# kbastani/pinot

Hardware: AMD Instinct MI355X
Metric: rows/sec scanned+aggregated (node) & % HBM peak, AdAnalytics GROUP BY query (higher is better)
Workload: dtype int64; 1 GPU; adanalytics; segments_per_gpu=1000, rows_per_gpu=1000000000, global_rows=1000000000, parallelism=dp1, groups=8, queries_in_flight=3, combine=local

## Files before the change

### include/pinotgpu.h

```cpp
#ifndef PINOTGPU_H
#define PINOTGPU_H

#include <stddef.h>
#include <stdint.h>

#ifdef __cplusplus
extern "C" {
#endif

#define PGPU_ABI_VERSION 3

#define PGPU_OK 0
#define PGPU_ERR_INVALID_ARGUMENT (-1)
#define PGPU_ERR_BAD_QUERY (-2)
#define PGPU_ERR_UNSUPPORTED (-3)
#define PGPU_ERR_DEVICE (-4)
#define PGPU_ERR_OUT_OF_MEMORY (-5)
#define PGPU_ERR_NOT_FOUND (-6)
#define PGPU_ERR_TIMEOUT (-7)
#define PGPU_ERR_CANCELLED (-8)

enum pgpu_data_type { PGPU_INT = 0, PGPU_LONG = 1, PGPU_FLOAT = 2, PGPU_DOUBLE = 3, PGPU_STRING = 4 };

enum pgpu_fwd_format { PGPU_FWD_FIXED_BIT = 0, PGPU_FWD_SORTED_PAIRS = 1, PGPU_FWD_RAW_FIXED = 2 };
// ... 78 lines not shown
  int32_t num_values;
  int32_t lower_inclusive;
  const char* const* values;
  int32_t upper_inclusive;
  int32_t reserved;
} pgpu_predicate;

enum pgpu_filter_opcode { PGPU_OP_PRED = 0, PGPU_OP_AND = 1, PGPU_OP_OR = 2, PGPU_OP_NOT = 3 };
typedef struct {
  int32_t op;
  int32_t arg;
} pgpu_filter_op;

enum pgpu_agg_fn { PGPU_AGG_COUNT = 0, PGPU_AGG_SUM = 1, PGPU_AGG_MIN = 2, PGPU_AGG_MAX = 3, PGPU_AGG_AVG = 4,
                   PGPU_AGG_DISTINCTCOUNT = 5, PGPU_AGG_PERCENTILE = 6 };
#define PGPU_AGG_PERCENTILE_MAX_E4 1000000
#define PGPU_AGG_PERCENTILE_OF(p_e4) ((int32_t)(PGPU_AGG_PERCENTILE | ((int32_t)(p_e4) << 8)))
#define PGPU_AGG_FN(fn) ((int32_t)((fn) & 0xFF))
#define PGPU_AGG_PERCENTILE_E4(fn) ((int32_t)(((uint32_t)(fn)) >> 8))
typedef struct {
  int32_t fn;
  int32_t column;
} pgpu_agg;

enum pgpu_expr_opcode { PGPU_EXPR_COLUMN = 0, PGPU_EXPR_LITERAL = 1, PGPU_EXPR_ADD = 2, PGPU_EXPR_SUB = 3,
                        PGPU_EXPR_MULT = 4, PGPU_EXPR_DIV = 5,
                        PGPU_EXPR_EQ = 6, PGPU_EXPR_NE = 7, PGPU_EXPR_GT = 8, PGPU_EXPR_GE = 9, PGPU_EXPR_LT = 10,
                        PGPU_EXPR_LE = 11, PGPU_EXPR_AND = 12, PGPU_EXPR_OR = 13, PGPU_EXPR_SELECT = 14,
                        PGPU_EXPR_ABS = 16, PGPU_EXPR_CEIL = 17, PGPU_EXPR_FLOOR = 18, PGPU_EXPR_SQRT = 19,
                        PGPU_EXPR_MOD = 20, PGPU_EXPR_LDIV = 21 };
#define PGPU_EXPR_MAX_OPS 16
#define PGPU_EXPR_MAX_DEPTH 4
#define PGPU_EXPR_MAX_COLUMNS 4
#define PGPU_EXPR_MAX_PER_TABLE 256
typedef struct {
  int32_t op;
  int32_t column;
  double literal;
} pgpu_expr_op;
int pgpu_table_add_expression(pgpu_table table, const pgpu_expr_op* ops, int32_t n, const char* name, int32_t* column);
int pgpu_table_expression(pgpu_table table, int32_t column, pgpu_expr_op* ops, int32_t cap, int32_t* n, char* name,
                          int32_t name_cap);

#define PGPU_GROUP_EXPR_COLUMN_BASE (1 << 20)
#define PGPU_GROUP_EXPR_MAX_PER_TABLE 64
#define PGPU_GROUP_EXPR_MAX_PRODUCT (1 << 22)
int pgpu_table_add_group_expression(pgpu_table table, const pgpu_expr_op* ops, int32_t n, const char* name,
                                    int32_t result_type , int32_t* column);

typedef struct {
  int32_t num_predicates;
  int32_t num_filter_ops;
  const pgpu_predicate* predicates;
  const pgpu_filter_op* filter;
  int32_t num_group_by;
  int32_t num_aggs;
  const int32_t* group_by;
  const pgpu_agg* aggs;
  int32_t num_groups_limit;
  int32_t options;
  int64_t end_time_ms;
} pgpu_query;

#define PGPU_OPT_NO_STAR_TREE 1
#define PGPU_OPT_SQL_GROUP_BY 2
#define PGPU_OPT_NO_PLAN_CACHE 4
#define PGPU_OPT_TIMING 8
#define PGPU_OPT_EXACT_FP_SUM 16

typedef struct pgpu_plan_s* pgpu_plan;
typedef struct pgpu_result_s* pgpu_result;

int pgpu_plan_create(pgpu_table table, const int64_t* segment_handles, int32_t num_segments, const pgpu_query* q,
                     pgpu_plan* out);
int pgpu_plan_destroy(pgpu_plan plan);

enum pgpu_slot_kind { PGPU_SLOT_COUNT = 0, PGPU_SLOT_SUM_I64 = 1, PGPU_SLOT_SUM_F64 = 2, PGPU_SLOT_MIN_KEY = 3,
                      PGPU_SLOT_MAX_KEY = 4 };
int pgpu_plan_layout(pgpu_plan plan, int32_t* num_slots, int64_t* num_keys, int32_t* slot_kinds );

int pgpu_plan_cancel(pgpu_plan plan);

int pgpu_plan_leaf_kinds(pgpu_plan plan, int64_t* counts);

int pgpu_plan_regexp_stats(pgpu_plan plan, int64_t* out4);
int pgpu_regex_check(const char* pattern, int32_t* states, int32_t* classes, int64_t* table_bytes);
int pgpu_regex_match_host(const char* pattern, const void* value, int64_t len, int32_t* matched);
int pgpu_table_regexp_dict_ids(pgpu_table table, int32_t column, const char* pattern, uint64_t* bitmap, int64_t words);

enum pgpu_group_path { PGPU_PATH_LDS = 0, PGPU_PATH_GLOBAL = 1, PGPU_PATH_HASH = 2, PGPU_PATH_PARTITIONED = 3,
                       PGPU_PATH_HASH_PARTITIONED = 4 };
int pgpu_plan_group_path(pgpu_plan plan, int32_t* path);

int pgpu_plan_execute(pgpu_plan plan, void* stream, void* d_table);

int pgpu_plan_finalize(pgpu_plan plan, void* stream, const void* d_table, pgpu_result* out);

int pgpu_plan_finalize_range(pgpu_plan plan, void* stream, const void* d_table_shard, int64_t key_begin,
                             int64_t key_count, pgpu_result* out);

int pgpu_plan_exchange_counts(pgpu_plan plan, void* stream, int32_t nparts, int64_t* counts);
int pgpu_plan_exchange_export(pgpu_plan plan, void* stream, int32_t nparts, const int32_t* kinds, void* d_out,
                              int64_t cap);
int pgpu_plan_exchange_merge(pgpu_plan plan, void* stream, const int32_t* kinds, const void* d_records, int64_t n);

typedef struct pgpu_comm_s* pgpu_comm;
#define PGPU_COMM_RCCL 0
#define PGPU_COMM_HOST 1
#define PGPU_COMM_ID_BYTES 128
int pgpu_comm_unique_id(int32_t kind, void* id );
int pgpu_comm_create(int32_t kind, const void* id, int32_t nranks, int32_t rank, int32_t device, pgpu_comm* out);
int pgpu_comm_destroy(pgpu_comm comm);
int pgpu_comm_rank(pgpu_comm comm, int32_t* rank, int32_t* nranks);
int pgpu_comm_allgather(pgpu_comm comm, const void* send, int64_t bytes, void* recv);
int pgpu_comm_set_timeout(pgpu_comm comm, int64_t timeout_ms);
int pgpu_comm_abort(pgpu_comm comm);
int pgpu_comm_status(pgpu_comm comm, int32_t* aborted);
int pgpu_comm_recreate(pgpu_comm comm, const void* id);

#define PGPU_COMBINE_LOCAL 0
#define PGPU_COMBINE_ALL_REDUCE 1
#define PGPU_COMBINE_REDUCE_SCATTER 2
#define PGPU_COMBINE_HASH 3
#define PGPU_COMBINE_ROWS 4
int pgpu_plan_combine_mode(pgpu_plan plan, pgpu_comm comm, int64_t shard_bytes, int32_t* mode, int32_t* kinds);
int pgpu_plan_combine(pgpu_plan plan, pgpu_comm comm, void* stream, void* d_table, int32_t mode, const int32_t* kinds,
                      void* d_shard, int64_t* key_begin, int64_t* key_count);
int pgpu_result_combine_rows(pgpu_result r, pgpu_comm comm, pgpu_result* out);

int pgpu_execute_groupby(pgpu_table table, const int64_t* segment_handles, int32_t num_segments, const pgpu_query* q,
                         void* stream, pgpu_result* out);

int pgpu_plan_create_execute(pgpu_table table, const int64_t* segment_handles, int32_t num_segments,
                             const pgpu_query* q, void* stream, void* d_table, pgpu_plan* out);

int pgpu_plan_timing(pgpu_plan plan, double* out4);

int pgpu_plan_fp_sum_format(pgpu_plan plan, int agg, int32_t out[4]);

typedef struct {
  int32_t is_sum;
  int32_t any, finite;
  int32_t E, L;
  int32_t reserved;
  int64_t docs;
  double  int_sum_bound;
} pgpu_fp_sum_range;
int pgpu_query_fp_sum_ranges(pgpu_table table, const int64_t* segment_handles, int32_t num_segments,
                             const pgpu_query* q, pgpu_fp_sum_range* out);
int pgpu_fp_sum_ranges_merge(const pgpu_fp_sum_range* all, int32_t nranks, int32_t num_aggs, pgpu_fp_sum_range* out);
int pgpu_comm_agree_fp_sum_ranges(pgpu_comm comm, pgpu_fp_sum_range* ranges, int32_t num_aggs);
int pgpu_plan_create_agreed(pgpu_table table, const int64_t* segment_handles, int32_t num_segments,
                            const pgpu_query* q, const pgpu_fp_sum_range* agreed, pgpu_plan* out);

int pgpu_plan_star_work(pgpu_plan plan, int64_t* out3);
int pgpu_plan_scan_geometry(pgpu_plan plan, int64_t* out16);
int pgpu_plan_star_metric_bytes(pgpu_plan plan, int64_t* bytes);

int pgpu_plan_scanned_segments(pgpu_plan plan, uint8_t* out);

enum pgpu_leaf_type { PGPU_LEAF_EMPTY = 0, PGPU_LEAF_MATCH_ALL = 1, PGPU_LEAF_SCAN = 2, PGPU_LEAF_SORTED = 3,
                      PGPU_LEAF_BITMAP = 4, PGPU_LEAF_RANGE_INDEX = 5, PGPU_LEAF_EXPRESSION = 6 };
int pgpu_filter_entries_scanned(const pgpu_filter_op* filter, int32_t num_filter_ops, const int32_t* leaf_types,
                                const uint32_t* const* leaf_masks, int32_t num_leaves, int32_t num_docs,
                                int64_t* out);

// ... 118 lines not shown
```

### pinot_amd/_lib.py

```python
import ctypes
import os

from .build import LIB_PATH

c_int = ctypes.c_int
c_i32 = ctypes.c_int32
c_i64 = ctypes.c_int64
c_u8p = ctypes.POINTER(ctypes.c_uint8)
c_i32p = ctypes.POINTER(ctypes.c_int32)
c_i64p = ctypes.POINTER(ctypes.c_int64)
c_u64p = ctypes.POINTER(ctypes.c_uint64)
c_f64p = ctypes.POINTER(ctypes.c_double)
c_voidp = ctypes.c_void_p
c_char_pp = ctypes.POINTER(ctypes.c_char_p)

PGPU_OK = 0
PGPU_ERR_INVALID_ARGUMENT = -1
PGPU_ERR_BAD_QUERY = -2
PGPU_ERR_UNSUPPORTED = -3
PGPU_ERR_DEVICE = -4
PGPU_ERR_OUT_OF_MEMORY = -5
PGPU_ERR_NOT_FOUND = -6
PGPU_ERR_TIMEOUT = -7
PGPU_ERR_CANCELLED = -8
# ... 114 lines not shown
    def as_tuple(self):
        return (self.is_sum, self.any, self.finite, self.E, self.L, self.docs, self.int_sum_bound)

    @classmethod
    def from_tuple(cls, t):
        return cls(int(t[0]), int(t[1]), int(t[2]), int(t[3]), int(t[4]), 0, int(t[5]), float(t[6]))


def fp_sum_range_array(ranges):
    items = [r if isinstance(r, FpSumRangeC) else FpSumRangeC.from_tuple(r) for r in ranges]
    arr = (FpSumRangeC * max(len(items), 1))()
    for i, r in enumerate(items):
        arr[i] = r
    return arr


def merge_fp_sum_ranges(per_rank):
    nranks, na = len(per_rank), len(per_rank[0])
    if any(len(r) != na for r in per_rank):
        raise ValueError("ranks report different numbers of aggregations")
    flat = fp_sum_range_array([x for r in per_rank for x in r])
    out = (FpSumRangeC * max(na, 1))()
    check(load().pgpu_fp_sum_ranges_merge(flat, nranks, na, out))
    return [FpSumRangeC.from_tuple(out[a].as_tuple()) for a in range(na)]


class PinotGpuError(RuntimeError):
    def __init__(self, code, message):
        super().__init__("pgpu error %d: %s" % (code, message))
        self.code = code
        self.message = message


class BadQueryRequestException(PinotGpuError):
    """PGPU_ERR_BAD_QUERY: mirrors org.apache.pinot.spi.exception.BadQueryRequestException."""


class UnsupportedQueryError(PinotGpuError):
    """PGPU_ERR_UNSUPPORTED: the query shape is outside the GPU path."""


class QueryCancelledError(PinotGpuError):
    """PGPU_ERR_CANCELLED: pgpu_plan_cancel abandoned the query (BaseOperator's EarlyTerminationException after the
    combine cancels its futures, BaseOperator.java:37-39 / BaseCombineOperator.java:124-130)."""


class QueryTimeoutError(PinotGpuError):
    """PGPU_ERR_TIMEOUT: the query's end time passed (the combine's TimeoutException; Pinot reports
    QueryException.EXECUTION_TIMEOUT_ERROR_CODE 250 for aggregation-only and QUERY_EXECUTION_ERROR_CODE 200 for
    group-by, BaseCombineOperator.java:193-203 / GroupByCombineOperator.java:193-203)."""


_PROTOS = {
    "pgpu_abi_version": (c_int, []),
    "pgpu_init": (c_int, [c_int]),
    "pgpu_shutdown": (c_int, []),
    "pgpu_last_error": (c_int, [ctypes.c_char_p, ctypes.c_size_t]),
    "pgpu_device_count": (c_int, [ctypes.POINTER(c_int)]),
    "pgpu_table_create": (c_int, [c_int, c_int, c_char_pp, c_i32p, ctypes.POINTER(c_voidp)]),
    "pgpu_config_default": (c_int, [ctypes.POINTER(ConfigC)]),
    "pgpu_table_set_config": (c_int, [c_voidp, ctypes.POINTER(ConfigC)]),
    "pgpu_table_get_config": (c_int, [c_voidp, ctypes.POINTER(ConfigC)]),
    "pgpu_table_destroy": (c_int, [c_voidp]),
    "pgpu_table_add_expression": (c_int, [c_voidp, ctypes.POINTER(ExprOpC), c_i32, ctypes.c_char_p, c_i32p]),
    "pgpu_table_add_group_expression": (c_int, [c_voidp, ctypes.POINTER(ExprOpC), c_i32, ctypes.c_char_p, c_i32, c_i32p]),
    "pgpu_table_expression": (c_int, [c_voidp, c_i32, ctypes.POINTER(ExprOpC), c_i32, c_i32p, ctypes.c_char_p, c_i32]),
    "pgpu_pin_segment": (c_int, [c_voidp, ctypes.POINTER(SegmentDesc), c_i64p]),
    "pgpu_unpin_segment": (c_int, [c_voidp, c_i64]),
    "pgpu_table_num_segments": (c_int, [c_voidp, c_i32p]),
    "pgpu_table_device_bytes": (c_i64, [c_voidp]),
    "pgpu_table_add_dictionary_values": (c_int, [c_voidp, c_int, c_i64, c_i64p, c_f64p, c_u8p, c_i64p]),
    "pgpu_table_dictionary_size": (c_int, [c_voidp, c_int, c_i64p]),
    "pgpu_table_dictionary_i64": (c_int, [c_voidp, c_int, c_i64p]),
    "pgpu_table_dictionary_f64": (c_int, [c_voidp, c_int, c_f64p]),
    "pgpu_table_dictionary_str": (c_int, [c_voidp, c_int, c_u8p, c_i64, c_i64p]),
    "pgpu_read_dict_ids": (c_int, [c_voidp, c_i64, c_int, c_i32p, c_i32, c_i32p]),
    "pgpu_unpack_fixed_bit_device": (c_int, [c_voidp, c_i64, c_i32, c_i64, c_i64, c_voidp, c_voidp]),
    "pgpu_plan_create": (c_int, [c_voidp, c_i64p, c_i32, ctypes.POINTER(QueryC), ctypes.POINTER(c_voidp)]),
    "pgpu_plan_destroy": (c_int, [c_voidp]),
    "pgpu_plan_create_execute": (c_int, [c_voidp, c_i64p, c_i32, ctypes.POINTER(QueryC), c_voidp, c_voidp,
                                         ctypes.POINTER(c_voidp)]),
    "pgpu_plan_layout": (c_int, [c_voidp, c_i32p, c_i64p, c_i32p]),
    "pgpu_plan_leaf_kinds": (c_int, [c_voidp, c_i64p]),
    "pgpu_plan_group_path": (c_int, [c_voidp, c_i32p]),
    "pgpu_plan_regexp_stats": (c_int, [c_voidp, c_i64p]),
    "pgpu_regex_check": (c_int, [ctypes.c_char_p, c_i32p, c_i32p, c_i64p]),
    "pgpu_regex_match_host": (c_int, [ctypes.c_char_p, ctypes.c_char_p, c_i64, c_i32p]),
    "pgpu_table_regexp_dict_ids": (c_int, [c_voidp, c_i32, ctypes.c_char_p, c_u64p, c_i64]),
    "pgpu_plan_cancel": (c_int, [c_voidp]),
    "pgpu_plan_execute": (c_int, [c_voidp, c_voidp, c_voidp]),
    "pgpu_plan_finalize": (c_int, [c_voidp, c_voidp, c_voidp, ctypes.POINTER(c_voidp)]),
    "pgpu_plan_finalize_range": (c_int, [c_voidp, c_voidp, c_voidp, c_i64, c_i64, ctypes.POINTER(c_voidp)]),
    "pgpu_plan_exchange_counts": (c_int, [c_voidp, c_voidp, c_i32, c_i64p]),
    "pgpu_plan_exchange_export": (c_int, [c_voidp, c_voidp, c_i32, c_i32p, c_voidp, c_i64]),
    "pgpu_plan_exchange_merge": (c_int, [c_voidp, c_voidp, c_i32p, c_voidp, c_i64]),
    "pgpu_execute_groupby": (c_int, [c_voidp, c_i64p, c_i32, ctypes.POINTER(QueryC), c_voidp,
                                     ctypes.POINTER(c_voidp)]),
    "pgpu_plan_timing": (c_int, [c_voidp, c_f64p]),
    "pgpu_plan_fp_sum_format": (c_int, [c_voidp, c_int, c_i32p]),
    "pgpu_query_fp_sum_ranges": (c_int, [c_voidp, c_i64p, c_i32, ctypes.POINTER(QueryC), ctypes.POINTER(FpSumRangeC)]),
    "pgpu_fp_sum_ranges_merge": (c_int, [ctypes.POINTER(FpSumRangeC), c_i32, c_i32, ctypes.POINTER(FpSumRangeC)]),
    "pgpu_comm_agree_fp_sum_ranges": (c_int, [c_voidp, ctypes.POINTER(FpSumRangeC), c_i32]),
    "pgpu_plan_create_agreed": (c_int, [c_voidp, c_i64p, c_i32, ctypes.POINTER(QueryC), ctypes.POINTER(FpSumRangeC),
                                        ctypes.POINTER(c_voidp)]),
    "pgpu_plan_star_work": (c_int, [c_voidp, c_i64p]),
    "pgpu_plan_scan_geometry": (c_int, [c_voidp, c_i64p]),
    "pgpu_plan_star_metric_bytes": (c_int, [c_voidp, c_i64p]),
    "pgpu_plan_scanned_segments": (c_int, [c_voidp, c_u8p]),
    "pgpu_attach_startree": (c_int, [c_voidp, c_i64, ctypes.POINTER(StarTreeDescC)]),
    "pgpu_attach_inverted_index": (c_int, [c_voidp, c_i64, c_i32, c_voidp, c_i64]),
    "pgpu_inverted_index_check": (c_int, [c_voidp, c_i64, c_i32, c_i32, c_voidp]),
    "pgpu_build_inverted_index": (c_int, [c_voidp, c_i64, c_i32, c_i32, c_i32, c_voidp, c_i64, c_i64p]),
    "pgpu_raw_forward_index_values": (c_int, [c_voidp, c_i64, c_i32, c_i32, c_i64p, c_f64p]),
    "pgpu_startree_build": (c_int, [ctypes.POINTER(SegmentDesc), c_i32p, c_i32p, c_i32, c_i32p, c_i32,
                                    ctypes.POINTER(AggC), c_i32, c_i32, ctypes.POINTER(c_voidp)]),
    "pgpu_startree_load": (c_int, [c_voidp, c_i64, ctypes.c_char_p, c_i64, c_i32, c_i32, c_i32, c_char_pp, c_i32p,
                                   ctypes.POINTER(c_voidp)]),
    "pgpu_startree_get_desc": (c_int, [c_voidp, ctypes.POINTER(StarTreeDescC)]),
    "pgpu_startree_num_raw_records": (c_int, [c_voidp, c_i32p]),
    "pgpu_startree_destroy": (c_int, [c_voidp]),
    "pgpu_result_num_groups": (c_int, [c_voidp, c_i64p]),
    "pgpu_result_key_dictionary": (c_int, [c_voidp, c_int, c_u64p, c_i64p]),
    "pgpu_result_key_dictionary_i64": (c_int, [c_voidp, c_int, c_i64p]),
    "pgpu_result_key_dictionary_f64": (c_int, [c_voidp, c_int, c_f64p]),
    "pgpu_result_key_dictionary_str": (c_int, [c_voidp, c_int, c_u8p, c_i64, c_i64p]),
    "pgpu_result_group_ids": (c_int, [c_voidp, c_i32p]),
    "pgpu_result_group_ids_column": (c_int, [c_voidp, c_int, c_i32p]),
    "pgpu_result_group_ids_view": (c_int, [c_voidp, c_int, ctypes.POINTER(c_voidp)]),
    "pgpu_result_words_view": (c_int, [c_voidp, c_int, ctypes.POINTER(c_voidp), c_i32p]),
    "pgpu_result_values": (c_int, [c_voidp, c_int, c_f64p]),
    "pgpu_result_avg_counts": (c_int, [c_voidp, c_int, c_i64p]),
    "pgpu_result_values_i64": (c_int, [c_voidp, c_int, c_i64p]),
    "pgpu_result_stats": (c_int, [c_voidp, c_i64p]),
    "pgpu_result_groups_limit_reached": (c_int, [c_voidp, ctypes.POINTER(ctypes.c_int32)]),
    "pgpu_result_slot_kinds": (c_int, [c_voidp, c_i32p, c_i32p]),
    "pgpu_result_exchange_rows": (c_int, [c_voidp, c_i32, c_i32p, c_i64p, c_i64p]),
    "pgpu_result_merge_rows": (c_int, [c_voidp, c_i64p, c_i64, c_i32p, ctypes.POINTER(c_voidp)]),
    "pgpu_result_destroy": (c_int, [c_voidp]),
    "pgpu_comm_unique_id": (c_int, [c_i32, c_voidp]),
    "pgpu_comm_create": (c_int, [c_i32, c_voidp, c_i32, c_i32, c_i32, ctypes.POINTER(c_voidp)]),
    "pgpu_comm_destroy": (c_int, [c_voidp]),
    "pgpu_comm_rank": (c_int, [c_voidp, c_i32p, c_i32p]),
    "pgpu_comm_allgather": (c_int, [c_voidp, c_voidp, c_i64, c_voidp]),
    "pgpu_comm_set_timeout": (c_int, [c_voidp, c_i64]),
    "pgpu_comm_abort": (c_int, [c_voidp]),
    "pgpu_comm_status": (c_int, [c_voidp, c_i32p]),
    "pgpu_attach_range_index": (c_int, [c_voidp, c_i64, c_i32, c_voidp, c_i64]),
    "pgpu_range_index_check": (c_int, [c_voidp, c_i64, c_i32, c_i32, c_i32p, c_i32p, c_i64p]),
    "pgpu_range_index_partial_entries": (c_int, [c_voidp, c_i64, c_i32, c_i32, c_i32, c_i32, c_i64p]),
    "pgpu_comm_recreate": (c_int, [c_voidp, c_voidp]),
    "pgpu_plan_combine_mode": (c_int, [c_voidp, c_voidp, c_i64, c_i32p, c_i32p]),
    "pgpu_plan_combine": (c_int, [c_voidp, c_voidp, c_voidp, c_voidp, c_i32, c_i32p, c_voidp, c_i64p, c_i64p]),
    "pgpu_result_combine_rows": (c_int, [c_voidp, c_voidp, ctypes.POINTER(c_voidp)]),
    "pgpu_free_result": (c_int, [c_voidp]),
    "pgpu_filter_bitmap": (c_int, [c_voidp, c_i64, ctypes.POINTER(QueryC), c_u64p]),
    "pgpu_result_trim_sql": (c_int, [c_voidp, ctypes.POINTER(SqlTrimC), ctypes.POINTER(c_voidp)]),
    "pgpu_result_trim_pql": (c_int, [c_voidp, c_i32, c_i32, c_i64p, c_i64, c_i64p]),
    "pgpu_result_datatable": (c_int, [c_voidp, c_voidp, c_voidp, c_i64, c_i64p]),
    "pgpu_broker_reduce_sql": (c_int, [ctypes.POINTER(c_voidp), c_i64p, c_i32, ctypes.POINTER(SqlTrimC), c_voidp,
                                       c_i64, c_i64p]),
    "pgpu_filter_entries_scanned": (c_int, [ctypes.POINTER(FilterOpC), c_i32, c_i32p, ctypes.POINTER(c_voidp), c_i32,
                                            c_i32, c_i64p]),
    "pgpu_generate_segment": (c_int, [c_voidp, ctypes.POINTER(GenColumnC), c_i32, c_i64, c_i32, c_i64p]),
    "pgpu_segment_column_info": (c_int, [c_voidp, c_i64, c_int, c_i32p, c_i32p, c_i64p, c_i64p]),
    "pgpu_segment_column_bytes": (c_int, [c_voidp, c_i64, c_int, c_u8p, c_u8p]),
}
# ... 79 lines not shown
```

### pinot_amd/build.py

```python
import hashlib
import os
import shutil
import subprocess

HERE = os.path.dirname(os.path.abspath(__file__))
ROOT = os.path.dirname(HERE)
CSRC = os.path.join(HERE, "csrc")
LIB_PATH = os.path.join(HERE, "libpinotgpu.so")
RUNTIME = ["rt_core", "rt_dict", "rt_plan", "rt_plan_create", "rt_exec", "rt_finalize", "rt_groups", "rt_regex",
           "abi_table", "abi_plan", "abi_combine", "abi_result"]
SOURCES = [("kernels.hip", [], "kernels")] + [(n + ".cpp", [], n) for n in RUNTIME] + [("startree.cpp", [], "startree"),
           ("filter_stats.cpp", [], "filter_stats"), ("range_index.cpp", [], "range_index"), ("comm.cpp", [], "comm"), ("server_response.cpp", [], "server_response"),
           ("k_partition.hip", [], "k_partition"), ("k_partition_fx.hip", [], "k_partition_fx"),
           ("k_hashfinal.hip", [], "k_hashfinal"), ("k_derive.hip", [], "k_derive"),
           ("regex_dfa.cpp", [], "regex_dfa"), ("k_regex.hip", [], "k_regex")] + \
    [("k_%s.hip" % k, ["-DPGPU_FAMILY=%d" % f, "-DPGPU_MODE=%d" % m], "k_%s%s_%d" % (k, ("", "_fx", "_dc", "_hist", "_expr")[f], m))
     for k, f, modes in (("direct", 0, 3), ("startree", 0, 3), ("direct", 1, 3), ("startree", 1, 3), ("direct", 2, 2),
                         ("direct", 3, 2), ("direct", 4, 3))
     for m in range(modes)]
HEADERS = ["internal.h", "device.h", "scan_direct.h", "host_common.h", "startree_kernels.h",
           "partition.h", "filter_stats.h", "host_result.h", "comm.h", "range_index.h", "rt.h",
           "rt_decls.h", "tile_split.h", "fx_sum.h", "key_range.h", "expr_eval.h", "expr_leaf.h", "expr_docs.h", "derive.h", "group_expr.h", "regex_dfa.h", "scan_direct_body.inc", "part_aggregate_body.inc",
           "part_hash_aggregate_body.inc"]
ARCH = os.environ.get("PGPU_OFFLOAD_ARCH", "gfx950")


def _hipcc():
    for cand in (os.environ.get("HIPCC"), "/opt/rocm/bin/hipcc", shutil.which("hipcc")):
        if cand and os.path.exists(cand):
            return cand
    raise RuntimeError("hipcc not found (ROCm is required to build libpinotgpu.so)")


def _inputs():
    files = [os.path.join(CSRC, s[0]) for s in SOURCES] + [os.path.join(CSRC, h) for h in HEADERS]
    files.append(os.path.join(ROOT, "include", "pinotgpu.h"))
    return files


def is_stale():
    if not os.path.exists(LIB_PATH):
        return True
    t = os.path.getmtime(LIB_PATH)
    return any(os.path.getmtime(f) > t for f in _inputs())


def build(force=False, verbose=False, defines=(), out=None):
    lib_path = out or LIB_PATH
    if not force and not defines and not out and not is_stale():
        return LIB_PATH
    hipcc = _hipcc()
    flags = ["--offload-arch=" + ARCH, "-O3", "-fPIC", "-std=c++17", "-munsafe-fp-atomics",
             "-Wall", "-Wno-unused-result", "-Wno-unused-value"] + ["-D" + d for d in defines]
    objdir = os.path.join(ROOT, "build", "obj" if not out else "obj_" + os.path.basename(out).replace(".", "_"))
    os.makedirs(objdir, exist_ok=True)
    procs = []
    objs = []
    common = hashlib.sha1()
    for h in HEADERS + ["../../include/pinotgpu.h"]:
        with open(os.path.join(CSRC, h), "rb") as f:
            common.update(f.read())
    for src, extra, name in SOURCES:
        obj = os.path.join(objdir, name + ".o")
        objs.append(obj)
        dbg = ["-g"] if src.endswith(".cpp") else []
        cmd = [hipcc] + flags + dbg + extra + ["-c", os.path.join(CSRC, src), "-o", obj]
        key = common.copy()
        key.update(" ".join(cmd).encode())
        with open(os.path.join(CSRC, src), "rb") as f:
            key.update(f.read())
        key = key.hexdigest()
        if not force and os.path.exists(obj) and os.path.exists(obj + ".key"):
            with open(obj + ".key") as f:
                if f.read() == key:
                    continue
        if verbose:
            print(" ".join(cmd))
        procs.append((src, obj, key, subprocess.Popen(cmd, cwd=ROOT, stdout=subprocess.PIPE, stderr=subprocess.STDOUT,
                                                      text=True)))
    errors = []
    for src, obj, key, pr in procs:
        out, _ = pr.communicate()
        if pr.returncode != 0:
            errors.append("%s:\n%s" % (src, out[-8000:]))
        else:
            with open(obj + ".key", "w") as f:
                f.write(key)
    if errors:
        raise RuntimeError("hipcc failed:\n" + "\n".join(errors))
    cmd = [hipcc, "--offload-arch=" + ARCH, "-shared", "-fPIC", "-o", lib_path + ".tmp"] + objs + ["-ldl"]
    res = subprocess.run(cmd, cwd=ROOT, stdout=subprocess.PIPE, stderr=subprocess.STDOUT, text=True)
    if res.returncode != 0:
        raise RuntimeError("hipcc link failed:\n" + res.stdout[-8000:])
    os.replace(lib_path + ".tmp", lib_path)
    return lib_path


def build_tools():
    hipcc = _hipcc()
    out = os.path.join(ROOT, "tools", "qps_native")
    cmd = [hipcc, "--offload-arch=" + ARCH, "-O2", "-std=c++17", os.path.join(ROOT, "tools", "qps_native.cpp"), "-I" + os.path.join(ROOT, "include"),
           "-L" + HERE, "-lpinotgpu", "-Wl,-rpath,$ORIGIN/../pinot_amd", "-o", out]
    res = subprocess.run(cmd, cwd=ROOT, stdout=subprocess.PIPE, stderr=subprocess.STDOUT, text=True)
    if res.returncode != 0:
        raise RuntimeError("hipcc (tools) failed:\n" + res.stdout[-4000:])
    return out


SAN_FLAGS = ["-Xarch_host", "-fsanitize=address", "-Xarch_host", "-fsanitize=undefined", "-Xarch_host",
             "-fno-sanitize-recover=undefined", "-Xarch_host", "-fno-omit-frame-pointer"]
FUZZ_PATH = os.path.join(ROOT, "build", "host_fuzz")


def build_host_fuzz(force=False):
    src = os.path.join(ROOT, "tools", "host_fuzz.cpp")
    if not force and os.path.exists(FUZZ_PATH) and \
            all(os.path.getmtime(f) <= os.path.getmtime(FUZZ_PATH) for f in _inputs() + [src]):
        return FUZZ_PATH
    hipcc = _hipcc()
    flags = ["--offload-arch=" + ARCH, "-O1", "-g", "-std=c++17", "-fPIC",
             "-I" + os.path.join(ROOT, "include")] + SAN_FLAGS
    objdir = os.path.join(ROOT, "build", "obj_san")
    os.makedirs(objdir, exist_ok=True)
    jobs = [(os.path.join(CSRC, s), extra, os.path.join(objdir, name + ".o")) for s, extra, name in SOURCES]
    jobs.append((src, [], os.path.join(objdir, "host_fuzz_main.o")))
    hdr_t = max(os.path.getmtime(f) for f in _inputs() if not f.endswith((".cpp", ".hip")))
    procs = [(s, subprocess.Popen([hipcc] + flags + extra + ["-c", s, "-o", o], cwd=ROOT, stdout=subprocess.PIPE,
                                  stderr=subprocess.STDOUT, text=True)) for s, extra, o in jobs
             if force or not os.path.exists(o) or os.path.getmtime(o) < max(os.path.getmtime(s), hdr_t)]
    errors = []
    for s, pr in procs:
        out, _ = pr.communicate()
        if pr.returncode != 0:
            errors.append("%s:\n%s" % (s, out[-6000:]))
    if errors:
        raise RuntimeError("hipcc (host sanitizers) failed:\n" + "\n".join(errors))
    cmd = [hipcc, "--offload-arch=" + ARCH, "-fsanitize=address", "-fsanitize=undefined", "-o", FUZZ_PATH + ".tmp"] + \
        [o for _, _, o in jobs] + ["-ldl", "-lpthread"]
    res = subprocess.run(cmd, cwd=ROOT, stdout=subprocess.PIPE, stderr=subprocess.STDOUT, text=True)
    if res.returncode != 0:
        raise RuntimeError("hipcc (host sanitizers) link failed:\n" + res.stdout[-6000:])
    os.replace(FUZZ_PATH + ".tmp", FUZZ_PATH)
    return FUZZ_PATH


def _build_header_check(name, src, hdr, force=False, extra=()):
    out = os.path.join(ROOT, "build", name)
    src = os.path.join(ROOT, "tools", src)
    hdr = os.path.join(CSRC, hdr)
    if not force and os.path.exists(out) and all(os.path.getmtime(f) <= os.path.getmtime(out) for f in (src, hdr)):
        return out
    os.makedirs(os.path.dirname(out), exist_ok=True)
    hipcc = _hipcc()
    obj = out + ".o"
    for cmd in ([hipcc, "--offload-arch=" + ARCH, "-O1", "-g", "-std=c++17", "-I" + CSRC] + SAN_FLAGS +
                list(extra) + ["-c", src, "-o", obj],
                [hipcc, "--offload-arch=" + ARCH, "-fsanitize=address", "-fsanitize=undefined", obj,
                 "-o", out + ".tmp"]):
        res = subprocess.run(cmd, cwd=ROOT, stdout=subprocess.PIPE, stderr=subprocess.STDOUT, text=True)
        if res.returncode != 0:
            raise RuntimeError("hipcc (%s) failed:\n%s" % (name, res.stdout[-6000:]))
    os.replace(out + ".tmp", out)
    return out


SPLIT_CHECK_PATH = os.path.join(ROOT, "build", "tile_split_check")
FX_CHECK_PATH = os.path.join(ROOT, "build", "fx_sum_check")
AGREE_CHECK_PATH = os.path.join(ROOT, "build", "fx_agree_check")


def build_tile_split_check(force=False):
    return _build_header_check("tile_split_check", "tile_split_check.cpp", "tile_split.h", force)


def build_fx_sum_check(force=False):
    return _build_header_check("fx_sum_check", "fx_sum_check.cpp", "fx_sum.h", force)


def build_fx_agree_check(force=False):
    return _build_header_check("fx_agree_check", "fx_agree_check.cpp", "fx_sum.h", force)


def build_key_range_check(force=False):
    return _build_header_check("key_range_check", "key_range_check.cpp", "key_range.h", force)


def build_expr_check(force=False):
    return _build_header_check("expr_check", "expr_check.cpp", "expr_eval.h", force, extra=("-ffp-contract=off",))


def build_case_check(force=False):
    return _build_header_check("case_check", "case_check.cpp", "expr_eval.h", force, extra=("-ffp-contract=off",))


def build_math_check(force=False):
    return _build_header_check("math_check", "math_check.cpp", "expr_eval.h", force, extra=("-ffp-contract=off",))


def build_group_expr_check(force=False):
    return _build_header_check("group_expr_check", "group_expr_check.cpp", "group_expr.h", force,
                               extra=("-ffp-contract=off",))


def build_expr_filter_check(force=False):
    out = os.path.join(ROOT, "build", "expr_filter_check")
    srcs = [os.path.join(ROOT, "tools", "expr_filter_check.cpp"), os.path.join(CSRC, "filter_stats.cpp")]
    deps = srcs + [os.path.join(CSRC, h) for h in ("expr_leaf.h", "expr_eval.h", "internal.h", "filter_stats.h",
                                                    "host_common.h", "tile_split.h")]
    if not force and os.path.exists(out) and all(os.path.getmtime(f) <= os.path.getmtime(out) for f in deps):
        return out
    os.makedirs(os.path.dirname(out), exist_ok=True)
    hipcc = _hipcc()
    objs = [out + "_%d.o" % i for i in range(len(srcs))]
    cmds = [[hipcc, "--offload-arch=" + ARCH, "-O1", "-g", "-std=c++17", "-I" + CSRC, "-I" + os.path.join(ROOT, "include"),
             "-ffp-contract=off"] + SAN_FLAGS + ["-c", s, "-o", o] for s, o in zip(srcs, objs)]
    cmds.append([hipcc, "--offload-arch=" + ARCH, "-fsanitize=address", "-fsanitize=undefined"] + objs + ["-o", out + ".tmp"])
    for cmd in cmds:
        res = subprocess.run(cmd, cwd=ROOT, stdout=subprocess.PIPE, stderr=subprocess.STDOUT, text=True)
        if res.returncode != 0:
            raise RuntimeError("hipcc (expr_filter_check) failed:\n%s" % res.stdout[-6000:])
    os.replace(out + ".tmp", out)
    return out


def build_regex_fuzz(force=False):
    out = os.path.join(ROOT, "build", "regex_fuzz")
    srcs = [os.path.join(ROOT, "tools", "regex_fuzz.cpp"), os.path.join(CSRC, "regex_dfa.cpp")]
    deps = srcs + [os.path.join(CSRC, "regex_dfa.h")]
    if not force and os.path.exists(out) and all(os.path.getmtime(f) <= os.path.getmtime(out) for f in deps):
        return out
    os.makedirs(os.path.dirname(out), exist_ok=True)
    hipcc = _hipcc()
    objs = [out + "_%d.o" % i for i in range(len(srcs))]
    cmds = [[hipcc, "--offload-arch=" + ARCH, "-O1", "-g", "-std=c++17", "-I" + CSRC] + SAN_FLAGS + ["-c", s, "-o", o]
            for s, o in zip(srcs, objs)]
    cmds.append([hipcc, "--offload-arch=" + ARCH, "-fsanitize=address", "-fsanitize=undefined"] + objs + ["-o", out + ".tmp"])
    for cmd in cmds:
        res = subprocess.run(cmd, cwd=ROOT, stdout=subprocess.PIPE, stderr=subprocess.STDOUT, text=True)
        if res.returncode != 0:
            raise RuntimeError("hipcc (regex_fuzz) failed:\n%s" % res.stdout[-6000:])
    os.replace(out + ".tmp", out)
    return out


if __name__ == "__main__":
    print(build(force=True, verbose=True))
```

### pinot_amd/csrc/abi_result.cpp

```cpp
#include "rt_decls.h"

extern "C" {

int pgpu_execute_groupby(pgpu_table t, const int64_t* handles, int32_t nsegs, const pgpu_query* q, void* stream,
                         pgpu_result* out) try {
  PGPU_ABI_GUARD;
  pgpu_plan P = nullptr;
  TRY(pgpu_plan_create_execute(t, handles, nsegs, q, stream, nullptr, &P));
  int rc = pgpu_plan_finalize(P, stream, nullptr, out);
  std::string keep = g_err;
  pgpu_plan_destroy(P);
  g_err = keep;
  return rc;
} PGPU_ABI_CATCH

int pgpu_plan_scanned_segments(pgpu_plan P, uint8_t* out) try {
  PGPU_ABI_GUARD;
  if (!P || !out) return fail(PGPU_ERR_INVALID_ARGUMENT, "null argument");
  if (!P->seg_scanned.empty()) memcpy(out, P->seg_scanned.data(), P->seg_scanned.size());
  return 0;
} PGPU_ABI_CATCH

int pgpu_plan_star_work(pgpu_plan P, int64_t* out3) try {
  PGPU_ABI_GUARD;
// ... 308 lines not shown
      std::vector<double> sorted = vals;
      std::sort(sorted.begin(), sorted.end(), dbl_less);
      sorted.erase(std::unique(sorted.begin(), sorted.end(),
                               [](double a, double b) { return !dbl_less(a, b) && !dbl_less(b, a); }),
                   sorted.end());
      D.code_to_pos.resize(g0.n);
      for (int i = 0; i < g0.n; ++i)
        D.code_to_pos[i] = (int32_t)(std::lower_bound(sorted.begin(), sorted.end(), vals[i], dbl_less) - sorted.begin());
      D.pos_f64 = sorted;
      D.npos = (int64_t)sorted.size();
    } else {
      return fail(PGPU_ERR_INVALID_ARGUMENT, "column %d: bad generator kind", c);
    }
  }
  GenScratch& G = t->gen;
  std::vector<std::vector<int32_t>> pos_to_id(ncols);
  TRY(G.pos.ensure((size_t)std::max(num_docs, 1) * 4 * ncols));
  for (int c = 0; c < ncols; ++c) {
    const pgpu_gen_column& g0 = gc[c];
    Domain& D = dom[c];
    const int64_t pres_words = (D.npos + 31) / 32;
    TRY(G.presence.ensure((size_t)pres_words * 4));
    HIP_TRY(hipMemsetAsync(G.presence.p, 0, (size_t)pres_words * 4, st));
    if (!D.code_to_pos.empty()) {
      TRY(G.code_to_pos.ensure(D.code_to_pos.size() * 4));
      HIP_TRY(hipMemcpyAsync(G.code_to_pos.p, D.code_to_pos.data(), D.code_to_pos.size() * 4, hipMemcpyHostToDevice, st));
    }
    if (g0.kind == PGPU_GEN_ZIPF) {
      TRY(G.cdf.ensure((size_t)g0.n * 8));
      HIP_TRY(hipMemcpyAsync(G.cdf.p, g0.cdf, (size_t)g0.n * 8, hipMemcpyHostToDevice, st));
    }
    const uint64_t seed = (uint64_t)(0x5EED0000u + (uint32_t)g0.column_index) << 32;
    const int32_t ncodes = g0.kind == PGPU_GEN_UNIFORM ? 0 : g0.n;
    if (launch_gen_positions(g0.kind, seed, g0.lo, g0.hi - g0.lo, G.cdf.as<double>(), G.code_to_pos.as<int32_t>(),
                             ncodes, row0, num_docs, G.pos.as<int32_t>() + (size_t)c * std::max(num_docs, 1),
                             G.presence.as<uint32_t>(), st))
      return fail(PGPU_ERR_DEVICE, "gen positions launch failed");
    std::vector<uint32_t> pres(pres_words);
    HIP_TRY(hipMemcpyAsync(pres.data(), G.presence.p, (size_t)pres_words * 4, hipMemcpyDeviceToHost, st));
    HIP_TRY(hipStreamSynchronize(st));
    Column& col = seg->cols[c];
    col.dict.type = t->types[c];
    std::vector<int32_t>& p2i = pos_to_id[c];
    p2i.assign(std::max<int64_t>(D.npos, 1), 0);
    int32_t card = 0;
    for (int64_t p = 0; p < D.npos; ++p)
      if ((pres[p >> 5] >> (p & 31)) & 1u) {
        p2i[p] = card++;
        if (g0.kind == PGPU_GEN_UNIFORM) col.dict.iv.push_back(g0.lo + p);
        else if (g0.kind == PGPU_GEN_ZIPF) col.dict.iv.push_back(D.pos_i64[p]);
        else col.dict.dv.push_back(D.pos_f64[p]);
      }
    col.card = card;
    col.bits = num_bits_per_value(card - 1);
    const int type = t->types[c];
    col.entry_width = (type == PGPU_INT || type == PGPU_FLOAT) ? 4 : 8;
    col.raw_dict.assign((size_t)card * col.entry_width, 0);
    for (int32_t i = 0; i < card; ++i) {
      uint8_t* o = col.raw_dict.data() + (size_t)i * col.entry_width;
      if (type == PGPU_INT) wr_be32(o, (uint32_t)(int32_t)col.dict.iv[i]);
      else if (type == PGPU_LONG) wr_be64(o, (uint64_t)col.dict.iv[i]);
      else if (type == PGPU_FLOAT) { float f = (float)col.dict.dv[i]; uint32_t u; memcpy(&u, &f, 4); wr_be32(o, u); }
      else { uint64_t u; memcpy(&u, &col.dict.dv[i], 8); wr_be64(o, u); }
    }
    col.fwd_bytes = ((int64_t)num_docs * col.bits + 7) / 8;
    col.fwd_words = padded_fwd_words(num_docs, col.bits);
    total_words += (col.fwd_words + 63) & ~int64_t(63);
  }
  HIP_TRY(hipMalloc(&seg->d_block, (size_t)std::max<int64_t>(total_words, 64) * 4));
  t->device_bytes += std::max<int64_t>(total_words, 64) * 4;
  HIP_TRY(hipMemsetAsync(seg->d_block, 0, (size_t)std::max<int64_t>(total_words, 64) * 4, st));
  int64_t off = 0;
  for (int c = 0; c < ncols; ++c) {
    Column& col = seg->cols[c];
    col.d_fwd = reinterpret_cast<uint32_t*>(seg->d_block) + off;
    off += (col.fwd_words + 63) & ~int64_t(63);
    TRY(G.pos_to_id.ensure(pos_to_id[c].size() * 4));
    HIP_TRY(hipMemcpyAsync(G.pos_to_id.p, pos_to_id[c].data(), pos_to_id[c].size() * 4, hipMemcpyHostToDevice, st));
    if (launch_gen_pack(G.pos.as<int32_t>() + (size_t)c * std::max(num_docs, 1), G.pos_to_id.as<int32_t>(), num_docs,
                        col.bits, col.d_fwd, st))
      return fail(PGPU_ERR_DEVICE, "gen pack launch failed");
    HIP_TRY(hipStreamSynchronize(st));
  }
  std::lock_guard<std::mutex> lk(t->mu);
  *handle = register_segment(t, std::move(seg));
  return 0;
} PGPU_ABI_CATCH

int pgpu_segment_column_info(pgpu_table t, int64_t h, int col, int32_t* card, int32_t* bits, int64_t* dict_len,
                             int64_t* fwd_len) try {
  PGPU_ABI_GUARD;
  if (!t) return fail(PGPU_ERR_INVALID_ARGUMENT, "null table");
  DeviceGuard g(t->device);
  std::lock_guard<std::mutex> lk(t->mu);
  auto it = t->segments.find(h);
  if (it == t->segments.end()) return fail(PGPU_ERR_NOT_FOUND, "unknown segment handle");
  const Column* cp = nullptr;
  TRY(segment_column(t, *it->second, col, &cp));
  const Column& c = *cp;
  if (card) *card = c.card;
  if (bits) *bits = c.bits;
  if (dict_len) *dict_len = (int64_t)c.raw_dict.size();
  if (fwd_len) *fwd_len = c.fwd_bytes;
  return 0;
} PGPU_ABI_CATCH

int pgpu_segment_column_bytes(pgpu_table t, int64_t h, int col, uint8_t* dict_out, uint8_t* fwd_out) try {
  PGPU_ABI_GUARD;
  if (!t) return fail(PGPU_ERR_INVALID_ARGUMENT, "null table");
  DeviceGuard g(t->device);
  std::shared_ptr<Segment> s;
  const Column* cp = nullptr;
  {
    std::lock_guard<std::mutex> lk(t->mu);
    auto it = t->segments.find(h);
    if (it == t->segments.end()) return fail(PGPU_ERR_NOT_FOUND, "unknown segment handle");
    s = it->second;
    TRY(segment_column(t, *s, col, &cp));
  }
  const Column& c = *cp;
  if (dict_out && !c.raw_dict.empty()) memcpy(dict_out, c.raw_dict.data(), c.raw_dict.size());
  if (fwd_out && c.fwd_bytes > 0) {
    HIP_TRY(hipMemcpyAsync(fwd_out, c.d_fwd, (size_t)c.fwd_bytes, hipMemcpyDeviceToHost, t->stream));
    HIP_TRY(hipStreamSynchronize(t->stream));
  }
  return 0;
} PGPU_ABI_CATCH

}
```

### pinot_amd/csrc/abi_table.cpp

```cpp
#include "rt_decls.h"

extern "C" {

int pgpu_abi_version(void) { return PGPU_ABI_VERSION; }

namespace {
std::mutex g_init_mu;
int g_init_devices = 0;
}

int pgpu_init(int n_gpus) try {
  PGPU_ABI_GUARD;
  install_crash_trace();
  int count = 0;
  HIP_TRY(hipGetDeviceCount(&count));
  if (n_gpus > count) return fail(PGPU_ERR_INVALID_ARGUMENT, "%d devices requested, %d visible", n_gpus, count);
  const int n = n_gpus > 0 ? n_gpus : count;
  std::lock_guard<std::mutex> g(g_init_mu);
  int prev = 0;
  HIP_TRY(hipGetDevice(&prev));
  for (int d = g_init_devices; d < n; ++d) {
    HIP_TRY(hipSetDevice(d));
    HIP_TRY(hipFree(nullptr));
  }
// ... 305 lines not shown
                    (long long)cb.fwd_len, (long long)need);
      col.fwd_bytes = need;
    } else if (cb.fwd_format == PGPU_FWD_SORTED_PAIRS) {
      if (cb.fwd_len < (int64_t)cb.cardinality * 8) return fail(PGPU_ERR_INVALID_ARGUMENT, "column %d: sorted index too small", c);
      col.bits = num_bits_per_value(cb.cardinality - 1);
      col.fwd_bytes = ((int64_t)d->num_docs * col.bits + 7) / 8;
      std::vector<uint32_t>& w = sorted_expansion[c];
      w.assign(padded_fwd_words(d->num_docs, col.bits), 0u);
      col.sorted = true;
      col.sorted_start.assign((size_t)cb.cardinality + 1, d->num_docs);
      int32_t prev_end = -1;
      for (int32_t id = 0; id < cb.cardinality; ++id) {
        const int32_t s = (int32_t)rd_be32(cb.fwd + (int64_t)id * 8), e = (int32_t)rd_be32(cb.fwd + (int64_t)id * 8 + 4);
        if (s < 0 || e >= d->num_docs || (e < s && e != s - 1)) return fail(PGPU_ERR_INVALID_ARGUMENT, "bad sorted pair");
        if (s != prev_end + 1) return fail(PGPU_ERR_INVALID_ARGUMENT, "sorted pairs are not contiguous");
        prev_end = e;
        col.sorted_start[id] = s;
        for (int32_t doc = s; doc <= e; ++doc) {
          const uint64_t bit = (uint64_t)doc * col.bits;
          for (int b = 0; b < col.bits; ++b)
            if ((id >> (col.bits - 1 - b)) & 1) {
              const uint64_t pos = bit + b;
              w[pos >> 5] |= 1u << (31 - (pos & 31));
            }
        }
      }
      if (d->num_docs > 0 && prev_end != d->num_docs - 1)
        return fail(PGPU_ERR_INVALID_ARGUMENT, "sorted pairs do not cover every doc");
      for (auto& x : w) x = __builtin_bswap32(x);
    } else if (cb.fwd_format == PGPU_FWD_RAW_FIXED) {
      TRY(parse_raw_column(t->types[c], cb, d->num_docs, c, &col, &raw_values[c]));
      any_raw = true;
      continue;
    } else {
      return fail(PGPU_ERR_INVALID_ARGUMENT, "column %d: bad forward-index format", c);
    }
    col.fwd_words = padded_fwd_words(d->num_docs, col.bits);
    total_words += (col.fwd_words + 63) & ~int64_t(63);
  }
  HIP_TRY(hipMalloc(&seg->d_block, (size_t)std::max<int64_t>(total_words, 64) * 4));
  t->device_bytes += std::max<int64_t>(total_words, 64) * 4;
  int64_t off = 0;
  for (int c = 0; c < d->num_columns; ++c) {
    Column& col = seg->cols[c];
    if (col.raw) {
      const size_t n = (size_t)raw_padded_docs(d->num_docs);
      raw_values[c].key.resize(n, 0);
      raw_values[c].val.resize(n, 0.0);
      HIP_TRY(hipMalloc(&col.d_key, n * 8));
      HIP_TRY(hipMalloc(&col.d_val, n * 8));
      t->device_bytes += 16 * (int64_t)n;
      HIP_TRY(hipMemcpyAsync(col.d_key, raw_values[c].key.data(), n * 8, hipMemcpyHostToDevice, t->stream));
      HIP_TRY(hipMemcpyAsync(col.d_val, raw_values[c].val.data(), n * 8, hipMemcpyHostToDevice, t->stream));
      continue;
    }
    col.d_fwd = reinterpret_cast<uint32_t*>(seg->d_block) + off;
    const pgpu_column_buffers& cb = d->columns[c];
    HIP_TRY(hipMemsetAsync(col.d_fwd, 0, (size_t)col.fwd_words * 4, t->stream));
    if (cb.fwd_format == PGPU_FWD_SORTED_PAIRS) {
      HIP_TRY(hipMemcpyAsync(col.d_fwd, sorted_expansion[c].data(), (size_t)col.fwd_words * 4, hipMemcpyHostToDevice,
                             t->stream));
    } else if (col.fwd_bytes > 0) {
      HIP_TRY(hipMemcpyAsync(col.d_fwd, cb.fwd, (size_t)col.fwd_bytes, hipMemcpyHostToDevice, t->stream));
    }
    off += (col.fwd_words + 63) & ~int64_t(63);
  }
  std::vector<int> check;
  for (int c = 0; c < d->num_columns; ++c) {
    const Column& col = seg->cols[c];
    if (!col.raw && !col.sorted && d->num_docs > 0 && (int64_t)col.card < (INT64_C(1) << col.bits)) check.push_back(c);
  }
  DevBuf dmax;
  struct Release { DevBuf& b; ~Release() { b.release(); } } release_dmax{dmax};
  std::vector<uint32_t> hmax(check.size(), 0);
  if (!check.empty()) {
    TRY(dmax.ensure(check.size() * 4));
    HIP_TRY(hipMemsetAsync(dmax.p, 0, check.size() * 4, t->stream));
    for (size_t i = 0; i < check.size(); ++i)
      if (launch_fwd_max(seg->cols[check[i]].d_fwd, d->num_docs, seg->cols[check[i]].bits,
                         dmax.as<unsigned int>() + i, t->stream))
        return fail(PGPU_ERR_DEVICE, "forward-index check launch failed: %s", hipGetErrorString(hipGetLastError()));
    HIP_TRY(hipMemcpyAsync(hmax.data(), dmax.p, check.size() * 4, hipMemcpyDeviceToHost, t->stream));
  }
  HIP_TRY(hipStreamSynchronize(t->stream));
  for (size_t i = 0; i < check.size(); ++i)
    if ((int64_t)hmax[i] >= seg->cols[check[i]].card) {
      account_unpin(t, seg.get());
      return fail(PGPU_ERR_INVALID_ARGUMENT, "column %d: forward index holds dictId %u, cardinality is %d", check[i],
                  hmax[i], seg->cols[check[i]].card);
    }
  std::lock_guard<std::mutex> lk(t->mu);
  if (any_raw) TRY(ensure_docid(t, d->num_docs, t->stream));
  *handle = register_segment(t, std::move(seg));
  return 0;
} PGPU_ABI_CATCH

int pgpu_unpin_segment(pgpu_table t, int64_t h) try {
  PGPU_ABI_GUARD;
  if (t) t->version++;
  if (!t) return fail(PGPU_ERR_INVALID_ARGUMENT, "null table");
  DeviceGuard g(t->device);
  std::shared_ptr<Segment> seg;
  {
    std::lock_guard<std::mutex> lk(t->mu);
    auto it = t->segments.find(h);
    if (it == t->segments.end()) return fail(PGPU_ERR_NOT_FOUND, "unknown segment handle %lld", (long long)h);
    seg = std::move(it->second);
    account_unpin(t, seg.get());
    t->by_handle[h].reset();
    t->segments.erase(it);
  }
  plan_cache_clear(t);
  hipStreamSynchronize(t->stream);
  return 0;
} PGPU_ABI_CATCH

namespace {
bool parse_roaring(const uint8_t* b, int64_t n, int32_t num_docs, std::vector<uint32_t>& words,
                   std::vector<InvIndex::Cont>& conts, int64_t* docs) {
  auto u16 = [&](int64_t o) { return (uint32_t)b[o] | ((uint32_t)b[o + 1] << 8); };
  auto u32 = [&](int64_t o) { return u16(o) | (u16(o + 2) << 16); };
  if (n < 4) return false;
  const uint32_t cookie = u32(0);
  int64_t pos, size;
  const uint8_t* runbits = nullptr;
  bool offsets;
  if ((cookie & 0xFFFF) == 12347) {
    size = (cookie >> 16) + 1;
    runbits = b + 4;
    pos = 4 + (size + 7) / 8;
    offsets = size >= 4;
  } else if (cookie == 12346) {
    if (n < 8) return false;
    size = u32(4);
    pos = 8;
    offsets = true;
  } else {
    return false;
  }
  if (size < 0 || size > 65536 || pos + size * 4 > n) return false;
  const int64_t desc = pos;
  pos += size * 4 + (offsets ? size * 4 : 0);
  *docs = 0;
  int32_t prev_key = -1;
  std::vector<uint32_t> vals;
  for (int64_t i = 0; i < size; ++i) {
    const int32_t key = (int32_t)u16(desc + 4 * i);
    const int32_t card = (int32_t)u16(desc + 4 * i + 2) + 1;
    if (key <= prev_key || ((int64_t)key << 16) >= num_docs) return false;
    prev_key = key;
    const bool run = runbits && ((runbits[i >> 3] >> (i & 7)) & 1);
    vals.clear();
    std::vector<uint32_t> bm;
    if (run) {
      if (pos + 2 > n) return false;
      const int64_t nruns = u16(pos);
      pos += 2;
      if (pos + nruns * 4 > n) return false;
      for (int64_t r = 0; r < nruns; ++r) {
        const uint32_t start = u16(pos + 4 * r), len = u16(pos + 4 * r + 2);
        if (start + len > 65535) return false;
        if ((int64_t)vals.size() + len + 1 > card) return false;
        for (uint32_t v = start; v <= start + len; ++v) vals.push_back(v);
      }
      pos += nruns * 4;
    } else if (card <= 4096) {
      if (pos + (int64_t)card * 2 > n) return false;
      for (int32_t k = 0; k < card; ++k) vals.push_back(u16(pos + 2 * k));
      pos += (int64_t)card * 2;
    } else {
      if (pos + 8192 > n) return false;
      bm.resize(kContainerWords);
      for (int w = 0; w < kContainerWords; ++w) bm[w] = u32(pos + 4 * w);
// ... 230 lines not shown
```

### pinot_amd/csrc/device.h

```cpp
#pragma once
#include <hip/hip_runtime.h>

#include <utility>

#include "fx_sum.h"
#include "internal.h"

namespace pgpu {

#define PGPU_HIP_OK(x) ((x) == hipSuccess ? 0 : -1)

template <typename T>
using gmem = const __attribute__((address_space(1))) T;
template <typename T>
__device__ __forceinline__ gmem<T>* gp(const T* p) { return (gmem<T>*)p; }
template <typename T>
using cmem = const __attribute__((address_space(4))) T;
using KColC = cmem<KCol>;
using KLeafC = cmem<KLeaf>;
template <typename T>
__device__ __forceinline__ cmem<T>* cp(const T* p) { return (cmem<T>*)p; }

__device__ __forceinline__ uint32_t bswap32(uint32_t x) { return __builtin_bswap32(x); }

// ... 170 lines not shown
}

__device__ __forceinline__ uint32_t bitdir_mask(uint64_t e, int negate, int64_t group) {
  const uint32_t m = (e & 1ull) ? array_group_mask(e, group) : e ? gp(reinterpret_cast<const uint32_t*>(e))[group & 2047] : 0u;
  return negate ? ~m : m;
}

template <int B>
__device__ __forceinline__ void bitdir_range_b(const uint32_t* __restrict__ words, uint32_t lo, uint32_t span,
                                               uint64_t e, int neg0, int64_t group, uint32_t& m0, uint32_t& m1) {
  uint32_t w[B + 1];
  load_group<B, true>(words, w);
  m0 = bitdir_mask(e, neg0, group);
  m1 = span == 1 ? eq_all<B>(w, lo, std::make_integer_sequence<int, 32>{})
                 : range_all<B>(w, lo, lo + span, std::make_integer_sequence<int, 32>{});
}
__device__ __forceinline__ void bitdir_range(const uint32_t* fwd, int bits, uint32_t lo, uint32_t span, int neg1,
                                             uint64_t e, int neg0, int64_t group, uint32_t& m0, uint32_t& m1) {
  const uint32_t* words = fwd + group * (int64_t)bits;
  m0 = 0;
  m1 = 0;
  switch (bits) {
#define PGPU_CASE(B)                                                 \
  case B:                                                            \
    bitdir_range_b<B>(words, lo, span, e, neg0, group, m0, m1); \
    break;
    PGPU_CASE(1) PGPU_CASE(2) PGPU_CASE(3) PGPU_CASE(4) PGPU_CASE(5) PGPU_CASE(6) PGPU_CASE(7) PGPU_CASE(8)
    PGPU_CASE(9) PGPU_CASE(10) PGPU_CASE(11) PGPU_CASE(12) PGPU_CASE(13) PGPU_CASE(14) PGPU_CASE(15)
    PGPU_CASE(16) PGPU_CASE(17) PGPU_CASE(18) PGPU_CASE(19) PGPU_CASE(20) PGPU_CASE(21) PGPU_CASE(22)
    PGPU_CASE(23) PGPU_CASE(24) PGPU_CASE(25) PGPU_CASE(26) PGPU_CASE(27) PGPU_CASE(28) PGPU_CASE(29)
    PGPU_CASE(30) PGPU_CASE(31)
#undef PGPU_CASE
    default: break;
  }
  if (neg1) m1 = ~m1;
}

__device__ __forceinline__ uint32_t leaf_eval(int kind, int negate, uint32_t lo, uint32_t span, const uint32_t* set,
                                              const uint32_t* fwd, int bits, int64_t group) {
  if (kind == LEAF_DOCRANGE) {
    const uint32_t m = docrange_mask(group, lo, span);
    return negate ? ~m : m;
  }
  if (kind == LEAF_BITMAP) {
    const uint32_t m = gp(set)[group];
    return negate ? ~m : m;
  }
  if (kind == LEAF_BITDIR) {
    const uint64_t e = gp(reinterpret_cast<const uint64_t*>(set))[group >> 11];
    const uint32_t m = (e & 1ull) ? array_group_mask(e, group) : e ? gp(reinterpret_cast<const uint32_t*>(e))[group & 2047] : 0u;
    return negate ? ~m : m;
  }
  return leaf_eval_words(kind, negate, lo, span, set, fwd + group * (int64_t)bits, bits);
}

__device__ __forceinline__ uint32_t raw_group_mask(int kind, int64_t lo, int64_t hi, const int64_t* set_keys,
                                                   const int64_t* keys, int64_t group) {
  gmem<int64_t>* __restrict__ s = gp(set_keys);
  gmem<int64_t>* __restrict__ v = gp(keys) + group * 32;
  uint32_t m = 0;
  if (kind == LEAF_RAW_RANGE) {
#pragma unroll
    for (int i = 0; i < 32; ++i) {
      const int64_t x = v[i];
      m |= (uint32_t)(lo <= x && x <= hi) << i;
    }
  } else {
    const int n = (int)hi;
    for (int i = 0; i < 32; ++i) {
      const int64_t key = v[i];
      int a = 0, b = n;
      while (a < b) {
        const int mid = (a + b) >> 1;
        if (s[mid] < key) a = mid + 1;
        else b = mid;
      }
      m |= (uint32_t)(a < n && s[a] == key) << i;
    }
  }
  return m;
}

__device__ __forceinline__ uint32_t leaf_mask(KLeafC& L, KColC& C, int64_t group) {
  return leaf_eval(L.kind, L.negate, L.lo, L.span, L.set, C.fwd, C.bits, group);
}

struct SegView {
  cmem<KSegHdr>* hdr;
  KColC* cols;
  KLeafC* leaves;
};

__device__ __forceinline__ uint32_t vidx(KColC& c, uint32_t id) {
  for (int k = 0; k < c.ngaps; ++k) id += id >= c.gaps[k] ? 1u : 0u;
  return id;
}
template <int N>
__device__ __forceinline__ void vidx_n(KColC& c, uint32_t (&ids)[N]) {
  const int ng = c.ngaps;
  for (int k = 0; k < ng; ++k) {
    const uint32_t g = c.gaps[k];
#pragma unroll
    for (int i = 0; i < N; ++i) ids[i] += ids[i] >= g ? 1u : 0u;
  }
}

__device__ __forceinline__ SegView seg_view(const KParams& p, int seg) {
  const uint8_t* base = p.segs + (int64_t)seg * p.seg_stride;
  SegView v;
  v.hdr = cp(reinterpret_cast<const KSegHdr*>(base));
  v.cols = cp(reinterpret_cast<const KCol*>(base + sizeof(KSegHdr)));
  v.leaves = cp(reinterpret_cast<const KLeaf*>(base + sizeof(KSegHdr) + sizeof(KCol) * p.num_cols));
  return v;
}

__device__ __forceinline__ void put_compact(uint8_t* o, int64_t j, int width, uint64_t v) {
  switch (width) {
    case 1: o[j] = (uint8_t)v; break;
    case 2: reinterpret_cast<uint16_t*>(o)[j] = (uint16_t)v; break;
    case 3:
      o[3 * j] = (uint8_t)v;
      o[3 * j + 1] = (uint8_t)(v >> 8);
      o[3 * j + 2] = (uint8_t)(v >> 16);
      break;
    case 4: reinterpret_cast<uint32_t*>(o)[j] = (uint32_t)v; break;
    default: reinterpret_cast<uint64_t*>(o)[j] = v; break;
  }
}

__device__ __forceinline__ uint64_t slot_init(int kind) {
  if (kind == SLOT_MIN_KEY) return (uint64_t)INT64_MAX;
  if (kind == SLOT_MAX_KEY) return (uint64_t)INT64_MIN;
  return 0ull;
}
__device__ __forceinline__ uint64_t slot_init_lds(int kind, bool narrow) {
  if (narrow) return kind == SLOT_MIN_KEY ? 0xFFFFFFFFull : 0ull;
  return slot_init(kind);
}

struct LeafReg {
  const uint32_t* fwd;
  const uint32_t* set;
  int32_t bits, kind, negate;
  uint32_t lo, span;
};

__device__ __forceinline__ uint32_t leaf_mask_reg(const LeafReg& R, int64_t group) {
  return leaf_eval(R.kind, R.negate, R.lo, R.span, R.set, R.fwd, R.bits, group);
}

__device__ __forceinline__ LeafReg load_leaf_reg(const KParams& p, const SegView& S, int l) {
  LeafReg r;
  KLeafC& L = S.leaves[l];
  KColC& C = S.cols[p.leaf_col[l]];
  r.fwd = C.fwd;
  r.bits = C.bits;
  r.kind = L.kind;
  r.negate = L.negate;
  r.lo = L.lo;
  r.span = L.span;
  r.set = L.set;
  return r;
}

__device__ __forceinline__ uint32_t eval_filter(const KParams& p, const SegView& S, int64_t group, uint32_t mask,
                                                uint32_t* __restrict__ stack) {
  if (p.num_ops == 0) return mask;
  if (p.pure_and) {
    for (int l = 0; l < p.num_leaves; ++l) {
      if (!__any(mask != 0u)) break;
      mask &= leaf_mask(S.leaves[l], S.cols[p.leaf_col[l]], group);
    }
    return mask;
  }
  const int tid = threadIdx.x;
  int sp = 0;
  for (int k = 0; k < p.num_ops; ++k) {
    const int op = p.ops[k] >> 16, arg = p.ops[k] & 0xFFFF;
    if (op == OP_LEAF) {
      stack[sp * kBlock + tid] = leaf_mask(S.leaves[arg], S.cols[p.leaf_col[arg]], group);
      ++sp;
    } else if (op == OP_NOT) {
      stack[(sp - 1) * kBlock + tid] = ~stack[(sp - 1) * kBlock + tid];
    } else {
      uint32_t acc = stack[(sp - arg) * kBlock + tid];
      for (int j = sp - arg + 1; j < sp; ++j) {
        const uint32_t x = stack[j * kBlock + tid];
        acc = (op == OP_AND) ? (acc & x) : (acc | x);
      }
      sp -= arg;
      stack[sp * kBlock + tid] = acc;
      ++sp;
    }
  }
  return mask & stack[tid];
}

__device__ __forceinline__ int64_t hash_slot(unsigned long long* __restrict__ keys, int64_t cap, uint64_t key,
                                             unsigned long long* full) {
  uint64_t h = key * 0x9E3779B97F4A7C15ull;
  h ^= h >> 29;
  int64_t s = (int64_t)(h & (uint64_t)(cap - 1));
  for (int64_t probes = 0; probes < cap; ++probes) {
    unsigned long long k = keys[s];
    if (k == key) return s;
    if (k == ~0ull) {
      const unsigned long long prev = atomicCAS(&keys[s], ~0ull, (unsigned long long)key);
      if (prev == ~0ull || prev == key) return s;
    }
    s = (s + 1) & (cap - 1);
  }
  if (full) atomicOr(full, 1ull);
  return -1;
}

__device__ __forceinline__ const KFxSplit& fx_split(const KParams& p) { return static_cast<const KParamsFx&>(p).fx; }

__device__ __forceinline__ const KDistinct& dc_bitmaps(const KParams& p) { return static_cast<const KParamsDc&>(p).dc; }

__device__ __forceinline__ void distinct_mark(unsigned long long* __restrict__ row, uint32_t gid) {
  unsigned long long* w = row + (gid >> 6);
  const unsigned long long m = 1ull << (gid & 63u);
  if (!(*gp(w) & m)) atomicOr(w, m);
}

__device__ __forceinline__ const KHist& side_hists(const KParams& p) { return static_cast<const KParamsHist&>(p).hs; }

__device__ __forceinline__ void hist_add(uint32_t* __restrict__ row, uint32_t gid) { atomicAdd(row + gid, 1u); }

constexpr int kSideNone = 0, kSideBitmap = 1, kSideHist = 2;
constexpr int kSideExpr = 3;
template <int DC>
__device__ __forceinline__ constexpr int side_slot_kind() { return DC == kSideHist ? SLOT_PERCENTILE : SLOT_DISTINCT; }

__device__ __forceinline__ const KExpr& expr_programs(const KParams& p) { return static_cast<const KParamsExpr&>(p).ex; }

template <int NB>
__device__ __forceinline__ void expr_batch(const ExprProg& P, const SegView (&S)[NB], const int64_t (&doc)[NB],
                                           const bool (&ok)[NB], double (&out)[NB]) {
// ... 802 lines not shown
```

### pinot_amd/csrc/internal.h

```cpp
#pragma once
#include <stdint.h>

#include "expr_eval.h"
#include "tile_split.h"

namespace pgpu {

constexpr int kDocsPerLane = 32;
constexpr int kTileDocs = kBlock * kDocsPerLane;
constexpr int kLdsPackShift = 40;
constexpr int kMaxQueryCols = 16;
constexpr int kMaxLeaves = 16;
constexpr int kMaxOps = 48;
constexpr int kMaxKeys = 16;
constexpr int kMaxSlots = 24;
constexpr int kFwdPadWords = 4;
constexpr int kFlushAt = 128;
constexpr int kDenseGroupMin = 256;
constexpr int kFastLeaves = 4;

enum LeafKind : int32_t { LEAF_NONE = 0, LEAF_ALL = 1, LEAF_RANGE = 2, LEAF_SET = 3, LEAF_DOCRANGE = 4, LEAF_BITMAP = 5,
                          LEAF_RAW_RANGE = 6, LEAF_RAW_IN = 7, LEAF_BITDIR = 8, LEAF_EXPR_RANGE = 9, LEAF_EXPR_IN = 10 };
constexpr int kLeafKinds = 9;
enum OpCode : int32_t { OP_LEAF = 0, OP_AND = 1, OP_OR = 2, OP_NOT = 3 };
enum SlotKind : int32_t { SLOT_COUNT = 0, SLOT_SUM_I64 = 1, SLOT_SUM_F64 = 2, SLOT_MIN_KEY = 3, SLOT_MAX_KEY = 4,
                          SLOT_SUM_FX = 5, SLOT_DISTINCT = 6, SLOT_PERCENTILE = 7 };
enum Mode : int32_t { MODE_LDS = 0, MODE_GLOBAL = 1, MODE_HASH = 2 };

enum StatsWord : int {
  STAT_MATCHED = 0,
  STAT_STAR_ENTRIES = 1,
  STAT_SCAN_ENTRIES = 2,
  STAT_STAR_DOCS_READ = 3,
  STAT_HASH_FULL = 4,
  STAT_TIMED_OUT = 5,
  STAT_TILE_CLAIMS = 6,
  STAT_STAR_SECTORS = 7,
};
constexpr int kStatsWords = 8;
constexpr int kStatsBytes = kStatsWords * 8;
constexpr int kStatsReadWords = STAT_TIMED_OUT + 1;
constexpr int kStatsReadBytes = kStatsReadWords * 8;

struct KLeaf {
  int32_t kind;
  int32_t negate;
  uint32_t lo;
  uint32_t span;
  const uint32_t* set;
};

constexpr int kMaxValueGaps = 16;

struct KCol {
  const uint32_t* fwd;
  const int32_t* lut;
  const int64_t* dkey;
  const double* dval;
  int64_t key_base;
  int32_t bits;
  int32_t lut_off;
  int32_t ngaps;
  uint32_t gaps[kMaxValueGaps];
};

struct KSegHdr {
  int32_t num_docs;
  int32_t tile_base;
  int32_t num_tiles;
  int32_t stats;
};
enum KStats : int32_t { KSTATS_NONE = 0, KSTATS_CHAIN = 1, KSTATS_LEAP2 = 2 };

struct KParams {
  const uint8_t* segs;
  const int32_t* tile_seg;
  int32_t seg_stride;
  int32_t num_cols;
  int32_t num_segs;
  int32_t num_tiles;
  int32_t tile_shift;
  int32_t tile_chunks;
  int32_t slot_n;
  uint16_t slot_w[4];
  int32_t pair_leaves;
  int32_t num_ops;
  int32_t pure_and;
  int32_t ops[kMaxOps];
  int32_t num_leaves;
  int32_t leaf_col[kMaxLeaves];
  int32_t num_keys;
  int32_t key_col[kMaxKeys];
  int64_t key_stride[kMaxKeys];
  int64_t num_keys_total;
  int64_t key_bias;
  int32_t num_slots;
  int32_t slot_kind[kMaxSlots];
  int32_t slot_col[kMaxSlots];
  int32_t pack_slot;
  int32_t pack_shift;
  uint32_t narrow;
  uint64_t* table;
  uint64_t* slab;
  unsigned long long* hash_keys;
  int32_t num_stages;
  int32_t stage_end[kMaxKeys];
  int64_t stage_cap[kMaxKeys];
  int64_t stage_off[kMaxKeys];
  int64_t stage_mult[kMaxKeys];
  unsigned long long* stage_keys;
  unsigned long long* stats;
  uint8_t* leap_maps;
  uint64_t deadline;
  unsigned long long* diag_times;
  unsigned int* claim;
  int32_t claim_base;
  int32_t claim_tiles;
};

struct KFxSplit {
  int16_t sh[kMaxSlots];
  int8_t k[kMaxSlots];
  int8_t j[kMaxSlots];
};
struct KParamsFx : KParams {
  KFxSplit fx;
};

constexpr int kMaxDistinct = 8;
constexpr int64_t kDistinctMaxBytes = int64_t(1) << 30;
struct KDistinct {
  unsigned long long* bits[kMaxDistinct];
// ... 154 lines not shown
  uint64_t* mid_val;
  int32_t val32;
  int32_t pack_bits;
  int64_t pack_min;
  int32_t fine_pack;
  int32_t cs_pack;
  int64_t pack_range;
  int32_t hashed;
  int32_t pbits;
  int32_t sbits;
  uint32_t* rec_key32;
  int32_t mid_pair;
  int32_t staged;
  int32_t stage_off;
  uint64_t* out_rec;
  unsigned long long* out_count;
  int64_t out_cap;
  unsigned long long* out_mm;
  uint32_t* chunk_cnt;
  long long* chunk_mm;
};
struct KPartParamsFx : KPartParams {
  KFxSplit fx;
};
constexpr int kHashPartStreams = 4;
constexpr int kHashPartProbes = 128;

constexpr int kSplitBatch = 2048;
constexpr size_t part_split_lds(int cshift, int streams, int batch, int key_bytes = 2) {
  return (size_t)3 * ((size_t)1 << cshift) * 4 + 8 + (size_t)streams * batch * 8 + (size_t)batch * (4 + key_bytes) + 16;
}
constexpr size_t part_hash_lds(int sbits, int num_slots) {
  return ((size_t)1 << sbits) * ((size_t)num_slots * 8 + 4);
}

enum ContainerType : int32_t { CONT_ARRAY = 0, CONT_BITMAP = 1 };
constexpr int kContainerWords = 2048;
struct KBitTask {
  const uint32_t* payload;
  int32_t type;
  int32_t n;
  int64_t dst;
};
struct KBitBlock {
  int64_t dst;
  int32_t task_begin;
  int32_t num_tasks;
};

struct KRawTask {
  const int64_t* keys;
  int64_t dst;
  int64_t lo, hi;
  int32_t num_docs;
  int32_t kind;
  int32_t negate;
  int32_t pad;
};
struct KRawJob {
  int32_t task;
  int32_t group0;
};

struct KExprLeafTask {
  ExprOperands ops;
  ExprProg prog;
  int64_t dst;
  int64_t lo, hi;
  int32_t num_docs;
  int32_t kind;
  int32_t negate;
  int32_t pad;
};
static_assert(__builtin_offsetof(KExprLeafTask, prog) == 80 && sizeof(KExprLeafTask) == 336, "the layout the kernel was built for");
constexpr int kExprLeafJobDocs = 8192;
struct KExprLeafJob {
  int32_t task;
  int32_t doc0;
};

int launch_unpack(const uint32_t* fwd, int32_t bits, int64_t start, int64_t n, int32_t* out, void* stream);
int launch_gather_ids(const uint32_t* fwd, int32_t bits, const int32_t* docs, int32_t n, int32_t* out, void* stream);
int launch_fwd_max(const void* d_fwd, int64_t n, int32_t bits, unsigned int* d_out, void* stream);
int launch_hash_unpack(uint64_t* table, const unsigned long long* hash_keys, int64_t cap, int32_t pack_slot,
                       int32_t shift, void* stream);
int launch_table_init(uint64_t* table, const int32_t* slot_kind, int32_t num_slots, int64_t num_keys,
                      unsigned long long* hash_keys, void* stream);
int launch_expand_tiles(const uint8_t* segs, int32_t seg_stride, int32_t num_segs, int32_t* tile_seg,
                        uint64_t deadline, unsigned long long* stats, void* stream);
KernelEntry scan_entry(int mode, int variant);
int launch_scan(const KParams& p, const KFxSplit& fx, const KDistinct& dc, const KHist& hs, const KExpr& ex, int mode,
                int variant, int grid, size_t lds_bytes, void* stream);
int launch_percentile_select(const KHist& hs, const KPctSelect& sel, uint64_t* table, int64_t num_keys, void* stream);
int launch_distinct_popcount(const KDistinct& dc, uint64_t* table, int64_t num_keys, void* stream);
int launch_distinct_merge_popcount(const KDistinct& dc, const KDistinctRecv& rv, uint64_t* table, int64_t num_keys,
                                   int64_t begin, int64_t count, int nranks, void* stream);
int occupancy_scan(int mode, int variant, size_t lds_bytes);
int launch_reduce_slabs(const uint64_t* slab, const int32_t* slot_kind_dev, int32_t num_slots, int64_t num_keys,
                        int32_t num_blocks, uint64_t* out, void* stream);
int launch_compact(const uint64_t* table, const unsigned long long* hash_keys, int32_t num_slots, int64_t num_keys,
                   unsigned long long* counter, uint64_t* out, int64_t out_cap, void* stream);
int64_t compact_ordered_chunks(int64_t num_keys);
int launch_compact_ordered(const uint64_t* table, int32_t num_slots, int64_t num_keys, int64_t key_base,
                           const int64_t* key_stride, const int64_t* key_card, const int64_t* key_off,
                           int32_t num_key_cols,
                           uint32_t* chunk_scratch,
                           unsigned long long* total, void* out, int64_t cap, void* stream);
int launch_exchange_count(const uint64_t* table, const unsigned long long* hash_keys, int64_t num_keys, int32_t nparts,
                          unsigned long long* counts, void* stream);
int launch_exchange_scatter(const uint64_t* table, const unsigned long long* hash_keys, int64_t num_keys,
                            int32_t num_slots, int32_t nparts, uint32_t conv, unsigned long long* cursor, uint64_t* out,
                            void* stream);
int launch_i64_to_f64(uint64_t* p, int64_t n, void* stream);
int launch_hash_minmax(const uint64_t* rec, const unsigned long long* count, int64_t cap, int32_t num_slots,
                       unsigned long long* mm, void* stream);
int launch_hash_minmax_parts(const unsigned long long* part_mm, int32_t num_parts, int32_t num_slots,
                             unsigned long long* mm, void* stream);
int launch_hash_compact(const uint64_t* rec, int64_t n, int32_t num_slots, int32_t key_width, const int32_t* width,
                        const int64_t* slot_off, uint8_t* out, void* stream);
int launch_hash_decode(const uint64_t* rec, int64_t n, int32_t num_slots, int32_t num_keys, const int64_t* stride,
                       const int64_t* card, const int64_t* off, uint8_t* out, size_t slot_off, void* stream);
int launch_merge_records(const uint64_t* rec, int64_t n, int32_t num_slots, const int32_t* slot_kind, uint64_t* table,
                         unsigned long long* hash_keys, int64_t num_keys, void* stream);
size_t compact_scratch_bytes(int64_t num_keys, int32_t num_slots);
int launch_compact_dense_count(const uint64_t* table, int32_t num_slots, int64_t num_keys, uint32_t* chunk_scratch,
                               unsigned long long* total, long long* minmax, void* stream, bool counted = false);
constexpr int kCompactChunkKeys = 4096;
int launch_compact_dense_scatter(const uint64_t* table, int32_t num_slots, int64_t num_keys, const int32_t* slot_kind,
                                 const uint32_t* chunk_scratch, const long long* minmax, uint64_t* bitmap,
                                 void* out_slots, int64_t cap, void* stream);
int compact_slot_width(long long lo, long long hi, int kind);
int launch_compact_ordered_scatter(const uint64_t* table, int32_t num_slots, int64_t num_keys, int64_t key_base,
                                   const int64_t* key_stride, const int64_t* key_card, const int64_t* key_off,
                                   int32_t num_key_cols, const uint32_t* chunk_scratch, void* out, int64_t cap,
                                   void* stream);
int occupancy_part_pass(size_t pass_lds, int num_parts, int num_coarse, int staged);
int launch_partitioned(const KPartParams& pp, int grid, size_t pass_lds, void* stream, const KFxSplit* fx = nullptr);
int launch_part_aggregate_fx(const KPartParamsFx& pp, size_t lds_bytes, void* stream);
int launch_part_hash_aggregate_fx(const KPartParamsFx& pp, size_t lds_bytes, void* stream);
int launch_exclusive_scan_u32(uint32_t* data, int32_t n, void* stream);
int launch_filter_bitmap(const KParams& p, uint32_t* out_words, void* stream);
int launch_epilogue(const uint64_t* slab, const int32_t* slot_kind, int32_t num_slots, int64_t num_keys,
                    int32_t num_blocks, uint64_t* out, const uint8_t* segs, int32_t seg_stride, int32_t num_segs,
                    const uint8_t* maps, unsigned long long* stats, void* stream);
int launch_leap2_compose(const uint8_t* segs, int32_t seg_stride, int32_t num_segs, const uint8_t* maps,
                         unsigned long long* stats, void* stream);
int launch_leaf_masks(const KParams& p, const KMaskJob* jobs, int32_t num_jobs, uint32_t* out, void* stream);
int launch_inv_materialize(const KBitBlock* blocks, int64_t num_blocks, const KBitTask* tasks, uint32_t* docbits,
                           void* stream);
int launch_raw_leaf_bitmaps(const KRawJob* jobs, int64_t num_jobs, const KRawTask* tasks, const int64_t* raw_vals,
                            uint32_t* docbits, void* stream);
int launch_expr_leaf_bitmaps(const KExprLeafJob* jobs, int64_t num_jobs, const KExprLeafTask* tasks,
                             const int64_t* expr_vals, uint32_t* docbits, void* stream);
constexpr int kStarMaxSegs = 4096;
int launch_deadline_gate(uint64_t deadline, unsigned long long* stats, void* stream);
int launch_startree_traverse(const KStarSeg* segs, int32_t num_segs, int64_t* seg_total, uint64_t deadline,
                             unsigned long long* stats, void* stream);
int launch_startree_scan(const KStarParams& p, int mode, bool fx, size_t lds_bytes, void* stream);
int launch_gen_positions(int32_t kind, uint64_t seed, int64_t lo, int64_t span, const double* cdf,
                         const int32_t* code_to_pos, int32_t n_codes, int64_t row0, int32_t num_docs,
                         int32_t* pos_out, uint32_t* presence, void* stream);
int launch_read_clock(uint64_t* out, void* stream);
int launch_gen_pack(const int32_t* pos, const int32_t* pos_to_id, int32_t num_docs, int32_t bits, uint32_t* fwd_out,
                    void* stream);

int launch_regex_match_dict(const uint8_t* cls, const uint16_t* table, int32_t table_entries, int32_t num_classes,
// ... 14 lines not shown
```

### pinot_amd/csrc/rt.h

```cpp
#pragma once
#include <hip/hip_runtime.h>
#include <dlfcn.h>
#include <execinfo.h>
#include <pthread.h>
#include <signal.h>
#include <unistd.h>

#include <algorithm>
#include <array>
#include <atomic>
#include <chrono>
#include <condition_variable>
#include <functional>
#include <thread>
#include <cerrno>
#include <cmath>
#include <cstdarg>
#include <cstdio>
#include <cstdlib>
#include <cstring>
#include <limits>
#include <list>
#include <map>
#include <unordered_map>
#include <memory>
#include <mutex>
#include <numeric>
#include <string>
#include <tuple>
#include <vector>

#include "../../include/pinotgpu.h"
#include "comm.h"
#include "filter_stats.h"
#include "host_common.h"
#include "host_result.h"
#include "internal.h"
#include "range_index.h"



namespace pgpu {

bool diag(const char* word);
void install_crash_trace();
extern thread_local std::string g_err;
bool trace_on();
double now_us();
int fail(int code, const char* fmt, ...) __attribute__((format(printf, 2, 3)));


#define HIP_TRY(expr)                                                                               \
  do {                                                                                              \
    hipError_t _e = (expr);                                                                         \
    if (_e != hipSuccess)                                                                           \
      return fail(_e == hipErrorOutOfMemory ? PGPU_ERR_OUT_OF_MEMORY : PGPU_ERR_DEVICE, "%s: %s (%s:%d)", \
                  #expr, hipGetErrorString(_e), __FILE__, __LINE__);                                \
  } while (0)

#define TRY(expr)          \
  do {                     \
    int _rc = (expr);      \
    if (_rc) return _rc;   \
  } while (0)

#define PGPU_TIMING_RECORD(P, ev, stream)                   \
  do {                                                      \
    if ((P)->timed) HIP_TRY(hipEventRecord(ev, stream));    \
  } while (0)

struct DeviceGuard {
  int prev = -1;
  explicit DeviceGuard(int dev) {
    hipGetDevice(&prev);
    if (prev != dev) hipSetDevice(dev);
  }
  ~DeviceGuard() {
    int cur = -1;
    hipGetDevice(&cur);
    if (prev >= 0 && cur != prev) hipSetDevice(prev);
  }
};

struct DevBuf {
  void* p = nullptr;
  size_t cap = 0;
  int ensure(size_t n) {
    if (n <= cap) return 0;
    if (p && trace_on()) fprintf(stderr, "[pgpu] device buffer grows %zu -> %zu bytes\n", cap, n + n / 4);
    if (p) HIP_TRY(hipFree(p));
    p = nullptr;
    size_t c = std::max<size_t>(n + n / 4, 4096);
    HIP_TRY(hipMalloc(&p, c));
    cap = c;
    return 0;
  }
  void release() {
    if (p) hipFree(p);
    p = nullptr;
    cap = 0;
  }
  template <class T>
  T* as() const { return reinterpret_cast<T*>(p); }
};

struct DevMem {
  void* p = nullptr;
  DevMem() = default;
  DevMem(const DevMem&) = delete;
  DevMem& operator=(const DevMem&) = delete;
  ~DevMem() { if (p) hipFree(p); }
};

class HostPool {
 public:
// ... 129 lines not shown
  while (max_value) { n++; max_value >>= 1; }
  return n;
}

inline bool parse_long(const char* s, int64_t lo, int64_t hi, int64_t* out) {
  const char* p = s;
  bool neg = false;
  if (*p == '+' || *p == '-') { neg = *p == '-'; ++p; }
  if (!*p) return false;
  unsigned __int128 v = 0;
  for (; *p; ++p) {
    if (*p < '0' || *p > '9') return false;
    v = v * 10 + (unsigned)(*p - '0');
    if (v > ((unsigned __int128)1 << 64)) return false;
  }
  __int128 sv = neg ? -(__int128)v : (__int128)v;
  if (sv < lo || sv > hi) return false;
  *out = (int64_t)sv;
  return true;
}
inline bool parse_double(const char* s, double* out) {
  char* end = nullptr;
  errno = 0;
  double d = strtod(s, &end);
  if (end == s) return false;
  while (*end == 'd' || *end == 'D' || *end == 'f' || *end == 'F' || *end == ' ') ++end;
  if (*end) return false;
  *out = d;
  return true;
}

inline int cmp_bytes(const uint8_t* a, size_t na, const uint8_t* b, size_t nb) {
  int c = memcmp(a, b, std::min(na, nb));
  if (c) return c;
  return na < nb ? -1 : (na > nb ? 1 : 0);
}

inline std::atomic<uint64_t> g_dict_ids{1};
struct Dict {
  int type = PGPU_INT;
  uint64_t id = 0;
  uint64_t digest = 0;
  std::vector<int64_t> iv;
  std::vector<double> dv;
  std::vector<std::string> sv;
  size_t size() const { return is_int_type(type) ? iv.size() : is_fp_type(type) ? dv.size() : sv.size(); }
};

struct InvIndex {
  struct Cont { int64_t word; int32_t type, n, key; };
  ~InvIndex() { if (d_block) hipFree(d_block); }
  void* d_block = nullptr;
  int64_t bytes = 0;
  struct Entry { int32_t begin, count; int64_t docs; };
  std::vector<Entry> ids;
  std::vector<Cont> conts;
};

struct Column {
  int32_t card = 0, bits = 0, entry_width = 0, padding = 0;
  int64_t fwd_bytes = 0;
  uint32_t* d_fwd = nullptr;
  int64_t fwd_words = 0;
  Dict dict;
  bool sorted = false;
  std::vector<int32_t> sorted_start;
  std::vector<uint8_t> raw_dict;
  std::shared_ptr<DevMem> lut;
  uint64_t lut_version = ~0ull;
  int32_t lut_off = -1;
  uint64_t vmap_version = ~0ull;
  int32_t vgap_first = -1;
  std::vector<uint32_t> vgaps;
  int64_t* d_key = nullptr;
  double* d_val = nullptr;
  bool key_affine = false;
  int64_t key_base = 0;
  std::shared_ptr<InvIndex> inv;
  std::shared_ptr<const RangeIdx> rng;
  bool raw = false;
  int64_t raw_min = 0, raw_max = 0;
  pgpu::FxRange fx;
  bool fx_known = false;
};

struct StarTreeDev {
  int32_t num_dims = 0, num_nodes = 0, num_docs = 0;
  std::vector<int32_t> dim_cols, dim_bits;
  std::vector<pgpu_agg> metrics;
  void* d_block = nullptr;
  int64_t bytes = 0;
  const int32_t* d_nodes = nullptr;
  std::vector<const uint32_t*> d_dim_fwd;
  std::vector<const double*> d_mf;
  std::vector<const int64_t*> d_mc;
  std::vector<uint8_t> mf_narrow, mc_narrow;
  std::vector<pgpu::FxRange> mf_fx;
  int dim_of(int col) const {
    for (int d = 0; d < num_dims; ++d) if (dim_cols[d] == col) return d;
    return -1;
  }
  int pair(int fn, int col) const {
    for (size_t m = 0; m < metrics.size(); ++m)
      if (metrics[m].fn == fn && (fn == PGPU_AGG_COUNT || metrics[m].column == col)) return (int)m;
    return -1;
  }
};

struct Segment {
  int64_t handle = 0;
  int32_t num_docs = 0;
  void* d_block = nullptr;
  std::vector<Column> cols;
  std::array<std::unique_ptr<Column>, PGPU_GROUP_EXPR_MAX_PER_TABLE> derived;
  Column& col(int c) { return is_group_expr_col(c) ? *derived[c - kGroupExprBase] : cols[c]; }
  const Column& col(int c) const { return is_group_expr_col(c) ? *derived[c - kGroupExprBase] : cols[c]; }
  std::unique_ptr<StarTreeDev> star;
  Segment() = default;
  Segment(const Segment&) = delete;
  Segment& operator=(const Segment&) = delete;
  ~Segment() {
    for (auto& c : cols) {
      if (c.d_key) hipFree(c.d_key);
      if (c.d_val) hipFree(c.d_val);
    }
    for (auto& d : derived) {
      if (!d) continue;
      if (d->d_fwd) hipFree(d->d_fwd);
      if (d->d_key) hipFree(d->d_key);
      if (d->d_val) hipFree(d->d_val);
    }
    if (d_block) hipFree(d_block);
    if (star && star->d_block) hipFree(star->d_block);
  }
};

struct PlanRefs {
  std::vector<std::shared_ptr<Segment>> segs;
  std::vector<std::shared_ptr<DevMem>> luts;
};
struct ValMap {
  const int64_t* keys = nullptr;
  const double* vals = nullptr;
  int32_t ngaps = 0;
  std::array<uint32_t, kMaxValueGaps> gaps{};
};
struct KeyLut {
  const int32_t* lut = nullptr;
  int32_t off = 0;
};

struct DeviceImage {
  std::mutex mu;
  std::atomic<bool> uploaded{false};
  bool ready = false;
  hipEvent_t built = nullptr;
  DevBuf segrec, sets, tile_seg;
  ~DeviceImage() {
    if (built) hipEventDestroy(built);
    segrec.release();
    sets.release();
    tile_seg.release();
  }
};

struct Scratch {
  DevBuf docbits, bittasks, bitblocks;
  DevBuf rawtasks;
  HostPinned rawstage;
  DevBuf exprtasks;
  HostPinned exprstage;
  DevBuf segrec, sets, slab, table, hash_keys, stats, ckeys, cslots, counter, bitmap, tile_seg, starrec, starwork;
  DevBuf part_start, block_off, rec_key, rec_val;
  DevBuf rec_key32;
  DevBuf stage_keys;
  DevBuf coarse_fill, fine_fill, mid_key, mid_val;
  DevBuf leap_maps, mask_jobs, leaf_masks;
  DevBuf xcursor;
  DevBuf xsend, xrecv, xshard;
  DevBuf hsort;
  DevBuf part_mm;
  DevBuf dc_bits;
  DevBuf dc_recv;
  HostPinned xstage;
  HostPinned stage, readback, starstage, bitstage, maskstage;
  std::vector<uint8_t> starrec_sent;
  hipEvent_t ev[4] = {nullptr, nullptr, nullptr, nullptr};
  std::vector<hipEvent_t> cev;
  hipEvent_t busy = nullptr;
  bool abandoned = false;
  std::shared_ptr<DeviceImage> image;
  size_t footprint() const {
    size_t n = 0;
    for (const DevBuf* b : {&docbits, &bittasks, &bitblocks, &rawtasks, &exprtasks, &segrec, &sets, &slab, &table, &hash_keys,
                            &stats, &ckeys, &cslots, &counter, &bitmap, &tile_seg, &starrec, &starwork, &part_start,
                            &block_off, &rec_key, &rec_val, &rec_key32, &stage_keys, &coarse_fill, &fine_fill,
                            &mid_key, &mid_val, &leap_maps, &mask_jobs, &leaf_masks, &hsort, &part_mm, &dc_bits, &dc_recv})
      n += b->cap;
    return n;
  }
  void release() {
    if (busy) { hipEventDestroy(busy); busy = nullptr; }
    abandoned = false;
    for (auto& e : cev) if (e) hipEventDestroy(e);
    cev.clear();
    docbits.release(); bittasks.release(); bitblocks.release(); rawtasks.release(); rawstage.release();
    exprtasks.release(); exprstage.release();
    segrec.release(); tile_seg.release(); sets.release(); slab.release(); table.release(); hash_keys.release(); stats.release();
    ckeys.release(); cslots.release(); counter.release(); bitmap.release(); stage.release(); readback.release();
    starrec.release();
    starrec_sent.clear();
    starstage.release();
    bitstage.release();
    starwork.release();
    part_start.release(); block_off.release(); rec_key.release(); rec_val.release(); stage_keys.release();
    coarse_fill.release(); fine_fill.release(); mid_key.release(); mid_val.release();
    leap_maps.release(); mask_jobs.release(); leaf_masks.release(); maskstage.release();
    xcursor.release(); xstage.release(); xsend.release(); xrecv.release(); xshard.release(); hsort.release(); part_mm.release();
    dc_bits.release();
    dc_recv.release();
    for (auto& e : ev) if (e) { hipEventDestroy(e); e = nullptr; }
  }
};

struct GenScratch {
  DevBuf pos, presence, code_to_pos, cdf, pos_to_id;
};


}

using namespace pgpu;

inline pgpu_config default_config() {
  pgpu_config c;
  memset(&c, 0, sizeof c);
  c.struct_size = (int32_t)sizeof(pgpu_config);
  c.plan_cache = 1;
  c.partitioned_group_by = 1;
  c.hash_partitions = 1;
  c.hash_partition_bits = 14;
  c.hash_partition_lds_kb = 0;
  c.lds_table_kb = 112;
  c.plan_chunk_segments = 4096;
  c.stream_chunks = 1;
  c.compact_results = 1;
  c.star_tree_workgroups = 0;
  c.dense_selectivity = 0.25;
  c.slot_weight_step = 0.11;
  return c;
}

struct pgpu_table_s {
  int device = 0;
  mutable std::mutex cfg_mu;
  pgpu_config cfg = default_config();
  std::vector<std::string> names;
  std::vector<int32_t> types;
  std::mutex mu;
  struct Expr {
    pgpu::ExprProg prog;
    std::vector<pgpu::ExprOpIn> ops;
    std::string name;
    int32_t type = PGPU_DOUBLE;
  };
  std::vector<Expr> exprs;
  using GroupExpr = Expr;
  std::vector<GroupExpr> gexprs;
  int col_slot(int c) const { return is_group_expr_col(c) ? (int)names.size() + (c - kGroupExprBase) : c; }
  bool has_dict_col(int c) const {
    return c >= 0 && (c < (int)names.size() || (is_group_expr_col(c) && c - kGroupExprBase < (int)gexprs.size()));
  }
  int32_t col_type(int c) const { return types[col_slot(c)]; }
  std::shared_ptr<const Dict>& col_global(int c) { return global[col_slot(c)]; }
  uint64_t& col_global_version(int c) { return global_version[col_slot(c)]; }
  const std::string& col_name(int c) const { return is_group_expr_col(c) ? gexprs[c - kGroupExprBase].name : names[c]; }
  std::unordered_map<int64_t, std::shared_ptr<Segment>> segments;
  std::vector<std::shared_ptr<Segment>> by_handle;
  int64_t next_handle = 1;
  std::vector<std::shared_ptr<const Dict>> global;
  std::vector<uint64_t> global_version;
  struct GlobalValues {
    uint64_t version = ~0ull;
    std::shared_ptr<DevMem> keys, vals;
    int64_t n = 0;
  };
  std::vector<GlobalValues> gvalues;
  GlobalValues& col_gvalues(int c) { return gvalues[col_slot(c)]; }
  struct DeviceDict {
    uint64_t version = ~0ull;
    std::shared_ptr<DevMem> blob, offsets;
    int64_t n = 0, bytes = 0, bad_value = -1;
    bool too_large = false;
  };
  std::vector<DeviceDict> ddicts;
  hipStream_t stream = nullptr;
  std::vector<std::unique_ptr<Scratch>> scratch_pool;
  GenScratch gen;
  std::shared_ptr<ResultPool> result_pool = std::make_shared<ResultPool>();
  int64_t device_bytes = 0;
  int num_cus = 256;
  std::atomic<int> scans_inflight{0};
  uint32_t* d_docid_fwd = nullptr;
  int64_t* d_docid_key = nullptr;
  int docid_bits = 0;
  int64_t docid_n = 0;
  std::vector<void*> retired;
  std::atomic<uint64_t> version{1};
  std::mutex cache_mu;
  std::list<std::pair<std::string, std::shared_ptr<pgpu_plan_s>>> plan_cache;
  std::mutex clock_mu;
  hipStream_t clock_stream = nullptr;
  uint64_t* clock_pinned = nullptr;
  double clock_rate_khz = 0;
  double clock_host_us = 0;
  uint64_t clock_ticks = 0;
  double clock_steady_us = -1;
};


namespace pgpu {
struct LeafHost {
  int32_t kind = LEAF_NONE, negate = 0;
  uint32_t lo = 0, span = 0;
  uint32_t dict_lo = 0, dict_span = 0;
  std::vector<uint32_t> set;
  std::vector<int32_t> inv_ids;
  std::vector<int64_t> raw;
  double inv_frac = 0;
};

enum Tri { T_NONE = 0, T_ALL = 1, T_VAR = 2 };

struct LaunchChunk {
  int64_t rec_begin = 0, num_recs = 0, tile_begin = 0, num_tiles = 0;
  int64_t fix_begin = 0, fix_end = 0, set_begin = 0, set_end = 0;
};

struct StreamExec {
// ... 37 lines not shown
  int mode = MODE_LDS;
  std::vector<int32_t> slot_kind, slot_col, slot_tcol;
  bool fx = false, fx_part = false, fx_agreed = false;
  std::vector<int32_t> slot_fx;
  std::vector<pgpu::FxFormat> slot_fmt;
  std::vector<Segment*> fx_scope;
  std::vector<pgpu::FxAgree> fx_ranges;
  struct Distinct {
    int32_t slot = 0, tcol = 0, qcol = 0;
    int64_t card = 0, words = 0;
    std::shared_ptr<const Dict> dict;
  };
  std::vector<Distinct> dc;
  std::vector<int32_t> slot_dc;
  std::vector<KeyLut> dc_lut;
  struct Percentile { int32_t slot = 0, hist = 0, p_e4 = 0; };
  struct Hist {
    int32_t tcol = 0, qcol = 0, dc_slot = -1;
    int64_t card = 0, stride = 0;
    std::shared_ptr<const Dict> dict;
    std::shared_ptr<DevMem> values;
  };
  std::vector<Percentile> pct;
  std::vector<Hist> hist;
  std::vector<int32_t> slot_pct;
  std::vector<KeyLut> hist_lut;
  bool side_slot(size_t s) const { return slot_dc[s] >= 0 || slot_pct[s] >= 0; }
  struct PlanExpr {
    int32_t vcol = 0;
    pgpu::ExprProg prog;
  };
  std::vector<PlanExpr> exprs;
  std::vector<int32_t> slot_expr;
  void slot_value_cols(size_t s, std::vector<int32_t>* out) const {
    out->clear();
    if (slot_expr[s] >= 0) {
      const pgpu::ExprProg& g = exprs[slot_expr[s]].prog;
      out->assign(g.col, g.col + g.ncols);
    } else if (slot_tcol[s] >= 0) {
      out->push_back(slot_tcol[s]);
    }
  }
  std::vector<int32_t> agg_fn, agg_slot, agg_col;
  int num_projected = 0;
  std::vector<uint8_t> segrec;
  int seg_stride = 0;
  std::vector<uint32_t> set_words;
  std::vector<std::pair<int64_t, int64_t>> set_fix;
  bool no_inverted = false;
  int64_t docbit_words = 0;
  std::vector<std::pair<int64_t, int64_t>> bit_fix;
  std::vector<KBitTask> bit_tasks;
  std::vector<KBitBlock> bit_blocks;
  std::vector<KRawTask> raw_tasks;
  std::vector<int64_t> raw_vals;
  std::vector<pgpu::ExprProg> leaf_exprs;
  std::vector<KExprLeafTask> expr_tasks;
  std::vector<int64_t> expr_vals;
  bool expr_leaf(int l) const { return (size_t)l < leaf_exprs.size() && leaf_exprs[l].ncols > 0; }
  std::vector<std::shared_ptr<InvIndex>> inv_refs;
  std::shared_ptr<DeviceImage> image;
  int64_t num_tiles = 0;
  int tile_shift = 0;
  int64_t total_docs = 0;
  int64_t scanned_entries_model = 0;
  bool in_kernel_stats = false;
  bool any_leap2 = false;
  bool leap_reserved = false;
  int64_t leap_tiles = 0;
  struct ScanLaunch {
    int64_t tiles = 0;
    int grid = 0, tile_chunks = 0, slot_n = 0;
    uint16_t slot_w[kMaxCuSlots] = {};
    bool alone = false, declined = false;
  } last_scan;
  struct GenericStat { int64_t rec; int32_t num_docs; StatTree tree; int64_t out_word; };
  std::vector<GenericStat> generic;
  int64_t generic_words = 0;
  std::vector<int> leaf_perm;
  int64_t post_exempt_docs = 0;
  int segments_matched_filter = 0;
  int64_t leaf_kinds[kLeafKinds] = {};
  int64_t regex_stats[4] = {};
  std::vector<uint8_t> seg_scanned;
  int grid = 0;
  size_t lds_bytes = 0;
  ScanVariant variant = kScanSparse;
  bool dense = false;
  bool gathers = false;
  bool fast_wide = false;
  bool partitioned = false;
  std::vector<LaunchChunk> chunks;
  int launches_done = 0;
  int64_t set_words_bound = 0;
  int64_t tile_bound = 0;
  int part_shift = 0, num_parts = 0, part_grid = 0;
  int part_grid_staged[2] = {0, 0};
  size_t part_lds = 0;
  std::vector<int32_t> stream_col, stream_f64, slot_stream;
  bool part_val32 = false;
  bool part_hash = false, part_hash_live = false;
  int part_pbits = 0, part_sbits = 0;
  int64_t part_pack_min = 0, part_pack_range = -1;
  double sel_estimate = 1.0;
  int64_t sel_docs = 0;
  Scratch* scratch = nullptr;
  hipStream_t last_stream = nullptr;
  bool executed = false;
  bool timed = false;
  bool inflight_counted = false;
  bool alone = false;
  bool comm_dense = false;
  bool k8d_counts = false;
  const void* d_table_used = nullptr;
  bool hash = false;
  int64_t num_groups_limit = 0;
  bool limit_sensitive = false;
  int64_t end_time_ms = 0;
  int64_t exec_start_ms = 0;
  int cancel = 0;
  std::vector<int32_t> stage_end;
  std::vector<int64_t> stage_cap, stage_mult, stage_space;
  unsigned long long* d_stats = nullptr;
  std::vector<int64_t> xchg_counts;
  int64_t merged_records = -1;
  int64_t group_bound = 0;
  std::shared_ptr<std::atomic<int64_t>> groups_seen;
  int32_t pack_slot = -1;
  int pack_shift = kLdsPackShift;
  const void* shard = nullptr;
  int64_t shard_begin = 0, shard_count = 0;
  std::vector<int32_t> slot_kind_planned;
  std::shared_ptr<pgpu::Comm> comm_used;
  bool first_doc_slot = false;
  bool composite = false;
  bool pql_cap = false;
  struct Part {
    std::shared_ptr<pgpu_plan_s> plan;
    std::vector<int32_t> seg_index;
    bool first_seen = false;
    bool truncate = false;
  };
  std::vector<Part> parts;
  std::vector<KStarSeg> star;
  std::vector<std::tuple<int, int, int64_t>> star_match_fix;
  std::vector<int64_t> star_work_off;
  int64_t star_work_bytes = 0;
  int star_chunks = 1;
  int star_batches = 0;
  int32_t star_range_cache = 0;
  size_t star_lds_bytes = 0;
  int32_t star_cache_ints = 0;
  int64_t star_segments = 0;
  int64_t star_metric_bytes = -1;
  int64_t star_docs_read = 0;
};

inline bool plan_has_fx(const pgpu_plan_s* P) {
  if (P->fx) return true;
  for (const auto& part : P->parts)
    if (part.plan && part.plan->fx) return true;
  return false;
}
inline bool plan_fx_local(const pgpu_plan_s* P) { return !P->fx_agreed && plan_has_fx(P); }
inline bool result_has_fx(const pgpu_result_s* r) {
  for (const pgpu::FxFormat& f : r->agg_fx)
// ... 192 lines not shown
```

### pinot_amd/csrc/rt_decls.h

```cpp
#pragma once
#include "regex_dfa.h"
#include "rt.h"

namespace pgpu {

void crash_trace_handler(int sig, siginfo_t* si, void* uc);
bool diag(const char* word);
void install_crash_trace();
extern thread_local std::string g_err;
bool trace_on();
double now_us();
int fail(int code, const char* fmt, ...);

int parse_dictionary(int type, const pgpu_column_buffers& cb, Dict* d);
bool dbl_less(double a, double b);
bool merge_dict(std::shared_ptr<const Dict>& g, const Dict& src);
int64_t global_index_of(const Dict& g, const Dict& local, size_t i);
int ensure_lut(pgpu_table_s* t, Segment& s, int col, hipStream_t stream);
int ensure_values(pgpu_table_s* t, Segment& s, int col, hipStream_t stream);
int ensure_global_values(pgpu_table_s* t, int col, hipStream_t stream);
int ensure_value_map(pgpu_table_s* t, Segment& s, int col);
int ensure_docid(pgpu_table_s* t, int64_t n, hipStream_t stream);
int check_expr_segment(const pgpu_table_s* t, const Segment& s, const ExprProg& prog, bool long_result, const char* what);
int ensure_derived(pgpu_table_s* t, Segment& s, int col, hipStream_t stream);
int segment_column(pgpu_table_s* t, Segment& s, int col, const Column** out);
int table_reader_dict(pgpu_table_s* t, int col);
void account_unpin(pgpu_table_s* t, const Segment* s);
int64_t padded_fwd_words(int64_t num_docs, int bits);
int64_t lz4_decode_block(const uint8_t* src, int64_t n, uint8_t* dst, int64_t cap);
int decode_raw_forward_index(int type, const uint8_t* b, int64_t n, int32_t num_docs, int c, RawValues* out);
int parse_raw_column(int type, const pgpu_column_buffers& cb, int32_t num_docs, int c, Column* col, RawValues* out);
int64_t register_segment(pgpu_table_s* t, std::unique_ptr<Segment> seg_in);

int regex_check(const char* pattern, int32_t* states, int32_t* classes, int64_t* table_bytes);
int regex_match_host(const char* pattern, const uint8_t* value, int64_t len, int32_t* matched);
int regex_check_column(const pgpu_table_s* t, const std::vector<Segment*>& segs, int col);
int regex_compile_pattern(const char* pattern, RegexDfa* d);
struct RegexJob {
  RegexDfa dfa;
  int col = -1;
  std::string name;
  std::shared_ptr<DevMem> blob, offsets;
  int64_t n = 0, dict_bytes = 0;
  std::vector<KRegexSetTask> tasks;
  std::vector<std::shared_ptr<DevMem>> luts;
  int64_t out_words = 0;
  int32_t max_card = 0, affine = 0;
  std::vector<std::vector<uint32_t>> sets;
};
int regex_job_snapshot(pgpu_table_s* t, const std::vector<Segment*>& segs, int col, RegexJob* job);
int regex_job_run(pgpu_table_s* t, RegexJob* job, uint64_t* global_out);
int regex_global_ids(pgpu_table_s* t, int col, const char* pattern, uint64_t* bitmap, int64_t words);

int64_t hash_capacity(int64_t groups);
Scratch* acquire_scratch(pgpu_table_s* t);
void release_scratch(pgpu_table_s* t, Scratch* s);
bool parse_literal(int type, const char* lit, bool allow_star, Literal* out);
int insertion_index(const Column& c, const Literal& v);
int parse_predicate(int type, const pgpu_predicate& p, ParsedPred* out);
void to_inverted_leaf(const Column& c, const pgpu_predicate& p, const Segment& s, LeafHost* L);
int translate_predicate(const Column& c, const pgpu_predicate& p, const ParsedPred& pp, LeafHost* L,
                        std::vector<int>& ids);
int translate_predicate_dict(const Column& c, const pgpu_predicate& p, const ParsedPred& pp, LeafHost* L,
                             std::vector<int>& ids);
void translate_raw_predicate(int type, const pgpu_predicate& p, const ParsedPred& pp, LeafHost* L);
double estimate_selectivity(const std::vector<int32_t>& ops, const std::vector<double>& leaf);
Tri fold_program(const std::vector<int32_t>& ops, const std::vector<Tri>& leaf);
bool star_composites(const std::vector<int32_t>& ops, const pgpu_query* q, std::vector<std::vector<int>>* out);
void leaf_bitset(const LeafHost& L, int32_t card, std::vector<uint32_t>& w);
int plan_star_segment(pgpu_plan_s* P, size_t seg_index, Segment* s, const pgpu_query* q,
                      const std::vector<std::vector<int>>& comps, const std::vector<LeafHost>& leaves, bool* used);
SegStats classify_segment_stats(const pgpu_plan_s* P, uint64_t sig);
bool column_int_ends(const Column& c, int64_t* lo, int64_t* hi);
struct IntRange {
  int64_t lo = INT64_MAX, hi = INT64_MIN;
  bool known = true;
};
IntRange int_column_range(const std::vector<Segment*>& segs, int col);
bool int_sum_fits(const std::vector<Segment*>& segs, int col);
long double int_sum_bound(const std::vector<Segment*>& segs, int col);
FxRange fx_operand_range(pgpu_table_s* t, const std::vector<Segment*>& segs, const pgpu_query* q, int tcol, int64_t* docs);
int query_fp_sum_ranges(pgpu_table_s* t, const std::vector<Segment*>& segs, const pgpu_query* q, FxAgree* out);
int32_t pack_slot_for(const pgpu_table_s* t, const pgpu_plan_s* P, const pgpu_query* q, int64_t max_count,
                      int shift);
int32_t lds_pack_slot(const pgpu_table_s* t, const pgpu_plan_s* P, const pgpu_query* q, int64_t G);
int32_t hash_pack_slot(const pgpu_table_s* t, const pgpu_plan_s* P, const pgpu_query* q, int* shift);
bool part_hash_eligible(const pgpu_plan_s* P, int64_t G);
bool dense_part_eligible(const pgpu_plan_s* P, int nslots, int64_t G);
bool part_eligible(const pgpu_plan_s* P, int nslots, int64_t G);
void hash_part_bits(const pgpu_config& cfg, int64_t groups, int nslots, int* pbits, int* sbits);
int part_coarse_shift(int num_parts);
int part_coarse_runs(int num_parts);
bool part_pass_shape(pgpu_plan_s* P, int64_t parts, int64_t tiles);
void hash_part_resize(pgpu_plan_s* P, int64_t groups);
int64_t part_hash_out_cap(const pgpu_plan_s* P);
int part_hash_overflow(const pgpu_plan_s* P, uint64_t groups);

int plan_create_impl(pgpu_table_s* t, const int64_t* handles, int32_t nsegs, const pgpu_query* q, pgpu_plan_s* P,
                     const StreamExec* se = nullptr);

int timeout_fail(const pgpu_plan_s* P);
int abandon_scratch(Scratch* sc, hipStream_t stream);
bool cancelled(const pgpu_plan_s* P);
int wait_plan(pgpu_plan_s* P, hipStream_t stream);
int launch_raw_leaves(const pgpu_plan_s* P, Scratch* sc, hipStream_t stream);
int launch_expr_leaves(const pgpu_plan_s* P, Scratch* sc, hipStream_t stream);
int exec_prologue(pgpu_plan_s* P, hipStream_t stream, void* d_table, int max_chunks, ExecCtx& X);
int exec_upload_chunk(pgpu_plan_s* P, hipStream_t stream, const ExecCtx& X, const LaunchChunk& C);
bool check_launch_on();
bool set_slot_weights(KParams& kp, int grid, int num_cus, double step, int64_t max_run);
void inflight_end(pgpu_plan_s* P);
int exec_launch_chunk(pgpu_plan_s* P, hipStream_t stream, ExecCtx& X, const LaunchChunk& C, int c);
int exec_epilogue(pgpu_plan_s* P, hipStream_t stream, ExecCtx& X);
int plan_execute_impl(pgpu_plan_s* P, hipStream_t stream, void* d_table);

// ... 15 lines not shown
```

### pinot_amd/csrc/rt_dict.cpp

```cpp
#include "derive.h"
#include "group_expr.h"
#include "rt_decls.h"

namespace pgpu {

int parse_dictionary(int type, const pgpu_column_buffers& cb, Dict* d) {
  d->type = type;
  const int64_t card = cb.cardinality;
  if (card < 0) return fail(PGPU_ERR_INVALID_ARGUMENT, "negative cardinality");
  const int w = cb.entry_width;
  if (card > 0 && (!cb.dict || cb.dict_len < card * (int64_t)w))
    return fail(PGPU_ERR_INVALID_ARGUMENT, "dictionary buffer too small (%lld < %lld x %d)", (long long)cb.dict_len,
                (long long)card, w);
  switch (type) {
    case PGPU_INT:
      if (w != 4) return fail(PGPU_ERR_INVALID_ARGUMENT, "INT dictionary entry width %d", w);
      d->iv.resize(card);
      for (int64_t i = 0; i < card; ++i) d->iv[i] = (int32_t)rd_be32(cb.dict + i * 4);
      break;
    case PGPU_LONG:
      if (w != 8) return fail(PGPU_ERR_INVALID_ARGUMENT, "LONG dictionary entry width %d", w);
      d->iv.resize(card);
      for (int64_t i = 0; i < card; ++i) d->iv[i] = (int64_t)rd_be64(cb.dict + i * 8);
      break;
// ... 285 lines not shown
  std::vector<uint32_t> used((size_t)ncand, 0u);
  if (ncand > 0) {
    HIP_TRY(hipMalloc(&d_scratch.p, (size_t)s.num_docs * 4));
    HIP_TRY(hipMalloc(&d_used.p, (size_t)ncand * 4));
    HIP_TRY(hipMemcpyAsync(d_keys.p, cand.data(), (size_t)ncand * 8, hipMemcpyHostToDevice, stream));
    HIP_TRY(hipMemsetAsync(d_used.p, 0, (size_t)ncand * 4, stream));
    ev.mark(2, stream);
    if (launch_derive_ids(T, reinterpret_cast<const int64_t*>(d_keys.p), ncand, reinterpret_cast<uint32_t*>(d_scratch.p),
                          reinterpret_cast<uint32_t*>(d_used.p), stream))
      return fail(PGPU_ERR_DEVICE, "derive ids launch failed: %s", hipGetErrorString(hipGetLastError()));
    ev.mark(3, stream);
    HIP_TRY(hipMemcpyAsync(used.data(), d_used.p, (size_t)ncand * 4, hipMemcpyDeviceToHost, stream));
    HIP_TRY(hipStreamSynchronize(stream));
  }
  GroupExprDict gd = group_expr_compact(cand, used, ge.type);
  auto col_out = std::make_unique<Column>();
  Column& d = *col_out;
  d.card = gd.card;
  d.bits = gd.bits;
  d.entry_width = gd.entry_width;
  d.dict.type = ge.type;
  d.dict.iv = std::move(gd.iv);
  d.dict.dv = std::move(gd.dv);
  d.raw_dict = std::move(gd.bytes);
  d.fwd_bytes = ((int64_t)s.num_docs * d.bits + 7) / 8;
  d.fwd_words = padded_fwd_words(s.num_docs, d.bits);
  void* fwd = nullptr;
  HIP_TRY(hipMalloc(&fwd, (size_t)d.fwd_words * 4));
  d.d_fwd = reinterpret_cast<uint32_t*>(fwd);
  struct FreeFwd {
    Column* c;
    ~FreeFwd() { if (c && c->d_fwd) hipFree(c->d_fwd); }
  } free_fwd{&d};
  if (ncand > 0) {
    HIP_TRY(hipMalloc(&d_remap.p, (size_t)ncand * 4));
    HIP_TRY(hipMemcpyAsync(d_remap.p, gd.remap.data(), (size_t)ncand * 4, hipMemcpyHostToDevice, stream));
    ev.mark(4, stream);
    if (launch_derive_pack(reinterpret_cast<const uint32_t*>(d_scratch.p), reinterpret_cast<const int32_t*>(d_remap.p),
                           s.num_docs, d.bits, d.d_fwd, d.fwd_words, stream))
      return fail(PGPU_ERR_DEVICE, "derive pack launch failed: %s", hipGetErrorString(hipGetLastError()));
    ev.mark(5, stream);
  } else {
    HIP_TRY(hipMemsetAsync(d.d_fwd, 0, (size_t)d.fwd_words * 4, stream));
  }
  HIP_TRY(hipStreamSynchronize(stream));
  free_fwd.c = nullptr;
  if (timed && ncand > 0)
    fprintf(stderr, "[pgpu] derive %s segment %lld docs %d candidates %lld unique %d card %d bits %d fwd_bytes %lld: "
            "candidates_us %.1f ids_us %.1f pack_us %.1f build_us %.1f\n", ge.name.c_str(), (long long)s.handle, s.num_docs,
            (long long)product, ncand, d.card, d.bits, (long long)d.fwd_words * 4, ev.us(0), ev.us(2), ev.us(4),
            now_us() - t_begin);
  t->device_bytes += d.fwd_words * 4;
  if (merge_dict(t->col_global(col), d.dict)) {
    t->col_global_version(col)++;
    t->version++;
    plan_cache_clear(t);
  }
  s.derived[k] = std::move(col_out);
  return 0;
}

int segment_column(pgpu_table_s* t, Segment& s, int col, const Column** out) {
  if (is_group_expr_col(col)) {
    TRY(ensure_derived(t, s, col, t->stream));
    *out = &s.col(col);
    return 0;
  }
  if (col < 0 || col >= (int)s.cols.size()) return fail(PGPU_ERR_INVALID_ARGUMENT, "bad column");
  *out = &s.cols[col];
  return 0;
}

int table_reader_dict(pgpu_table_s* t, int col) {
  if (!t->has_dict_col(col)) return fail(PGPU_ERR_INVALID_ARGUMENT, "bad arguments");
  if (is_group_expr_col(col))
    for (auto& hs : t->segments) TRY(ensure_derived(t, *hs.second, col, t->stream));
  return 0;
}

void account_unpin(pgpu_table_s* t, const Segment* s) {
  int64_t fwd_words = 0;
  for (const auto& c : s->cols) {
    if (c.inv) t->device_bytes -= c.inv->bytes;
    t->device_bytes -= (c.lut ? 4 * std::max(c.card, 1) : 0) +
                       (c.d_key ? 16 * (c.raw ? raw_padded_docs(s->num_docs) : std::max(c.card, 1)) : 0);
    if (!c.raw) fwd_words += (c.fwd_words + 63) & ~int64_t(63);
  }
  for (const auto& d : s->derived)
    if (d)
      t->device_bytes -= d->fwd_words * 4 + (d->lut ? 4 * std::max(d->card, 1) : 0) + (d->d_key ? 16 * std::max(d->card, 1) : 0);
  if (s->d_block) t->device_bytes -= std::max<int64_t>(fwd_words, 64) * 4;
  if (s->star) t->device_bytes -= s->star->bytes;
}

int64_t padded_fwd_words(int64_t num_docs, int bits) {
  return ((num_docs + kTileDocs - 1) / kTileDocs) * (int64_t)kBlock * bits + kFwdPadWords;
}

int64_t lz4_decode_block(const uint8_t* src, int64_t n, uint8_t* dst, int64_t cap) {
  const uint8_t* ip = src;
  const uint8_t* const iend = src + n;
  uint8_t* op = dst;
  uint8_t* const oend = dst + cap;
  auto ext_len = [&](int64_t& len) -> bool {
    uint32_t b;
    do {
      if (ip >= iend) return false;
      b = *ip++;
      len += b;
    } while (b == 255);
    return true;
  };
  while (ip < iend) {
    const uint32_t token = *ip++;
    int64_t lit = token >> 4;
    if (lit == 15 && !ext_len(lit)) return -1;
    if (lit > iend - ip || lit > oend - op) return -1;
    memcpy(op, ip, (size_t)lit);
    ip += lit;
    op += lit;
    if (ip == iend) return op - dst;
    if (iend - ip < 2) return -1;
    const int64_t off = (int64_t)ip[0] | ((int64_t)ip[1] << 8);
    ip += 2;
    int64_t ml = token & 15;
    if (ml == 15 && !ext_len(ml)) return -1;
    ml += 4;
    if (off == 0 || off > op - dst || ml > oend - op) return -1;
    const uint8_t* m = op - off;
    if (off >= ml) {
      memcpy(op, m, (size_t)ml);
      op += ml;
    } else {
      for (int64_t k = 0; k < ml; ++k) op[k] = m[k];
      op += ml;
    }
  }
  return -1;
}

int decode_raw_forward_index(int type, const uint8_t* b, int64_t n, int32_t num_docs, int c, RawValues* out) {
  if (type == PGPU_STRING) return fail(PGPU_ERR_UNSUPPORTED, "column %d: raw STRING columns are not on the GPU path", c);
  if (!b || n < 16) return fail(PGPU_ERR_INVALID_ARGUMENT, "column %d: raw forward index too short", c);
  const int32_t version = (int32_t)rd_be32(b), num_chunks = (int32_t)rd_be32(b + 4);
  const int32_t per_chunk = (int32_t)rd_be32(b + 8), size = (int32_t)rd_be32(b + 12);
  if (version != 2 && version != 3)
    return fail(PGPU_ERR_UNSUPPORTED, "column %d: raw forward index version %d (2 and 3 are read)", c, version);
  if (n < 28) return fail(PGPU_ERR_INVALID_ARGUMENT, "column %d: raw forward index header truncated", c);
  const int32_t total = (int32_t)rd_be32(b + 16), compression = (int32_t)rd_be32(b + 20);
  const int32_t header_start = (int32_t)rd_be32(b + 24);
  if (compression != 0 && compression != 3 && compression != 4)
    return fail(PGPU_ERR_UNSUPPORTED, "column %d: raw chunk compression type %d (PASS_THROUGH, LZ4 and "
                "LZ4_LENGTH_PREFIXED are read)", c, compression);
  const int want = (type == PGPU_INT || type == PGPU_FLOAT) ? 4 : 8;
  if (size != want) return fail(PGPU_ERR_INVALID_ARGUMENT, "column %d: raw entry size %d, type needs %d", c, size, want);
  if (num_chunks < 0 || per_chunk <= 0 || total < num_docs || (int64_t)num_chunks * per_chunk < num_docs)
    return fail(PGPU_ERR_INVALID_ARGUMENT, "column %d: raw forward index covers %d docs, segment has %d", c, total,
                num_docs);
  const int entry = version == 2 ? 4 : 8;
  const int64_t data = (int64_t)header_start + (int64_t)num_chunks * entry;
  if (header_start < 28 || data > n || (compression == 0 && data + (int64_t)num_docs * size > n))
    return fail(PGPU_ERR_INVALID_ARGUMENT, "column %d: raw forward index too short for %d docs", c, num_docs);
  const int64_t chunk_bytes = compression ? std::min<int64_t>(per_chunk, total) * size : 0;
  if (compression && chunk_bytes > (n - data) * 256 + 64)
    return fail(PGPU_ERR_INVALID_ARGUMENT, "column %d: raw chunk of %d docs cannot come from a %lld-byte index", c,
                per_chunk, (long long)n);
// ... 84 lines not shown
```

### pinot_amd/csrc/rt_plan_create.cpp

```cpp
#include "expr_leaf.h"
#include "rt_decls.h"

namespace pgpu {
namespace {

struct PlanCtx {
  pgpu_table_s* t;
  const pgpu_query* q;
  pgpu_plan_s* P;
  const StreamExec* se;
  int64_t G = 1;
  int nslots = 0;
  bool any_raw_leaf = false;
  std::vector<int64_t> gcard;
  std::vector<ParsedPred> parsed;
  std::vector<std::vector<int>> star_comps;
  bool star_allowed = false, exempt_kind = false, minmax_kind = false, any_star = false, any_inv = false;
  std::vector<int> qcol_key;
  std::vector<char> qcol_val;
  std::vector<int> qcol_dc;
  std::vector<int> qcol_hist;
  std::vector<int> perm;
  std::vector<RegexJob> regex;
  double t_start = 0, tr[8] = {0};
  int ntr = 0;
  void mark() { if (trace_on() && ntr < 8) tr[ntr++] = now_us(); }
};

struct Chunk {
  bool gathers = false;
  std::vector<uint8_t> rec;
  std::vector<uint32_t> set_words;
  std::vector<std::pair<int64_t, int64_t>> set_fix;
  std::vector<std::pair<int64_t, int64_t>> bit_fix;
  std::vector<KBitTask> bit_tasks;
  std::vector<KBitBlock> bit_blocks;
  std::vector<KRawTask> raw_tasks;
  std::vector<int64_t> raw_vals;
  std::vector<KExprLeafTask> expr_tasks;
  std::vector<int64_t> expr_vals;
  std::vector<std::shared_ptr<InvIndex>> inv_refs;
  std::vector<pgpu_plan_s::GenericStat> generic;
  bool any_leap2 = false;
  int64_t docbit_words = 0;
  std::vector<uint8_t> scanned;
  int64_t tiles = 0, entries = 0, matched = 0, sel_docs = 0, exempt = 0;
  int64_t leaf_kinds[kLeafKinds] = {};
  double sel = 1.0;
  int rc = 0;
  std::string err;
};

int query_col(pgpu_plan_s* P, int col) {
  for (size_t i = 0; i < P->query_cols.size(); ++i)
    if (P->query_cols[i] == col) return (int)i;
  P->query_cols.push_back(col);
  return (int)P->query_cols.size() - 1;
}

const Column& pred_column(const pgpu_plan_s* P, const Segment* s, const pgpu_query* q, int l) {
  static const Column kNoColumn;
  return P->expr_leaf(l) ? kNoColumn : s->cols[q->predicates[l].column];
}

bool regex_leaf(const pgpu_query* q, int l) { return q->predicates[l].type == PGPU_PRED_REGEXP_LIKE; }

int acquire_segments(PlanCtx& cx, const int64_t* handles, int32_t nsegs) {
  pgpu_table_s* t = cx.t;
  pgpu_plan_s* P = cx.P;
  P->refs = std::make_shared<PlanRefs>();
  std::lock_guard<std::mutex> g(t->mu);
  P->segs.reserve(nsegs);
  P->refs->segs.reserve(nsegs);
  for (int i = 0; i < nsegs; ++i) {
    const int64_t h = handles[i];
    const std::shared_ptr<Segment>* sp = h > 0 && h < (int64_t)t->by_handle.size() ? &t->by_handle[h] : nullptr;
    if (!sp || !*sp) return fail(PGPU_ERR_NOT_FOUND, "unknown segment handle %lld", (long long)h);
    P->segs.push_back(sp->get());
    P->refs->segs.push_back(*sp);
  }
  return 0;
}

int table_expr_prog(pgpu_table_s* t, int vcol, const char* what, ExprProg* out) {
  std::lock_guard<std::mutex> g(t->mu);
  const int e = vcol - (int)t->names.size();
  if (e < 0 || e >= (int)t->exprs.size()) return fail(PGPU_ERR_INVALID_ARGUMENT, "%s: bad column %d", what, vcol);
  *out = t->exprs[e].prog;
  return 0;
}

int bind_expr_leaf(PlanCtx& cx, int i, int vcol) {
  ExprProg& prog = cx.P->leaf_exprs[i];
  const std::string what = "predicate " + std::to_string(i);
  TRY(table_expr_prog(cx.t, vcol, what.c_str(), &prog));
  for (const Segment* s : cx.P->segs) TRY(check_expr_segment(cx.t, *s, prog, false, (what + ": expression").c_str()));
  cx.any_raw_leaf = true;
  return 0;
}

int bind_group_expr(PlanCtx& cx, int i, int gcol) {
  pgpu_table_s* t = cx.t;
  pgpu_plan_s* P = cx.P;
  if (cx.se && cx.se->d_table) return fail(PGPU_ERR_UNSUPPORTED, "a GROUP BY expression with an external table");
  std::lock_guard<std::mutex> g(t->mu);
  if (!t->has_dict_col(gcol)) return fail(PGPU_ERR_INVALID_ARGUMENT, "group-by %d: bad column %d", i, gcol);
  for (Segment* s : P->segs) TRY(ensure_derived(t, *s, gcol, t->stream));
  const ExprProg& prog = t->gexprs[gcol - kGroupExprBase].prog;
  P->group_exprs.push_back({gcol, std::vector<int32_t>(prog.col, prog.col + prog.ncols)});
  return 0;
}

int bind_query_columns(PlanCtx& cx) {
  const pgpu_query* q = cx.q;
  pgpu_plan_s* P = cx.P;
  const int ncols = (int)cx.t->names.size();
  for (int i = 0; i < q->num_predicates; ++i) {
    if (!regex_leaf(q, i)) continue;
    const pgpu_predicate& pr = q->predicates[i];
    if (pr.num_values != 1 || !pr.values || !pr.values[0])
      return fail(PGPU_ERR_INVALID_ARGUMENT, "REGEXP_LIKE predicate %d takes one value, the pattern", i);
    TRY(regex_check_column(cx.t, P->segs, pr.column));
    if (cx.regex.empty()) cx.regex.resize(q->num_predicates);
    TRY(regex_compile_pattern(pr.values[0], &cx.regex[i].dfa));
  }
  for (int i = 0; i < q->num_predicates; ++i)
    if (q->predicates[i].column >= ncols) { P->leaf_exprs.assign(q->num_predicates, ExprProg{}); break; }
  for (int i = 0; i < q->num_predicates; ++i) {
    const int c = q->predicates[i].column;
    if (c >= ncols) {
// ... 835 lines not shown
    const LeafHost& lh = leaves[l];
    C.entries += s->cols[q->predicates[l].column].rng->partial_entries(lh.lo, (int64_t)lh.lo + lh.span - 1);
  }
  if (ss.kind == STATS_GENERIC)
    C.generic.push_back({(int64_t)(C.rec.size() / P->seg_stride), s->num_docs, ss.tree, 0});
  return ss.rec_stats;
}

void estimate_chunk_selectivity(const PlanCtx& cx, const Segment* s, const std::vector<LeafHost>& leaves, Chunk& C) {
  const pgpu_plan_s* P = cx.P;
  std::vector<double> frac(P->num_leaves, 1.0);
  for (int l = 0; l < P->num_leaves; ++l) {
    const LeafHost& lh = leaves[l];
    const double card = std::max(1, pred_column(P, s, cx.q, l).card);
    double f = lh.kind == LEAF_ALL ? 1.0 : lh.kind == LEAF_NONE ? 0.0 : lh.kind == LEAF_RANGE ? lh.span / card : 0.0;
    if (lh.kind == LEAF_DOCRANGE) f = (double)lh.span / std::max(1, s->num_docs);
    if (lh.kind == LEAF_BITMAP) f = lh.inv_frac;
    if (lh.kind == LEAF_RAW_RANGE || lh.kind == LEAF_RAW_IN) f = 0.5;
    if (lh.kind == LEAF_EXPR_RANGE || lh.kind == LEAF_EXPR_IN) f = 0.5;
    if (regex_leaf(cx.q, l)) f = 0.5;
    else if (lh.kind == LEAF_SET) {
      int64_t ones = 0;
      for (uint32_t w : lh.set) ones += __builtin_popcount(w);
      f = ones / card;
    }
    frac[l] = lh.negate ? 1.0 - f : f;
  }
  C.sel = P->num_leaves ? estimate_selectivity(P->ops, frac) : 1.0;
  C.sel_docs = s->num_docs;
}

bool fill_kcols(const PlanCtx& cx, size_t i, KCol* kc) {
  const pgpu_plan_s* P = cx.P;
  const Segment* s = P->segs[i];
  const int nqc = (int)P->query_cols.size();
  bool gathers = false;
  for (int j = 0; j < nqc; ++j) {
    const int tc = P->query_cols[j];
    const Column* c = tc == kDocIdColumn ? nullptr : &s->col(tc);
    if (!c || c->raw) {
      kc[j].fwd = P->docid_fwd;
      kc[j].lut = nullptr;
      kc[j].dkey = c ? c->d_key : P->docid_key;
      kc[j].dval = c ? c->d_val : nullptr;
      kc[j].bits = P->docid_bits;
    } else {
      kc[j].fwd = c->d_fwd;
      kc[j].bits = c->bits;
      if (cx.qcol_key[j] >= 0) {
        const KeyLut& kl = P->key_lut[i * P->key_cols.size() + cx.qcol_key[j]];
        kc[j].lut = kl.lut;
        kc[j].lut_off = kl.off;
      } else if (cx.qcol_dc[j] >= 0) {
        const KeyLut& kl = P->dc_lut[i * P->dc.size() + cx.qcol_dc[j]];
        kc[j].lut = kl.lut;
        kc[j].lut_off = kl.off;
      } else if (cx.qcol_hist[j] >= 0) {
        const KeyLut& kl = P->hist_lut[i * P->hist.size() + cx.qcol_hist[j]];
        kc[j].lut = kl.lut;
        kc[j].lut_off = kl.off;
      }
      if (cx.qcol_val[j]) {
        kc[j].dkey = c->key_affine ? nullptr : c->d_key;
        kc[j].key_base = c->key_base;
        kc[j].dval = c->d_val;
        for (size_t v = 0; v < P->val_cols.size(); ++v) {
          if (P->val_cols[v] != tc) continue;
          const ValMap& vm = P->val_map[i * P->val_cols.size() + v];
          if (vm.keys) {
            kc[j].dkey = vm.keys;
            kc[j].dval = vm.vals;
            kc[j].ngaps = vm.ngaps;
            std::copy(vm.gaps.begin(), vm.gaps.end(), kc[j].gaps);
          }
        }
      }
    }
    gathers |= ((cx.qcol_key[j] >= 0 || cx.qcol_dc[j] >= 0 || cx.qcol_hist[j] >= 0) && kc[j].lut != nullptr) ||
               (cx.qcol_val[j] && kc[j].dkey != nullptr);
  }
  return gathers || !P->exprs.empty();
}

void emit_set_words(Chunk& C, const LeafHost& lh, int64_t field) {
  C.set_fix.emplace_back(field, (int64_t)C.set_words.size());
  C.set_words.insert(C.set_words.end(), lh.set.begin(), lh.set.end());
  if (C.set_words.size() & 1) C.set_words.push_back(0);
}

void emit_raw_task(Chunk& C, const Segment* s, const Column& col, const LeafHost& lh, KLeaf& kl, int64_t field) {
  C.bit_fix.emplace_back(field, C.docbit_words);
  KRawTask rt;
  memset(&rt, 0, sizeof rt);
  rt.keys = col.d_key;
  rt.dst = C.docbit_words;
  rt.num_docs = s->num_docs;
  rt.kind = lh.kind;
  rt.negate = lh.negate;
  if (lh.kind == LEAF_RAW_RANGE) {
    rt.lo = lh.raw[0];
    rt.hi = lh.raw[1];
  } else {
    rt.lo = (int64_t)C.raw_vals.size();
    rt.hi = (int64_t)lh.raw.size();
    C.raw_vals.insert(C.raw_vals.end(), lh.raw.begin(), lh.raw.end());
  }
  C.raw_tasks.push_back(rt);
  C.docbit_words += ((((int64_t)s->num_docs + 31) / 32) + 1) & ~int64_t(1);
  kl.kind = LEAF_BITMAP;
  kl.negate = 0;
}

void emit_expr_task(Chunk& C, const Segment* s, const ExprProg& prog, const LeafHost& lh, KLeaf& kl, int64_t field) {
  C.bit_fix.emplace_back(field, C.docbit_words);
  C.expr_tasks.push_back(make_expr_leaf_task(prog, expr_operands(*s, prog), s->num_docs, lh.kind == LEAF_EXPR_IN, lh.raw,
                                             lh.negate, C.docbit_words, 0, &C.expr_vals));
  C.docbit_words += leaf_region_words(s->num_docs);
  kl.kind = LEAF_BITMAP;
  kl.negate = 0;
}

bool emit_bitdir(Chunk& C, const Segment* s, const Column& col, const LeafHost& lh, KLeaf& kl, int64_t field) {
  const InvIndex& inv = *col.inv;
  const InvIndex::Entry& e = inv.ids[lh.inv_ids[0]];
  auto payload = [&](const InvIndex::Cont& ct) {
    return reinterpret_cast<uint64_t>(reinterpret_cast<const uint32_t*>(inv.d_block) + ct.word);
  };
  for (int32_t ci = e.begin; ci < e.begin + e.count; ++ci) {
    const InvIndex::Cont& ct = inv.conts[ci];
    if (ct.type != CONT_BITMAP && !(ct.type == CONT_ARRAY && ct.n >= 0 && ct.n < 65536 && (payload(ct) >> 47) == 0))
      return false;
  }
  const int64_t nblk = ((int64_t)s->num_docs + 65535) >> 16;
  std::vector<uint64_t> dir((size_t)nblk, 0);
  for (int32_t ci = e.begin; ci < e.begin + e.count; ++ci) {
    const InvIndex::Cont& ct = inv.conts[ci];
    if (ct.key < 0 || ct.key >= nblk) continue;
    const uint64_t a = payload(ct);
    dir[ct.key] = ct.type == CONT_BITMAP ? a : (ct.n > 0 ? (a | 1ull | ((uint64_t)ct.n << 48)) : 0);
  }
  C.inv_refs.push_back(col.inv);
  C.set_fix.emplace_back(field, (int64_t)C.set_words.size());
  for (uint64_t d : dir) {
    C.set_words.push_back((uint32_t)d);
    C.set_words.push_back((uint32_t)(d >> 32));
  }
  kl.kind = LEAF_BITDIR;
  return true;
}

void emit_bitmap_tasks(Chunk& C, const Segment* s, const Column& col, const LeafHost& lh, int64_t field) {
  const InvIndex& inv = *col.inv;
  C.inv_refs.push_back(col.inv);
  C.bit_fix.emplace_back(field, C.docbit_words);
  const int64_t nblk = ((int64_t)s->num_docs + 65535) >> 16;
  const size_t t0 = C.bit_tasks.size();
  for (int32_t id : lh.inv_ids) {
    const InvIndex::Entry& e = inv.ids[id];
    for (int32_t ci = e.begin; ci < e.begin + e.count; ++ci) {
      const InvIndex::Cont& ct = inv.conts[ci];
      KBitTask task;
      task.payload = reinterpret_cast<const uint32_t*>(inv.d_block) + ct.word;
      task.type = ct.type;
      task.n = ct.n;
      task.dst = C.docbit_words + (int64_t)ct.key * kContainerWords;
      C.bit_tasks.push_back(task);
    }
  }
  if (lh.inv_ids.size() > 1)
    std::stable_sort(C.bit_tasks.begin() + t0, C.bit_tasks.end(),
                     [](const KBitTask& x, const KBitTask& y) { return x.dst < y.dst; });
  size_t ti = t0;
  for (int64_t kb = 0; kb < nblk; ++kb) {
    KBitBlock blk;
    blk.dst = C.docbit_words + kb * kContainerWords;
    blk.task_begin = (int32_t)ti;
    while (ti < C.bit_tasks.size() && C.bit_tasks[ti].dst == blk.dst) ++ti;
    blk.num_tasks = (int32_t)(ti - blk.task_begin);
    C.bit_blocks.push_back(blk);
  }
  C.docbit_words += nblk * kContainerWords;
}

void emit_leaves(const PlanCtx& cx, const Segment* s, const std::vector<LeafHost>& leaves, KLeaf* kl, int64_t kl_off,
                 Chunk& C) {
  for (int k = 0; k < cx.P->num_leaves; ++k) {
    const LeafHost& lh = leaves[cx.perm[k]];
    const Column& col = pred_column(cx.P, s, cx.q, cx.perm[k]);
    const int64_t field = kl_off + (int64_t)(k * sizeof(KLeaf) + offsetof(KLeaf, set));
    kl[k].kind = lh.kind;
    kl[k].negate = lh.negate;
    kl[k].lo = lh.lo;
    kl[k].span = lh.span;
    kl[k].set = nullptr;
    if (lh.kind == LEAF_SET) emit_set_words(C, lh, field);
    if (lh.kind == LEAF_RAW_RANGE || lh.kind == LEAF_RAW_IN) emit_raw_task(C, s, col, lh, kl[k], field);
    if (lh.kind == LEAF_EXPR_RANGE || lh.kind == LEAF_EXPR_IN)
      emit_expr_task(C, s, cx.P->leaf_exprs[cx.perm[k]], lh, kl[k], field);
    const bool bitdir = lh.kind == LEAF_BITMAP && lh.inv_ids.size() == 1 && emit_bitdir(C, s, col, lh, kl[k], field);
    if (kl[k].kind >= 0 && kl[k].kind < kLeafKinds) C.leaf_kinds[kl[k].kind]++;
    if (lh.kind == LEAF_BITMAP && !bitdir) emit_bitmap_tasks(C, s, col, lh, field);
  }
}

int plan_range(const PlanCtx& cx, size_t b, size_t e, Chunk& C) {
  const pgpu_plan_s* P = cx.P;
  const int nqc = (int)P->query_cols.size();
  std::vector<LeafHost> leaves(P->num_leaves);
  std::vector<Tri> tri(P->num_leaves);
  std::vector<int> ids_scratch;
  std::vector<uint8_t> rec(P->seg_stride);
  std::unordered_map<uint64_t, SegStats> stat_cache;
  for (size_t i = b; i < e; ++i) {
    Segment* s = P->segs[i];
    Tri whole;
    TRY(translate_leaves(cx, i, leaves, tri, ids_scratch, &whole));
    C.scanned.push_back(0);
    if (whole == T_NONE || s->num_docs == 0) continue;
    C.scanned.back() = 1;
    C.matched++;
    if (cx.exempt_kind && whole == T_ALL && !raw_minmax(cx, s)) C.exempt += s->num_docs;
    if (cx.star_allowed && s->star) {
      bool used = false;
      TRY(plan_star_segment(cx.P, i, s, cx.q, cx.star_comps, leaves, &used));
      if (used) continue;
    }
    const int32_t rec_stats = segment_stats(cx, s, leaves, tri, stat_cache, C);
    if (C.sel_docs == 0) estimate_chunk_selectivity(cx, s, leaves, C);
    std::fill(rec.begin(), rec.end(), 0);
    KSegHdr* h = reinterpret_cast<KSegHdr*>(rec.data());
    h->num_docs = s->num_docs;
    h->tile_base = (int32_t)C.tiles;
    h->num_tiles = (int32_t)((s->num_docs + kTileDocs - 1) / kTileDocs);
    h->stats = rec_stats;
    C.gathers |= fill_kcols(cx, i, reinterpret_cast<KCol*>(rec.data() + sizeof(KSegHdr)));
    const size_t kl_at = sizeof(KSegHdr) + sizeof(KCol) * nqc;
    emit_leaves(cx, s, leaves, reinterpret_cast<KLeaf*>(rec.data() + kl_at), (int64_t)(C.rec.size() + kl_at), C);
    C.rec.insert(C.rec.end(), rec.begin(), rec.end());
    C.tiles += h->num_tiles;
  }
  return 0;
}

void configure_star(PlanCtx& cx) {
  pgpu_plan_s* P = cx.P;
  P->star_segments = (int64_t)P->star.size();
  if (P->star.empty()) return;
  if (P->star_cache_ints < 0) P->star_cache_ints = 0;
  int64_t max_nodes = 0;
  for (const KStarSeg& k : P->star) max_nodes = std::max<int64_t>(max_nodes, k.num_nodes);
  P->star_range_cache = max_nodes * 16 <= 32 * 1024 ? (int32_t)max_nodes : 0;
  const int64_t nseg_launch = std::min<int64_t>((int64_t)P->star.size(), kStarMaxSegs);
  P->star_batches = (int)(((int64_t)P->star.size() + kStarMaxSegs - 1) / kStarMaxSegs);
  const int64_t rc = P->star_range_cache;
  const size_t table_bytes = P->mode == MODE_LDS ? (size_t)((cx.nslots * cx.G + 1) & ~int64_t(1)) * 8 : 0;
  P->star_lds_bytes = table_bytes + (size_t)((nseg_launch + 2) & ~int64_t(1)) * 8 + (size_t)((rc + 2) & ~int64_t(1)) * 8 +
                      (size_t)((2 * rc + 3) & ~int64_t(3)) * 4 + (size_t)P->star_cache_ints * 4;
  const int64_t per_cu = P->mode == MODE_LDS ? std::max<int64_t>(1, std::min<int64_t>(2, (160 * 1024) /
                                                  std::max<size_t>(P->star_lds_bytes, 1))) : 8;
  const int64_t want = P->cfg.star_tree_workgroups;
  P->star_chunks = (int)(want > 0 ? want : (int64_t)cx.t->num_cus * per_cu);
}

void configure_scan_grid(PlanCtx& cx, int64_t tile_base) {
  pgpu_table_s* t = cx.t;
  pgpu_plan_s* P = cx.P;
  P->dense = P->mode != MODE_HASH && P->sel_estimate >= P->cfg.dense_selectivity;
  bool f64 = false;
  for (int k : P->slot_kind) f64 |= k == SLOT_SUM_F64;
  const bool dense_simple = P->dense && !P->gathers && !f64 && !P->fx && P->dc.empty() && P->tile_bound == 0;
  const bool pair = !P->dense && P->pure_and && P->num_leaves == 2 && P->leaf_kinds[LEAF_BITDIR] > 0;
  const bool fast = !P->dense && !pair && P->pure_and && P->num_leaves <= kFastLeaves;
  P->fast_wide = fast && P->sel_estimate >= 1.0 / 16;
  P->variant = !P->exprs.empty() ? (P->dense ? kScanExprDense : kScanExprSparse)
               : !P->pct.empty() ? (P->dense ? kScanHistDense : kScanHistSparse)
               : !P->dc.empty() ? (P->dense ? kScanDcDense : kScanDcSparse)
               : P->fx        ? (P->dense ? kScanFxDense : kScanFxSparse)
               : dense_simple ? kScanDenseSimple
// ... 72 lines not shown
    return;
  const bool hash_part = part_hash_eligible(P, cx.G);
  int shift = 16;
  while (shift > 8 && ((int64_t)nslots << shift) * 8 > kPartLds) --shift;
  int64_t parts = (cx.G + (int64_t(1) << shift) - 1) >> shift;
  int pbits = 0, sbits = 0;
  if (hash_part) {
    hash_part_bits(P->cfg, P->group_bound, nslots, &pbits, &sbits);
    shift = 0;
    parts = int64_t(1) << pbits;
  }
  std::vector<int32_t> scol, sf64, sstream;
  partition_streams(P, &scol, &sf64, &sstream);
  const int64_t rec_bytes = P->total_docs * ((hash_part ? 4 : 2) + 8 * (int64_t)scol.size());
  if (parts > kMaxParts || rec_bytes > kPartMaxRecordBytes || (hash_part && (int)scol.size() > kHashPartStreams) ||
      !part_pass_shape(P, parts, tile_base))
    return;
  P->partitioned = true;
  P->part_hash = hash_part;
  if (hash_part) P->pack_slot = -1;
  P->part_pbits = pbits;
  P->part_sbits = sbits;
  P->part_shift = shift;
  P->num_parts = (int)parts;
  P->stream_col = scol;
  P->stream_f64 = sf64;
  P->slot_stream = sstream;
  partition_value_widths(P);
}

int configure(PlanCtx& cx, int64_t tile_base) {
  cx.P->num_tiles = tile_base;
  if (tile_base > INT32_MAX) return fail(PGPU_ERR_UNSUPPORTED, "too many tiles in one plan");
  configure_star(cx);
  configure_scan_grid(cx, tile_base);
  reserve_leap2(cx, tile_base);
  configure_partitions(cx, tile_base);
  return 0;
}

void merge_chunk(pgpu_plan_s* P, Chunk& C, int64_t tile_shift) {
  if (P->set_words.size() & 1) P->set_words.push_back(0);
  const int64_t rec0 = (int64_t)P->segrec.size(), set0 = (int64_t)P->set_words.size();
  if (tile_shift)
    for (size_t r = 0; r < C.rec.size(); r += P->seg_stride)
      reinterpret_cast<KSegHdr*>(C.rec.data() + r)->tile_base += (int32_t)tile_shift;
  for (auto& f : C.set_fix) P->set_fix.emplace_back(rec0 + f.first, set0 + f.second);
  for (auto& f : C.bit_fix) P->bit_fix.emplace_back(rec0 + f.first, P->docbit_words + f.second);
  for (KBitBlock blk : C.bit_blocks) {
    blk.dst += P->docbit_words;
    blk.task_begin += (int32_t)P->bit_tasks.size();
    P->bit_blocks.push_back(blk);
  }
  P->bit_tasks.insert(P->bit_tasks.end(), C.bit_tasks.begin(), C.bit_tasks.end());
  for (KRawTask rt : C.raw_tasks) {
    rt.dst += P->docbit_words;
    if (rt.kind == LEAF_RAW_IN) rt.lo += (int64_t)P->raw_vals.size();
    P->raw_tasks.push_back(rt);
  }
  P->raw_vals.insert(P->raw_vals.end(), C.raw_vals.begin(), C.raw_vals.end());
  for (KExprLeafTask et : C.expr_tasks) {
    et.dst += P->docbit_words;
    if (et.kind == LEAF_RAW_IN) et.lo += (int64_t)P->expr_vals.size();
    P->expr_tasks.push_back(et);
  }
  P->expr_vals.insert(P->expr_vals.end(), C.expr_vals.begin(), C.expr_vals.end());
  P->inv_refs.insert(P->inv_refs.end(), C.inv_refs.begin(), C.inv_refs.end());
  for (auto& g : C.generic) {
    g.rec += rec0 / std::max(P->seg_stride, 1);
    g.out_word = P->generic_words;
    P->generic_words += (int64_t)P->num_leaves * (((int64_t)g.num_docs + 31) / 32);
    P->generic.push_back(std::move(g));
  }
  P->any_leap2 |= C.any_leap2;
  P->gathers |= C.gathers;
  P->docbit_words += C.docbit_words;
  P->segrec.insert(P->segrec.end(), C.rec.begin(), C.rec.end());
  P->set_words.insert(P->set_words.end(), C.set_words.begin(), C.set_words.end());
  P->seg_scanned.insert(P->seg_scanned.end(), C.scanned.begin(), C.scanned.end());
  P->segments_matched_filter += C.matched;
  P->scanned_entries_model += C.entries;
  P->post_exempt_docs += C.exempt;
  for (int k = 0; k < kLeafKinds; ++k) P->leaf_kinds[k] += C.leaf_kinds[k];
  if (P->sel_docs == 0 && C.sel_docs) { P->sel_estimate = C.sel; P->sel_docs = C.sel_docs; }
}

int run_streamed(PlanCtx& cx, int stream_chunks) {
  const pgpu_query* q = cx.q;
  pgpu_plan_s* P = cx.P;
  const StreamExec* se = cx.se;
  const size_t nseg = P->segs.size();
  for (Segment* s : P->segs) {
    P->tile_bound += (s->num_docs + kTileDocs - 1) / kTileDocs;
    for (int l = 0; l < P->num_leaves; ++l) {
      const int ty = q->predicates[l].type;
      if (ty == PGPU_PRED_IN || ty == PGPU_PRED_NOT_IN || ty == PGPU_PRED_REGEXP_LIKE)
        P->set_words_bound += ((int64_t)pred_column(P, s, q, l).card + 31) / 32;
    }
  }
  if (!P->scratch) return fail(PGPU_ERR_INVALID_ARGUMENT, "streamed plan without scratch");
  ExecCtx X;
  int64_t tile_off = 0;
  cx.mark();
  for (int c = 0; c < stream_chunks; ++c) {
    Chunk C;
    C.rec.reserve((nseg / stream_chunks + 1) * (size_t)P->seg_stride);
    TRY(plan_range(cx, nseg * c / stream_chunks, nseg * (c + 1) / stream_chunks, C));
    LaunchChunk L;
    L.rec_begin = (int64_t)(P->segrec.size() / P->seg_stride);
    L.fix_begin = (int64_t)P->set_fix.size();
    L.set_begin = (int64_t)P->set_words.size();
    L.tile_begin = tile_off;
    merge_chunk(P, C, 0);
    L.num_recs = (int64_t)(P->segrec.size() / P->seg_stride) - L.rec_begin;
    L.fix_end = (int64_t)P->set_fix.size();
    L.set_end = (int64_t)P->set_words.size();
    L.num_tiles = C.tiles;
    tile_off += C.tiles;
    P->chunks.push_back(L);
    if (c == 0) {
      TRY(configure(cx, P->tile_bound));
      TRY(exec_prologue(P, se->stream, se->d_table, stream_chunks, X));
    }
    TRY(exec_upload_chunk(P, se->stream, X, L));
    TRY(exec_launch_chunk(P, se->stream, X, L, c));
  }
  cx.mark();
  P->num_tiles = tile_off;
  TRY(exec_epilogue(P, se->stream, X));
  if (trace_on())
    fprintf(stderr, "[pgpu] plan_create (streamed, %d launches): %.1f us (%zu segments)\n", stream_chunks,
            now_us() - cx.t_start, P->segs.size());
  return 0;
}

int64_t split_small_tiles(PlanCtx& cx, int64_t tile_base) {
  pgpu_plan_s* P = cx.P;
  if (tile_base <= 0 || tile_base >= 2 * (int64_t)cx.t->num_cus || P->any_leap2 || !P->star.empty() ||
      dense_part_eligible(P, cx.nslots, cx.G))
    return tile_base;
  int sh = 1;
  while (sh < 2 && (tile_base << sh) < 2 * (int64_t)cx.t->num_cus) ++sh;
  P->tile_shift = sh;
  for (size_t r = 0; r + sizeof(KSegHdr) <= P->segrec.size(); r += P->seg_stride) {
    KSegHdr* h = reinterpret_cast<KSegHdr*>(P->segrec.data() + r);
    h->tile_base <<= sh;
    h->num_tiles <<= sh;
  }
  return tile_base << sh;
}

int run_pooled(PlanCtx& cx) {
  pgpu_plan_s* P = cx.P;
  const size_t nseg = P->segs.size();
  const int nchunks = cx.any_star ? 1 : (int)std::min<size_t>(host_pool().size() + 1, (nseg + plan_chunk_segs(P->cfg) - 1) / plan_chunk_segs(P->cfg));
  std::vector<Chunk> chunks(std::max(nchunks, 1));
  auto run_chunk = [&](int c) {
    Chunk& C = chunks[c];
    C.rec.reserve((nseg / chunks.size() + 1) * (size_t)P->seg_stride);
    C.rc = plan_range(cx, nseg * c / chunks.size(), nseg * (c + 1) / chunks.size(), C);
    if (C.rc) C.err = g_err;
  };
  cx.mark();
  if (chunks.size() == 1) run_chunk(0);
  else host_pool().run((int)chunks.size(), run_chunk);
  cx.mark();
  int64_t tile_base = 0;
  for (Chunk& C : chunks) {
    if (C.rc) return fail(C.rc, "%s", C.err.c_str());
    merge_chunk(P, C, tile_base);
    tile_base += C.tiles;
  }
  TRY(configure(cx, split_small_tiles(cx, tile_base)));
  P->chunks.assign(1, LaunchChunk{0, (int64_t)(P->segrec.size() / std::max(P->seg_stride, 1)), 0, P->num_tiles, 0,
                                  (int64_t)P->set_fix.size(), 0, (int64_t)P->set_words.size()});
  if (trace_on())
    fprintf(stderr, "[pgpu] plan_create: %.1f us (%zu segments; setup %.1f, ensure %.1f, translate %.1f, rest %.1f)\n",
            now_us() - cx.t_start, P->segs.size(), cx.tr[0] - cx.t_start, cx.tr[1] - cx.tr[0], cx.tr[2] - cx.tr[1],
            now_us() - cx.tr[2]);
  return 0;
}

}

int plan_create_impl(pgpu_table_s* t, const int64_t* handles, int32_t nsegs, const pgpu_query* q, pgpu_plan_s* P,
                     const StreamExec* se) {
  if (!q) return fail(PGPU_ERR_INVALID_ARGUMENT, "null query");
  PlanCtx cx{t, q, P, se};
  cx.t_start = trace_on() ? now_us() : 0;
  P->cfg = table_config(t);
  if (q->num_group_by < 0) return fail(PGPU_ERR_INVALID_ARGUMENT, "negative group-by count");
  if (q->num_group_by > kMaxKeys) return fail(PGPU_ERR_UNSUPPORTED, "more than %d group-by columns", kMaxKeys);
  if (q->num_predicates > kMaxLeaves) return fail(PGPU_ERR_UNSUPPORTED, "more than %d predicates", kMaxLeaves);
  if (q->num_filter_ops > kMaxOps) return fail(PGPU_ERR_UNSUPPORTED, "filter program longer than %d", kMaxOps);
  P->table = t;
  P->end_time_ms = q->end_time_ms;
  TRY(acquire_segments(cx, handles, nsegs));
  TRY(bind_query_columns(cx));
  TRY(compile_filter(q, &P->ops, &P->pure_and, &P->max_depth));
  TRY(assign_slots(cx));
  note_groups_limit(cx);
  TRY(build_device_arrays(cx));
  TRY(run_regex_leaves(cx));
  std::vector<int64_t> kspan;
  TRY(restrict_key_space(cx, &kspan));
  TRY(layout_keys(cx, kspan));
  choose_table_mode(cx);
  TRY(check_distinct_shape(cx));
  TRY(prepare_translation(cx));
  order_leaves(cx);
  const bool partitions = part_eligible(P, cx.nslots, cx.G);
  P->in_kernel_stats = P->pure_and && P->num_leaves <= kFastLeaves && !partitions;
  const int stream_chunks = se ? stream_chunk_count(P->cfg, P->segs.size()) : 1;
  if (se && !cx.any_star && !cx.any_inv && !cx.any_raw_leaf && !partitions && stream_chunks > 1)
    return run_streamed(cx, stream_chunks);
  return run_pooled(cx);
}

}
```

### pinot_amd/executor.py

```python
import ctypes
import time

import numpy as np

from . import _lib as L
from .query import QueryContext


class ExecutionStatistics:

    def __init__(self, stats6):
        (self.num_docs_scanned, self.num_entries_scanned_in_filter, self.num_entries_scanned_post_filter,
         self.num_total_docs, self.num_segments_processed, self.num_segments_matched) = [int(x) for x in stats6]

    def as_tuple(self):
        return (self.num_docs_scanned, self.num_entries_scanned_in_filter, self.num_entries_scanned_post_filter,
                self.num_total_docs)

    def __repr__(self):
        return "ExecutionStatistics(docsScanned=%d, inFilter=%d, postFilter=%d, totalDocs=%d)" % self.as_tuple()


class AvgPair:
    __slots__ = ("sum", "count")
# ... 110 lines not shown
        L.check(lib.pgpu_result_datatable(self._holder.r, self._table.handle, buf, n.value, ctypes.byref(n)))
        return buf.raw[:n.value]


def broker_reduce_sql(datatables, query):
    import json
    lib = L.load()
    keep, spec = query.sql_trim_c()
    bufs = [ctypes.create_string_buffer(bytes(b), max(len(b), 1)) for b in datatables]
    ptrs = (ctypes.c_void_p * max(len(bufs), 1))(*[ctypes.cast(b, ctypes.c_void_p) for b in bufs])
    lens = np.array([len(b) for b in datatables] or [0], dtype=np.int64)
    n = ctypes.c_int64()
    L.check(lib.pgpu_broker_reduce_sql(ptrs, L.ptr(lens, ctypes.c_int64), len(bufs), ctypes.byref(spec), None, 0,
                                       ctypes.byref(n)))
    out = ctypes.create_string_buffer(n.value + 1)
    L.check(lib.pgpu_broker_reduce_sql(ptrs, L.ptr(lens, ctypes.c_int64), len(bufs), ctypes.byref(spec), out,
                                       n.value + 1, ctypes.byref(n)))
    return json.loads(out.value.decode("utf-8"))


def aggregation_defaults(aggregations):
    out = []
    for fn, _ in aggregations:
        if fn.startswith("PERCENTILE"):
            out.append(float("-inf"))
            continue
        out.append({"COUNT": 0, "SUM": 0.0, "MIN": float("inf"), "MAX": float("-inf"), "DISTINCTCOUNT": 0}.get(fn, None)
                   if fn != "AVG" else AvgPair(0.0, 0))
    return out


class AggregationResult:

    def __init__(self, values, stats):
        self.values = values
        self.stats = stats

    def __repr__(self):
        return "AggregationResult(%r, %r)" % (self.values, self.stats)


def _key_str(x):
    if isinstance(x, float):
        return repr(x)
    return str(x)


class GpuTable:
    def __init__(self, schema, device=0, config=None):
        self.lib = L.load()
        self.names = [n for n, _ in schema]
        self.types = [L.TYPE_NAMES[t] if isinstance(t, str) else int(t) for _, t in schema]
        self.index = {n: i for i, n in enumerate(self.names)}
        self.device = device
        names = (ctypes.c_char_p * len(self.names))(*[n.encode() for n in self.names])
        types = (ctypes.c_int32 * len(self.types))(*self.types)
        h = ctypes.c_void_p()
        L.check(self.lib.pgpu_table_create(device, len(self.names), names, types, ctypes.byref(h)))
        self.handle = h
        self._dict_cache = {}
        self._snapshots = {}
        self.group_types = {}
        if config:
            self.set_config(**config)

    def config(self):
        c = L.ConfigC()
        L.check(self.lib.pgpu_table_get_config(self.handle, ctypes.byref(c)))
        return {f: getattr(c, f) for f in L.CONFIG_FIELDS}

    def set_config(self, **fields):
        cur = self.config()
        bad = set(fields) - set(cur)
        if bad:
            raise ValueError("unknown config fields: %s" % sorted(bad))
        cur.update(fields)
        c = L.ConfigC(ctypes.sizeof(L.ConfigC), **cur)
        L.check(self.lib.pgpu_table_set_config(self.handle, ctypes.byref(c)))

    def reset_config(self):
        c = L.ConfigC()
        L.check(self.lib.pgpu_config_default(ctypes.byref(c)))
        L.check(self.lib.pgpu_table_set_config(self.handle, ctypes.byref(c)))

    def close(self):
        if self.handle:
            self.lib.pgpu_table_destroy(self.handle)
            self.handle = None

    def __del__(self):
        try:
            self.close()
        except Exception:
            pass

    def __enter__(self):
        return self

    def __exit__(self, *a):
        self.close()

    def add_expression(self, ops, name=None):
        arr = (L.ExprOpC * max(len(ops), 1))()
        for i, (op, col, lit) in enumerate(ops):
            arr[i].op, arr[i].column, arr[i].literal = int(op), int(col), float(lit)
        out = ctypes.c_int32()
        L.check(self.lib.pgpu_table_add_expression(self.handle, arr, len(ops), name.encode() if name else None,
                                                   ctypes.byref(out)))
        return out.value

    def add_group_expression(self, ops, result_type, name=None):
        arr = (L.ExprOpC * max(len(ops), 1))()
        for i, (op, col, lit) in enumerate(ops):
            arr[i].op, arr[i].column, arr[i].literal = int(op), int(col), float(lit)
        rt = L.TYPE_NAMES[result_type] if isinstance(result_type, str) else int(result_type)
        out = ctypes.c_int32()
        L.check(self.lib.pgpu_table_add_group_expression(self.handle, arr, len(ops), name.encode() if name else None, rt,
                                                         ctypes.byref(out)))
        return out.value

    def _expr_ops(self, tree):
        from .query import expr_columns, expr_program
        types = {n: L.TYPE_NAME_OF[t] for n, t in zip(self.names, self.types)}
        for c in expr_columns(tree):
            if c not in types:
                raise KeyError("unknown column %r" % c)
        return [(op, self.names.index(c) if c is not None else 0, lit) for op, c, lit in expr_program(tree, types)], types

    def _check_long_leaves(self, f, exprs):
        from .query import FilterContext, LONG, expr_type, long_predicate
        if f.type != FilterContext.PREDICATE:
            for k in f.children:
                self._check_long_leaves(k, exprs)
        elif f.predicate.column in exprs:
            types = {n: L.TYPE_NAME_OF[t] for n, t in zip(self.names, self.types)}
            if expr_type(exprs[f.predicate.column], types) == LONG:
                long_predicate(f.predicate)

    def expression(self, column):
        n = ctypes.c_int32()
        arr = (L.ExprOpC * L.EXPR_MAX_OPS)()
        name = ctypes.create_string_buffer(1024)
        L.check(self.lib.pgpu_table_expression(self.handle, column, arr, L.EXPR_MAX_OPS, ctypes.byref(n), name, len(name)))
        return [(arr[i].op, arr[i].column, arr[i].literal) for i in range(n.value)], name.value.decode()

    def query_c(self, query):
        exprs = query.expressions
        used = [(fn, col) for fn, col in query.aggregations]
        if query.filter is not None and exprs:
            preds = []
            query.filter.postfix(preds, [])
            used += [("WHERE", p.column) for p in preds]
        for fn, col in used:
            if col in exprs and col not in self.index and fn != "COUNT":
                ops, _ = self._expr_ops(exprs[col])
                self.index[col] = self.add_expression(ops, col)
        if query.filter is not None and exprs:
            self._check_long_leaves(query.filter, exprs)
        for col in query.group_by:
            if col in exprs and ("group", col) not in self.index:
                from .query import expr_type
                ops, types = self._expr_ops(exprs[col])
                rtype = expr_type(exprs[col], types)
                self.index[("group", col)] = self.add_group_expression(ops, rtype, col)
                self.group_types[col] = L.TYPE_NAMES[rtype]
        return query.to_c(self.index)
# ... 210 lines not shown
        out = (L.FpSumRangeC * max(na, 1))()
        L.check(self.lib.pgpu_query_fp_sum_ranges(self.handle, L.ptr(hs, ctypes.c_int64), len(hs), ctypes.byref(q), out))
        return [L.FpSumRangeC.from_tuple(out[a].as_tuple()) for a in range(na)]

    def plan(self, handles, query, fp_sum_ranges=None):
        return Plan(self, handles, query, fp_sum_ranges=fp_sum_ranges)

    def execute_groupby(self, handles, query, stream=None):
        with Plan(self, handles, query, execute=(stream, None)) as p:
            return p.finalize(stream)

    def plan_execute(self, handles, query, stream=None, d_table=None, fp_sum_ranges=None):
        if fp_sum_ranges is not None:
            p = Plan(self, handles, query, fp_sum_ranges=fp_sum_ranges)
            try:
                p.execute(stream, d_table)
            except Exception:
                p.close()
                raise
            return p
        return Plan(self, handles, query, execute=(stream, d_table))


class Plan:
    def __init__(self, table, handles, query, execute=None, fp_sum_ranges=None):
        if isinstance(query, str):
            from .query import parse_query
            query = parse_query(query, filter_expressions=True, group_by_expressions=True)
        self.table = table
        self.query = query
        self.lib = table.lib
        hs = handles if isinstance(handles, np.ndarray) and handles.dtype == np.int64 else \
            np.ascontiguousarray(list(handles), dtype=np.int64)
        q, keep = table.query_c(query)
        h = ctypes.c_void_p()
        if fp_sum_ranges is not None:
            assert execute is None, "an agreed plan is created, then executed"
            if len(fp_sum_ranges) != len(query.aggregations):
                raise ValueError("one agreed range per aggregation")
            L.check(self.lib.pgpu_plan_create_agreed(table.handle, L.ptr(hs, ctypes.c_int64), len(hs), ctypes.byref(q),
                                                     L.fp_sum_range_array(fp_sum_ranges), ctypes.byref(h)))
        elif execute is None:
            L.check(self.lib.pgpu_plan_create(table.handle, L.ptr(hs, ctypes.c_int64), len(hs), ctypes.byref(q),
                                              ctypes.byref(h)))
        else:
            stream, d_table = execute
            L.check(self.lib.pgpu_plan_create_execute(table.handle, L.ptr(hs, ctypes.c_int64), len(hs),
                                                      ctypes.byref(q), ctypes.c_void_p(stream or 0),
                                                      ctypes.c_void_p(d_table or 0), ctypes.byref(h)))
        self.handle = h
        self.num_segments = len(hs)

    def close(self):
        if self.handle:
            self.lib.pgpu_plan_destroy(self.handle)
            self.handle = None

    def __enter__(self):
        return self

    def __exit__(self, *a):
        self.close()

    def __del__(self):
        try:
            self.close()
        except Exception:
            pass

    def layout(self):
        ns, nk = ctypes.c_int32(), ctypes.c_int64()
        kinds = (ctypes.c_int32 * 32)()
        L.check(self.lib.pgpu_plan_layout(self.handle, ctypes.byref(ns), ctypes.byref(nk), kinds))
        return ns.value, nk.value, [kinds[i] for i in range(ns.value)]

    def cancel(self):
        L.check(self.lib.pgpu_plan_cancel(self.handle))

    def leaf_kinds(self):
        out = np.zeros(len(L.LEAF_KIND_NAMES), dtype=np.int64)
        L.check(self.lib.pgpu_plan_leaf_kinds(self.handle, L.ptr(out, ctypes.c_int64)))
        return {n: int(v) for n, v in zip(L.LEAF_KIND_NAMES, out) if v}

    def regexp_stats(self):
        out = np.zeros(4, dtype=np.int64)
        L.check(self.lib.pgpu_plan_regexp_stats(self.handle, L.ptr(out, ctypes.c_int64)))
        return dict(zip(("sets", "affine", "dict_bytes", "table_bytes"), (int(v) for v in out)))

    def group_path(self):
        out = ctypes.c_int32(-1)
        L.check(self.lib.pgpu_plan_group_path(self.handle, ctypes.byref(out)))
        return L.GROUP_PATH_NAMES[out.value]

    def execute(self, stream=None, d_table=None):
        L.check(self.lib.pgpu_plan_execute(self.handle, ctypes.c_void_p(stream or 0), ctypes.c_void_p(d_table or 0)))

    def scanned_segments(self):
        out = np.zeros(max(self.num_segments, 1), dtype=np.uint8)
        L.check(self.lib.pgpu_plan_scanned_segments(self.handle, L.ptr(out, ctypes.c_uint8)))
        return out[:self.num_segments].astype(bool)

    def timing_us(self):
        out = (ctypes.c_double * 4)()
        L.check(self.lib.pgpu_plan_timing(self.handle, out))
        return out[0], out[1], out[2], out[3]

    def fp_sum_format(self, agg):
        out = (ctypes.c_int32 * 4)()
        L.check(self.lib.pgpu_plan_fp_sum_format(self.handle, int(agg), out))
        return {"mode": L.FP_SUM_MODE_NAMES[out[0]], "E": out[1], "K": out[2], "W": out[3]}

    def star_metric_bytes(self):
        fn = getattr(self.lib, "pgpu_plan_star_metric_bytes", None)
        if fn is None:
            return -1
        out = ctypes.c_int64(0)
        L.check(fn(self.handle, ctypes.byref(out)))
        return out.value

    def star_work(self):
        out = (ctypes.c_int64 * 3)()
        L.check(self.lib.pgpu_plan_star_work(self.handle, out))
        return out[0], out[1], out[2]

    def scan_geometry(self):
        out = (ctypes.c_int64 * 16)()
        L.check(self.lib.pgpu_plan_scan_geometry(self.handle, out))
        return {"grid": out[0], "lds_bytes": out[1], "leap_tiles": out[2], "tiles": out[3],
                "tile_chunks": out[4], "slot_weights": tuple(out[6 + s] for s in range(out[5])),
                "longest_run": out[10], "launch_grid": out[11], "launch_tiles": out[12],
                "alone": bool(out[13]), "weights_declined": bool(out[14]), "variant": out[15]}

    def finalize(self, stream=None, d_table=None):
        r = ctypes.c_void_p()
        t0 = time.perf_counter()
        L.check(self.lib.pgpu_plan_finalize(self.handle, ctypes.c_void_p(stream or 0), ctypes.c_void_p(d_table or 0),
                                            ctypes.byref(r)))
        t1 = time.perf_counter()
        holder = _ResultHolder(self.lib, r)
        res = _decode_result(self.table, self.query, holder)
        self.finalize_us = ((t1 - t0) * 1e6, (time.perf_counter() - t1) * 1e6)
        return res

    def exchange_counts(self, stream, nparts):
        counts = np.zeros(nparts, dtype=np.int64)
        L.check(self.lib.pgpu_plan_exchange_counts(self.handle, ctypes.c_void_p(stream or 0), nparts,
                                                   L.ptr(counts, ctypes.c_int64)))
        return counts

    def exchange_export(self, stream, nparts, kinds, d_out, cap):
        k = np.ascontiguousarray(kinds, dtype=np.int32)
        L.check(self.lib.pgpu_plan_exchange_export(self.handle, ctypes.c_void_p(stream or 0), nparts,
                                                   L.ptr(k, ctypes.c_int32), ctypes.c_void_p(d_out or 0), cap))

    def exchange_merge(self, stream, kinds, d_records, n):
        k = np.ascontiguousarray(kinds, dtype=np.int32)
        L.check(self.lib.pgpu_plan_exchange_merge(self.handle, ctypes.c_void_p(stream or 0), L.ptr(k, ctypes.c_int32),
                                                  ctypes.c_void_p(d_records or 0), n))

    def finalize_range(self, stream, d_shard, key_begin, key_count):
        return _finalize_range(self, stream, d_shard, key_begin, key_count)


GpuPlan = Plan


# ... 76 lines not shown
```

Before: 1571 billion rows/s.

## Add 8-bit filter sketch columns so filter leaves read narrower forward indexes

At segment pin time, builds a per-column histogram on the GPU and picks up to 127 hot dictionary ids as singleton codes, with the gaps between them becoming range codes. It then encodes an 8-bit sketch forward index for wide columns (at least 12 bits). When a range or set predicate maps exactly onto whole codes, the filter leaf reads the narrow sketch instead of the full-width forward index, cutting the bytes filters pull from HBM. The cost is extra device memory, slower segment pinning with extra synchronisation, and per-leaf fwd/bits pointer selection in the kernel.

```diff
diff --git a/include/pinotgpu.h b/include/pinotgpu.h
--- a/include/pinotgpu.h
+++ b/include/pinotgpu.h
@@ -184,6 +184,11 @@
 int pgpu_plan_cancel(pgpu_plan plan);
 
 int pgpu_plan_leaf_kinds(pgpu_plan plan, int64_t* counts);
+
+int pgpu_table_set_filter_sketch(pgpu_table table, int32_t min_bits, double min_cover);
+int pgpu_segment_sketch_info(pgpu_table table, int64_t segment_handle, int32_t column, int32_t* ncodes,
+                             int64_t* singleton_docs, int64_t* bytes, int32_t* first_id_out, int32_t cap);
+int pgpu_plan_sketch_leaves(pgpu_plan plan, int64_t* pairs_using_sketch, int64_t* pairs_declined);
 
 int pgpu_plan_regexp_stats(pgpu_plan plan, int64_t* out4);
 int pgpu_regex_check(const char* pattern, int32_t* states, int32_t* classes, int64_t* table_bytes);
diff --git a/pinot_amd/_lib.py b/pinot_amd/_lib.py
--- a/pinot_amd/_lib.py
+++ b/pinot_amd/_lib.py
@@ -220,6 +220,9 @@
                                          ctypes.POINTER(c_voidp)]),
     "pgpu_plan_layout": (c_int, [c_voidp, c_i32p, c_i64p, c_i32p]),
     "pgpu_plan_leaf_kinds": (c_int, [c_voidp, c_i64p]),
+    "pgpu_table_set_filter_sketch": (c_int, [c_voidp, c_i32, ctypes.c_double]),
+    "pgpu_segment_sketch_info": (c_int, [c_voidp, c_i64, c_i32, c_i32p, c_i64p, c_i64p, c_i32p, c_i32]),
+    "pgpu_plan_sketch_leaves": (c_int, [c_voidp, c_i64p, c_i64p]),
     "pgpu_plan_group_path": (c_int, [c_voidp, c_i32p]),
     "pgpu_plan_regexp_stats": (c_int, [c_voidp, c_i64p]),
     "pgpu_regex_check": (c_int, [ctypes.c_char_p, c_i32p, c_i32p, c_i64p]),
diff --git a/pinot_amd/build.py b/pinot_amd/build.py
--- a/pinot_amd/build.py
+++ b/pinot_amd/build.py
@@ -8,19 +8,19 @@
 CSRC = os.path.join(HERE, "csrc")
 LIB_PATH = os.path.join(HERE, "libpinotgpu.so")
 RUNTIME = ["rt_core", "rt_dict", "rt_plan", "rt_plan_create", "rt_exec", "rt_finalize", "rt_groups", "rt_regex",
-           "abi_table", "abi_plan", "abi_combine", "abi_result"]
+           "rt_sketch", "abi_table", "abi_plan", "abi_combine", "abi_result"]
 SOURCES = [("kernels.hip", [], "kernels")] + [(n + ".cpp", [], n) for n in RUNTIME] + [("startree.cpp", [], "startree"),
            ("filter_stats.cpp", [], "filter_stats"), ("range_index.cpp", [], "range_index"), ("comm.cpp", [], "comm"), ("server_response.cpp", [], "server_response"),
            ("k_partition.hip", [], "k_partition"), ("k_partition_fx.hip", [], "k_partition_fx"),
            ("k_hashfinal.hip", [], "k_hashfinal"), ("k_derive.hip", [], "k_derive"),
-           ("regex_dfa.cpp", [], "regex_dfa"), ("k_regex.hip", [], "k_regex")] + \
+           ("regex_dfa.cpp", [], "regex_dfa"), ("k_regex.hip", [], "k_regex"), ("k_sketch.hip", [], "k_sketch")] + \
     [("k_%s.hip" % k, ["-DPGPU_FAMILY=%d" % f, "-DPGPU_MODE=%d" % m], "k_%s%s_%d" % (k, ("", "_fx", "_dc", "_hist", "_expr")[f], m))
      for k, f, modes in (("direct", 0, 3), ("startree", 0, 3), ("direct", 1, 3), ("startree", 1, 3), ("direct", 2, 2),
                          ("direct", 3, 2), ("direct", 4, 3))
      for m in range(modes)]
 HEADERS = ["internal.h", "device.h", "scan_direct.h", "host_common.h", "startree_kernels.h",
            "partition.h", "filter_stats.h", "host_result.h", "comm.h", "range_index.h", "rt.h",
-           "rt_decls.h", "tile_split.h", "fx_sum.h", "key_range.h", "expr_eval.h", "expr_leaf.h", "expr_docs.h", "derive.h", "group_expr.h", "regex_dfa.h", "scan_direct_body.inc", "part_aggregate_body.inc",
+           "rt_decls.h", "tile_split.h", "fx_sum.h", "key_range.h", "expr_eval.h", "expr_leaf.h", "expr_docs.h", "derive.h", "group_expr.h", "regex_dfa.h", "col_sketch.h", "scan_direct_body.inc", "part_aggregate_body.inc",
            "part_hash_aggregate_body.inc"]
 ARCH = os.environ.get("PGPU_OFFLOAD_ARCH", "gfx950")
 
@@ -173,6 +173,10 @@
     return _build_header_check("tile_split_check", "tile_split_check.cpp", "tile_split.h", force)
 
 
+def build_col_sketch_check(force=False):
+    return _build_header_check("col_sketch_check", "col_sketch_check.cpp", "col_sketch.h", force)
+
+
 def build_fx_sum_check(force=False):
     return _build_header_check("fx_sum_check", "fx_sum_check.cpp", "fx_sum.h", force)
 
diff --git a/pinot_amd/csrc/abi_result.cpp b/pinot_amd/csrc/abi_result.cpp
--- a/pinot_amd/csrc/abi_result.cpp
+++ b/pinot_amd/csrc/abi_result.cpp
@@ -414,6 +414,16 @@
       return fail(PGPU_ERR_DEVICE, "gen pack launch failed");
     HIP_TRY(hipStreamSynchronize(st));
   }
+  {
+    SketchBuild sketches;
+    int rc = sketch_begin(t, seg.get(), st, &sketches);
+    if (!rc && hipStreamSynchronize(st) != hipSuccess) rc = fail(PGPU_ERR_DEVICE, "sketch histogram failed");
+    if (!rc) rc = sketch_finish(t, seg.get(), st, &sketches);
+    if (rc) {
+      account_unpin(t, seg.get());
+      return rc;
+    }
+  }
   std::lock_guard<std::mutex> lk(t->mu);
   *handle = register_segment(t, std::move(seg));
   return 0;
diff --git a/pinot_amd/csrc/abi_table.cpp b/pinot_amd/csrc/abi_table.cpp
--- a/pinot_amd/csrc/abi_table.cpp
+++ b/pinot_amd/csrc/abi_table.cpp
@@ -411,6 +411,11 @@
         return fail(PGPU_ERR_DEVICE, "forward-index check launch failed: %s", hipGetErrorString(hipGetLastError()));
     HIP_TRY(hipMemcpyAsync(hmax.data(), dmax.p, check.size() * 4, hipMemcpyDeviceToHost, t->stream));
   }
+  SketchBuild sketches;
+  if (const int rc = sketch_begin(t, seg.get(), t->stream, &sketches)) {
+    account_unpin(t, seg.get());
+    return rc;
+  }
   HIP_TRY(hipStreamSynchronize(t->stream));
   for (size_t i = 0; i < check.size(); ++i)
     if ((int64_t)hmax[i] >= seg->cols[check[i]].card) {
@@ -418,6 +423,10 @@
       return fail(PGPU_ERR_INVALID_ARGUMENT, "column %d: forward index holds dictId %u, cardinality is %d", check[i],
                   hmax[i], seg->cols[check[i]].card);
     }
+  if (const int rc = sketch_finish(t, seg.get(), t->stream, &sketches)) {
+    account_unpin(t, seg.get());
+    return rc;
+  }
   std::lock_guard<std::mutex> lk(t->mu);
   if (any_raw) TRY(ensure_docid(t, d->num_docs, t->stream));
   *handle = register_segment(t, std::move(seg));
diff --git a/pinot_amd/csrc/col_sketch.h b/pinot_amd/csrc/col_sketch.h
--- /dev/null
+++ b/pinot_amd/csrc/col_sketch.h
@@ -0,0 +1,99 @@
+#pragma once
+#include <stdint.h>
+
+#include <algorithm>
+#include <vector>
+
+namespace pgpu {
+
+constexpr int kSketchHot = 127;
+constexpr int kSketchMaxCodes = 256;
+constexpr int kSketchBits = 8;
+constexpr int kSketchSetWords = kSketchMaxCodes / 32;
+
+struct ColSketch {
+  int32_t card = 0;
+  int32_t ncodes = 0;
+  std::vector<int32_t> first_id;
+  std::vector<uint8_t> singleton;
+  std::vector<uint8_t> lut;
+  int64_t singleton_docs = 0;
+  int64_t total_docs = 0;
+  int code(int64_t id) const { return id >= card ? ncodes : (int)lut[id]; }
+};
+
+template <typename Count>
+inline void sketch_assign(const Count* counts, int32_t card, ColSketch* out) {
+  ColSketch& s = *out;
+  s = ColSketch();
+  if (card <= 0) return;
+  s.card = card;
+  std::vector<int32_t> hot;
+  for (int32_t i = 0; i < card; ++i) {
+    s.total_docs += (int64_t)counts[i];
+    if (counts[i] > 0) hot.push_back(i);
+  }
+  auto hotter = [&](int32_t a, int32_t b) { return counts[a] != counts[b] ? counts[a] > counts[b] : a < b; };
+  if ((int)hot.size() > kSketchHot) {
+    std::nth_element(hot.begin(), hot.begin() + kSketchHot, hot.end(), hotter);
+    hot.resize(kSketchHot);
+  }
+  std::sort(hot.begin(), hot.end());
+  s.lut.assign((size_t)card, 0);
+  int32_t next = 0;
+  auto close_gap = [&](int32_t end) {
+    if (end <= next) return;
+    std::fill(s.lut.begin() + next, s.lut.begin() + end, (uint8_t)s.first_id.size());
+    s.first_id.push_back(next);
+    s.singleton.push_back(0);
+    next = end;
+  };
+  for (int32_t h : hot) {
+    close_gap(h);
+    s.lut[h] = (uint8_t)s.first_id.size();
+    s.first_id.push_back(h);
+    s.singleton.push_back(1);
+    s.singleton_docs += (int64_t)counts[h];
+    next = h + 1;
+  }
+  close_gap(card);
+  s.ncodes = (int32_t)s.first_id.size();
+  s.first_id.push_back(card);
+}
+
+inline bool sketch_range_exact(const ColSketch& s, int64_t lo, int64_t hi, int* clo, int* chi) {
+  if (s.ncodes <= 0 || lo < 0 || lo >= hi || hi > s.card) return false;
+  const int a = s.code(lo), b = s.code(hi);
+  if (s.first_id[a] != lo) return false;
+  if (hi != s.card && s.first_id[b] != hi) return false;
+  *clo = a;
+  *chi = b;
+  return true;
+}
+
+inline int64_t sketch_bits_set(const uint32_t* w, int64_t a, int64_t b) {
+  int64_t n = 0;
+  while (a < b) {
+    const int sh = (int)(a & 31);
+    const int64_t take = std::min<int64_t>(32 - sh, b - a);
+    uint32_t x = w[a >> 5] >> sh;
+    if (take < 32) x &= (1u << take) - 1u;
+    n += __builtin_popcount(x);
+    a += take;
+  }
+  return n;
+}
+
+inline bool sketch_set_exact(const ColSketch& s, const uint32_t* set, uint32_t* codes) {
+  if (s.ncodes <= 0) return false;
+  for (int k = 0; k < kSketchSetWords; ++k) codes[k] = 0;
+  for (int c = 0; c < s.ncodes; ++c) {
+    const int64_t a = s.first_id[c], b = s.first_id[c + 1];
+    const int64_t n = sketch_bits_set(set, a, b);
+    if (n == b - a) codes[c >> 5] |= 1u << (c & 31);
+    else if (n != 0) return false;
+  }
+  return true;
+}
+
+}
diff --git a/pinot_amd/csrc/device.h b/pinot_amd/csrc/device.h
--- a/pinot_amd/csrc/device.h
+++ b/pinot_amd/csrc/device.h
@@ -276,7 +276,8 @@
 }
 
 __device__ __forceinline__ uint32_t leaf_mask(KLeafC& L, KColC& C, int64_t group) {
-  return leaf_eval(L.kind, L.negate, L.lo, L.span, L.set, C.fwd, C.bits, group);
+  const uint32_t* lf = L.fwd;
+  return leaf_eval(L.kind, L.negate, L.lo, L.span, L.set, lf ? lf : C.fwd, lf ? L.bits : C.bits, group);
 }
 
 struct SegView {
@@ -347,8 +348,9 @@
   LeafReg r;
   KLeafC& L = S.leaves[l];
   KColC& C = S.cols[p.leaf_col[l]];
-  r.fwd = C.fwd;
-  r.bits = C.bits;
+  const uint32_t* lf = L.fwd;
+  r.fwd = lf ? lf : C.fwd;
+  r.bits = lf ? L.bits : C.bits;
   r.kind = L.kind;
   r.negate = L.negate;
   r.lo = L.lo;
diff --git a/pinot_amd/csrc/internal.h b/pinot_amd/csrc/internal.h
--- a/pinot_amd/csrc/internal.h
+++ b/pinot_amd/csrc/internal.h
@@ -48,6 +48,9 @@
   uint32_t lo;
   uint32_t span;
   const uint32_t* set;
+  const uint32_t* fwd;
+  int32_t bits;
+  int32_t pad;
 };
 
 constexpr int kMaxValueGaps = 16;
@@ -368,6 +371,10 @@
 int launch_unpack(const uint32_t* fwd, int32_t bits, int64_t start, int64_t n, int32_t* out, void* stream);
 int launch_gather_ids(const uint32_t* fwd, int32_t bits, const int32_t* docs, int32_t n, int32_t* out, void* stream);
 int launch_fwd_max(const void* d_fwd, int64_t n, int32_t bits, unsigned int* d_out, void* stream);
+int launch_sketch_hist(const uint32_t* fwd, int32_t bits, int32_t num_docs, int32_t card, uint32_t* counts,
+                       void* stream);
+int launch_sketch_encode(const uint32_t* fwd, int32_t bits, int32_t num_docs, int32_t card, const uint8_t* lut,
+                         uint32_t* out, void* stream);
 int launch_hash_unpack(uint64_t* table, const unsigned long long* hash_keys, int64_t cap, int32_t pack_slot,
                        int32_t shift, void* stream);
 int launch_table_init(uint64_t* table, const int32_t* slot_kind, int32_t num_slots, int64_t num_keys,
diff --git a/pinot_amd/csrc/k_sketch.hip b/pinot_amd/csrc/k_sketch.hip
--- /dev/null
+++ b/pinot_amd/csrc/k_sketch.hip
@@ -0,0 +1,109 @@
+#include "device.h"
+
+namespace pgpu {
+
+static inline hipStream_t S(void* s) { return reinterpret_cast<hipStream_t>(s); }
+
+constexpr int kSketchHistRange = 16384;
+constexpr int kSketchHistTiles = 8;
+
+__global__ __launch_bounds__(256) void sketch_hist_kernel(const uint32_t* __restrict__ fwd, const int32_t bits,
+                                                          const int32_t num_docs, const int32_t card,
+                                                          uint32_t* __restrict__ counts) {
+  __shared__ uint32_t h[kSketchHistRange];
+  const int tid = threadIdx.x;
+  const int32_t base = (int32_t)blockIdx.y * kSketchHistRange;
+  const uint32_t n = (uint32_t)(card - base < kSketchHistRange ? card - base : kSketchHistRange);
+  for (uint32_t i = tid; i < n; i += 256) h[i] = 0;
+  __syncthreads();
+  const int64_t ngroups = ((int64_t)num_docs + 31) >> 5;
+  for (int k = 0; k < kSketchHistTiles; ++k) {
+    const int64_t group = ((int64_t)blockIdx.x * kSketchHistTiles + k) * 256 + tid;
+    if (group >= ngroups) break;
+    const int64_t doc0 = group << 5;
+    uint32_t ids[16];
+    decode_group<0>(fwd, bits, group, ids);
+#pragma unroll
+    for (int i = 0; i < 16; ++i) {
+      const uint32_t id = ids[i] - (uint32_t)base;
+      if (doc0 + i < num_docs && id < n) atomicAdd(&h[id], 1u);
+    }
+    decode_group<16>(fwd, bits, group, ids);
+#pragma unroll
+    for (int i = 0; i < 16; ++i) {
+      const uint32_t id = ids[i] - (uint32_t)base;
+      if (doc0 + 16 + i < num_docs && id < n) atomicAdd(&h[id], 1u);
+    }
+  }
+  __syncthreads();
+  for (uint32_t i = tid; i < n; i += 256) {
+    const uint32_t v = h[i];
+    if (v) atomicAdd(counts + base + i, v);
+  }
+}
+
+__global__ __launch_bounds__(256) void sketch_encode_kernel(const uint32_t* __restrict__ fwd, const int32_t bits,
+                                                            const int32_t num_docs, const int32_t card,
+                                                            const uint8_t* __restrict__ lut, uint32_t* __restrict__ out) {
+  const int64_t group = (int64_t)blockIdx.x * 256 + threadIdx.x;
+  const int64_t ngroups = ((int64_t)num_docs + 31) >> 5;
+  if (group >= ngroups) return;
+  const int64_t doc0 = group << 5;
+  gmem<uint8_t>* __restrict__ t = gp(lut);
+  uint32_t w[8];
+  uint32_t ids[16];
+  decode_group<0>(fwd, bits, group, ids);
+#pragma unroll
+  for (int q = 0; q < 4; ++q) {
+    uint32_t word = 0;
+#pragma unroll
+    for (int j = 0; j < 4; ++j) {
+      const int i = q * 4 + j;
+      const uint32_t id = ids[i];
+      const uint32_t c = (doc0 + i < num_docs && id < (uint32_t)card) ? (uint32_t)t[id] : 0u;
+      word |= c << (8 * j);
+    }
+    w[q] = word;
+  }
+  decode_group<16>(fwd, bits, group, ids);
+#pragma unroll
+  for (int q = 0; q < 4; ++q) {
+    uint32_t word = 0;
+#pragma unroll
+    for (int j = 0; j < 4; ++j) {
+      const int i = q * 4 + j;
+      const uint32_t id = ids[i];
+      const uint32_t c = (doc0 + 16 + i < num_docs && id < (uint32_t)card) ? (uint32_t)t[id] : 0u;
+      word |= c << (8 * j);
+    }
+    w[4 + q] = word;
+  }
+  uint32_t* o = out + group * 8;
+#pragma unroll
+  for (int q = 0; q < 8; ++q) o[q] = w[q];
+}
+
+int launch_sketch_hist(const uint32_t* fwd, int32_t bits, int32_t num_docs, int32_t card, uint32_t* counts,
+                       void* stream) {
+  if (num_docs <= 0 || card <= 0) return 0;
+  if (bits < 1 || bits > 31) return -1;
+  const int64_t tiles = ((int64_t)num_docs + kTileDocs - 1) / kTileDocs;
+  const int64_t gx = (tiles + kSketchHistTiles - 1) / kSketchHistTiles;
+  const int64_t gy = ((int64_t)card + kSketchHistRange - 1) / kSketchHistRange;
+  if (gx > INT32_MAX || gy > 65535) return -1;
+  hipLaunchKernelGGL(sketch_hist_kernel, dim3((unsigned)gx, (unsigned)gy), dim3(256), 0, S(stream), fwd, bits, num_docs,
+                     card, counts);
+  return PGPU_HIP_OK(hipGetLastError());
+}
+
+int launch_sketch_encode(const uint32_t* fwd, int32_t bits, int32_t num_docs, int32_t card, const uint8_t* lut,
+                         uint32_t* out, void* stream) {
+  if (num_docs <= 0 || card <= 0) return 0;
+  if (bits < 1 || bits > 31) return -1;
+  const int64_t grid = ((((int64_t)num_docs + 31) >> 5) + 255) / 256;
+  hipLaunchKernelGGL(sketch_encode_kernel, dim3((unsigned)grid), dim3(256), 0, S(stream), fwd, bits, num_docs, card, lut,
+                     out);
+  return PGPU_HIP_OK(hipGetLastError());
+}
+
+}
diff --git a/pinot_amd/csrc/rt.h b/pinot_amd/csrc/rt.h
--- a/pinot_amd/csrc/rt.h
+++ b/pinot_amd/csrc/rt.h
@@ -31,6 +31,7 @@
 #include <vector>
 
 #include "../../include/pinotgpu.h"
+#include "col_sketch.h"
 #include "comm.h"
 #include "filter_stats.h"
 #include "host_common.h"
@@ -326,6 +327,9 @@
   int64_t raw_min = 0, raw_max = 0;
   pgpu::FxRange fx;
   bool fx_known = false;
+  uint8_t* d_sketch = nullptr;
+  int64_t sketch_bytes = 0;
+  pgpu::ColSketch sketch;
 };
 
 struct StarTreeDev {
@@ -367,6 +371,7 @@
     for (auto& c : cols) {
       if (c.d_key) hipFree(c.d_key);
       if (c.d_val) hipFree(c.d_val);
+      if (c.d_sketch) hipFree(c.d_sketch);
     }
     for (auto& d : derived) {
       if (!d) continue;
@@ -499,6 +504,8 @@
   int device = 0;
   mutable std::mutex cfg_mu;
   pgpu_config cfg = default_config();
+  int32_t sketch_min_bits = 12;
+  double sketch_min_cover = 0.125;
   std::vector<std::string> names;
   std::vector<int32_t> types;
   std::mutex mu;
@@ -702,6 +709,8 @@
   int segments_matched_filter = 0;
   int64_t leaf_kinds[kLeafKinds] = {};
   int64_t regex_stats[4] = {};
+  bool sketch_on = true;
+  int64_t sketch_leaves[2] = {};
   std::vector<uint8_t> seg_scanned;
   int grid = 0;
   size_t lds_bytes = 0;
diff --git a/pinot_amd/csrc/rt_decls.h b/pinot_amd/csrc/rt_decls.h
--- a/pinot_amd/csrc/rt_decls.h
+++ b/pinot_amd/csrc/rt_decls.h
@@ -31,6 +31,20 @@
 int decode_raw_forward_index(int type, const uint8_t* b, int64_t n, int32_t num_docs, int c, RawValues* out);
 int parse_raw_column(int type, const pgpu_column_buffers& cb, int32_t num_docs, int c, Column* col, RawValues* out);
 int64_t register_segment(pgpu_table_s* t, std::unique_ptr<Segment> seg_in);
+
+struct SketchBuild {
+  std::vector<int> cols;
+  std::vector<int64_t> off;
+  DevBuf d_counts;
+  std::vector<uint32_t> h_counts;
+  double min_cover = 0;
+  SketchBuild() = default;
+  SketchBuild(const SketchBuild&) = delete;
+  SketchBuild& operator=(const SketchBuild&) = delete;
+  ~SketchBuild() { d_counts.release(); }
+};
+int sketch_begin(pgpu_table_s* t, Segment* seg, hipStream_t st, SketchBuild* b);
+int sketch_finish(pgpu_table_s* t, Segment* seg, hipStream_t st, SketchBuild* b);
 
 int regex_check(const char* pattern, int32_t* states, int32_t* classes, int64_t* table_bytes);
 int regex_match_host(const char* pattern, const uint8_t* value, int64_t len, int32_t* matched);
diff --git a/pinot_amd/csrc/rt_dict.cpp b/pinot_amd/csrc/rt_dict.cpp
--- a/pinot_amd/csrc/rt_dict.cpp
+++ b/pinot_amd/csrc/rt_dict.cpp
@@ -391,6 +391,7 @@
   int64_t fwd_words = 0;
   for (const auto& c : s->cols) {
     if (c.inv) t->device_bytes -= c.inv->bytes;
+    t->device_bytes -= c.sketch_bytes;
     t->device_bytes -= (c.lut ? 4 * std::max(c.card, 1) : 0) +
                        (c.d_key ? 16 * (c.raw ? raw_padded_docs(s->num_docs) : std::max(c.card, 1)) : 0);
     if (!c.raw) fwd_words += (c.fwd_words + 63) & ~int64_t(63);
diff --git a/pinot_amd/csrc/rt_plan_create.cpp b/pinot_amd/csrc/rt_plan_create.cpp
--- a/pinot_amd/csrc/rt_plan_create.cpp
+++ b/pinot_amd/csrc/rt_plan_create.cpp
@@ -46,6 +46,7 @@
   std::vector<uint8_t> scanned;
   int64_t tiles = 0, entries = 0, matched = 0, sel_docs = 0, exempt = 0;
   int64_t leaf_kinds[kLeafKinds] = {};
+  int64_t sketch_leaves[2] = {};
   double sel = 1.0;
   int rc = 0;
   std::string err;
@@ -1047,10 +1048,51 @@
   return gathers || !P->exprs.empty();
 }
 
-void emit_set_words(Chunk& C, const LeafHost& lh, int64_t field) {
+void emit_set_words(Chunk& C, const uint32_t* words, size_t n, int64_t field) {
   C.set_fix.emplace_back(field, (int64_t)C.set_words.size());
-  C.set_words.insert(C.set_words.end(), lh.set.begin(), lh.set.end());
+  C.set_words.insert(C.set_words.end(), words, words + n);
   if (C.set_words.size() & 1) C.set_words.push_back(0);
+}
+
+struct SketchLeaf {
+  bool on_sketched = false;
+  bool exact = false;
+  bool use = false;
+  uint32_t lo = 0, span = 0;
+  uint32_t codes[kSketchSetWords] = {};
+};
+
+void choose_sketch_leaves(const PlanCtx& cx, const Segment* s, const std::vector<LeafHost>& leaves,
+                          std::array<SketchLeaf, kMaxLeaves>& sk, Chunk& C) {
+  const pgpu_plan_s* P = cx.P;
+  const int nl = P->num_leaves;
+  for (SketchLeaf& x : sk) x = SketchLeaf();
+  if (!P->sketch_on || nl > kMaxLeaves) return;
+  const Column* lcol[kMaxLeaves] = {};
+  for (int l = 0; l < nl; ++l) {
+    const LeafHost& lh = leaves[l];
+    if ((lh.kind != LEAF_RANGE && lh.kind != LEAF_SET) || P->expr_leaf(l)) continue;
+    const Column& col = pred_column(P, s, cx.q, l);
+    if (!col.d_sketch || col.sketch.ncodes <= 0) continue;
+    lcol[l] = &col;
+    sk[l].on_sketched = true;
+    if (lh.kind == LEAF_RANGE) {
+      int a = 0, b = 0;
+      sk[l].exact = sketch_range_exact(col.sketch, lh.lo, (int64_t)lh.lo + lh.span, &a, &b);
+      sk[l].lo = (uint32_t)a;
+      sk[l].span = (uint32_t)(b - a);
+    } else {
+      sk[l].exact = (int64_t)lh.set.size() * 32 >= col.card && sketch_set_exact(col.sketch, lh.set.data(), sk[l].codes);
+    }
+  }
+  for (int l = 0; l < nl; ++l) {
+    if (!sk[l].on_sketched) continue;
+    bool all = true;
+    for (int m = 0; m < nl; ++m)
+      if (lcol[m] == lcol[l]) all &= sk[m].exact;
+    sk[l].use = all;
+    C.sketch_leaves[all ? 0 : 1]++;
+  }
 }
 
 void emit_raw_task(Chunk& C, const Segment* s, const Column& col, const LeafHost& lh, KLeaf& kl, int64_t field) {
@@ -1149,6 +1191,8 @@
 
 void emit_leaves(const PlanCtx& cx, const Segment* s, const std::vector<LeafHost>& leaves, KLeaf* kl, int64_t kl_off,
                  Chunk& C) {
+  std::array<SketchLeaf, kMaxLeaves> sk;
+  choose_sketch_leaves(cx, s, leaves, sk, C);
   for (int k = 0; k < cx.P->num_leaves; ++k) {
     const LeafHost& lh = leaves[cx.perm[k]];
     const Column& col = pred_column(cx.P, s, cx.q, cx.perm[k]);
@@ -1158,7 +1202,19 @@
     kl[k].lo = lh.lo;
     kl[k].span = lh.span;
     kl[k].set = nullptr;
-    if (lh.kind == LEAF_SET) emit_set_words(C, lh, field);
+    const SketchLeaf* sl = cx.perm[k] < kMaxLeaves && sk[cx.perm[k]].use ? &sk[cx.perm[k]] : nullptr;
+    if (sl) {
+      kl[k].fwd = reinterpret_cast<const uint32_t*>(col.d_sketch);
+      kl[k].bits = kSketchBits;
+      if (lh.kind == LEAF_RANGE) {
+        kl[k].lo = sl->lo;
+        kl[k].span = sl->span;
+      }
+    }
+    if (lh.kind == LEAF_SET) {
+      if (sl) emit_set_words(C, sl->codes, kSketchSetWords, field);
+      else emit_set_words(C, lh.set.data(), lh.set.size(), field);
+    }
     if (lh.kind == LEAF_RAW_RANGE || lh.kind == LEAF_RAW_IN) emit_raw_task(C, s, col, lh, kl[k], field);
     if (lh.kind == LEAF_EXPR_RANGE || lh.kind == LEAF_EXPR_IN)
       emit_expr_task(C, s, cx.P->leaf_exprs[cx.perm[k]], lh, kl[k], field);
@@ -1397,6 +1453,7 @@
   P->scanned_entries_model += C.entries;
   P->post_exempt_docs += C.exempt;
   for (int k = 0; k < kLeafKinds; ++k) P->leaf_kinds[k] += C.leaf_kinds[k];
+  for (int k = 0; k < 2; ++k) P->sketch_leaves[k] += C.sketch_leaves[k];
   if (P->sel_docs == 0 && C.sel_docs) { P->sel_estimate = C.sel; P->sel_docs = C.sel_docs; }
 }
 
@@ -1504,6 +1561,10 @@
   PlanCtx cx{t, q, P, se};
   cx.t_start = trace_on() ? now_us() : 0;
   P->cfg = table_config(t);
+  {
+    std::lock_guard<std::mutex> g(t->cfg_mu);
+    P->sketch_on = t->sketch_min_bits > 0;
+  }
   if (q->num_group_by < 0) return fail(PGPU_ERR_INVALID_ARGUMENT, "negative group-by count");
   if (q->num_group_by > kMaxKeys) return fail(PGPU_ERR_UNSUPPORTED, "more than %d group-by columns", kMaxKeys);
   if (q->num_predicates > kMaxLeaves) return fail(PGPU_ERR_UNSUPPORTED, "more than %d predicates", kMaxLeaves);
diff --git a/pinot_amd/csrc/rt_sketch.cpp b/pinot_amd/csrc/rt_sketch.cpp
--- /dev/null
+++ b/pinot_amd/csrc/rt_sketch.cpp
@@ -0,0 +1,139 @@
+#include "rt_decls.h"
+
+namespace pgpu {
+
+namespace {
+constexpr int32_t kSketchMaxCard = 1 << 28;
+}
+
+int sketch_begin(pgpu_table_s* t, Segment* seg, hipStream_t st, SketchBuild* b) {
+  int32_t min_bits;
+  {
+    std::lock_guard<std::mutex> g(t->cfg_mu);
+    min_bits = t->sketch_min_bits;
+    b->min_cover = t->sketch_min_cover;
+  }
+  b->cols.clear();
+  b->off.clear();
+  if (min_bits <= 0 || seg->num_docs <= 0) return 0;
+  int64_t total = 0;
+  for (size_t c = 0; c < seg->cols.size(); ++c) {
+    const Column& col = seg->cols[c];
+    if (col.raw || col.sorted || !col.d_fwd || col.bits < min_bits || col.bits <= kSketchBits || col.card <= 0 ||
+        col.card > kSketchMaxCard)
+      continue;
+    b->cols.push_back((int)c);
+    b->off.push_back(total);
+    total += col.card;
+  }
+  if (b->cols.empty()) return 0;
+  TRY(b->d_counts.ensure((size_t)total * 4));
+  HIP_TRY(hipMemsetAsync(b->d_counts.p, 0, (size_t)total * 4, st));
+  for (size_t k = 0; k < b->cols.size(); ++k) {
+    const Column& col = seg->cols[b->cols[k]];
+    if (launch_sketch_hist(col.d_fwd, col.bits, seg->num_docs, col.card, b->d_counts.as<uint32_t>() + b->off[k], st))
+      return fail(PGPU_ERR_DEVICE, "sketch histogram launch failed: %s", hipGetErrorString(hipGetLastError()));
+  }
+  b->h_counts.resize((size_t)total);
+  HIP_TRY(hipMemcpyAsync(b->h_counts.data(), b->d_counts.p, (size_t)total * 4, hipMemcpyDeviceToHost, st));
+  return 0;
+}
+
+int sketch_finish(pgpu_table_s* t, Segment* seg, hipStream_t st, SketchBuild* b) {
+  if (b->cols.empty()) return 0;
+  std::vector<size_t> kept;
+  std::vector<int64_t> lut_off;
+  std::vector<uint8_t> luts;
+  for (size_t k = 0; k < b->cols.size(); ++k) {
+    Column& col = seg->cols[b->cols[k]];
+    ColSketch s;
+    sketch_assign(b->h_counts.data() + b->off[k], col.card, &s);
+    if (s.ncodes <= 0 || s.total_docs != seg->num_docs) continue;
+    if ((double)s.singleton_docs < b->min_cover * (double)s.total_docs) continue;
+    lut_off.push_back((int64_t)luts.size());
+    luts.insert(luts.end(), s.lut.begin(), s.lut.end());
+    luts.resize((luts.size() + 255) & ~size_t(255), 0);
+    col.sketch = std::move(s);
+    kept.push_back(k);
+  }
+  if (kept.empty()) return 0;
+  DevBuf d_luts;
+  struct Release { DevBuf& b; ~Release() { b.release(); } } release_luts{d_luts};
+  TRY(d_luts.ensure(luts.size()));
+  HIP_TRY(hipMemcpyAsync(d_luts.p, luts.data(), luts.size(), hipMemcpyHostToDevice, st));
+  int rc = 0;
+  for (size_t i = 0; i < kept.size() && !rc; ++i) {
+    Column& col = seg->cols[b->cols[kept[i]]];
+    const int64_t bytes = padded_fwd_words(seg->num_docs, kSketchBits) * 4;
+    void* p = nullptr;
+    const hipError_t e = hipMalloc(&p, (size_t)bytes);
+    if (e != hipSuccess) {
+      rc = fail(e == hipErrorOutOfMemory ? PGPU_ERR_OUT_OF_MEMORY : PGPU_ERR_DEVICE, "sketch of column %d: %s",
+                b->cols[kept[i]], hipGetErrorString(e));
+      break;
+    }
+    col.d_sketch = reinterpret_cast<uint8_t*>(p);
+    col.sketch_bytes = bytes;
+    t->device_bytes += bytes;
+    if (hipMemsetAsync(p, 0, (size_t)bytes, st) != hipSuccess ||
+        launch_sketch_encode(col.d_fwd, col.bits, seg->num_docs, col.card, d_luts.as<uint8_t>() + lut_off[i],
+                             reinterpret_cast<uint32_t*>(p), st))
+      rc = fail(PGPU_ERR_DEVICE, "sketch encode launch failed: %s", hipGetErrorString(hipGetLastError()));
+  }
+  const hipError_t es = hipStreamSynchronize(st);
+  if (!rc && es != hipSuccess) rc = fail(PGPU_ERR_DEVICE, "sketch build: %s", hipGetErrorString(es));
+  if (rc) {
+    for (size_t k : kept) seg->cols[b->cols[k]].sketch = ColSketch();
+  }
+  return rc;
+}
+
+}
+
+extern "C" {
+
+int pgpu_table_set_filter_sketch(pgpu_table t, int32_t min_bits, double min_cover) try {
+  PGPU_ABI_GUARD;
+  if (!t || min_bits < 0 || min_bits > 31 || !(min_cover >= 0.0 && min_cover <= 1.0))
+    return fail(PGPU_ERR_INVALID_ARGUMENT, "bad filter-sketch arguments");
+  {
+    std::lock_guard<std::mutex> g(t->cfg_mu);
+    t->sketch_min_bits = min_bits;
+    t->sketch_min_cover = min_cover;
+  }
+  t->version.fetch_add(1);
+  plan_cache_clear(t);
+  return 0;
+} PGPU_ABI_CATCH
+
+int pgpu_segment_sketch_info(pgpu_table t, int64_t h, int32_t column, int32_t* ncodes, int64_t* singleton_docs,
+                             int64_t* bytes, int32_t* first_id_out, int32_t cap) try {
+  PGPU_ABI_GUARD;
+  if (!t || !ncodes || cap < 0 || (cap > 0 && !first_id_out)) return fail(PGPU_ERR_INVALID_ARGUMENT, "bad arguments");
+  std::lock_guard<std::mutex> lk(t->mu);
+  auto it = t->segments.find(h);
+  if (it == t->segments.end()) return fail(PGPU_ERR_NOT_FOUND, "unknown segment handle %lld", (long long)h);
+  const Segment& seg = *it->second;
+  if (column < 0 || column >= (int)seg.cols.size()) return fail(PGPU_ERR_INVALID_ARGUMENT, "bad column %d", column);
+  const Column& col = seg.cols[column];
+  const bool has = col.d_sketch && col.sketch.ncodes > 0;
+  *ncodes = has ? col.sketch.ncodes : 0;
+  if (singleton_docs) *singleton_docs = has ? col.sketch.singleton_docs : 0;
+  if (bytes) *bytes = has ? col.sketch_bytes : 0;
+  for (int32_t k = 0; has && k < cap && k <= col.sketch.ncodes; ++k) first_id_out[k] = col.sketch.first_id[k];
+  return 0;
+} PGPU_ABI_CATCH
+
+int pgpu_plan_sketch_leaves(pgpu_plan P, int64_t* pairs_using_sketch, int64_t* pairs_declined) try {
+  PGPU_ABI_GUARD;
+  if (!P || !pairs_using_sketch || !pairs_declined) return fail(PGPU_ERR_INVALID_ARGUMENT, "bad arguments");
+  *pairs_using_sketch = P->sketch_leaves[0];
+  *pairs_declined = P->sketch_leaves[1];
+  for (const auto& part : P->parts) {
+    *pairs_using_sketch += part.plan->sketch_leaves[0];
+    *pairs_declined += part.plan->sketch_leaves[1];
+  }
+  return 0;
+} PGPU_ABI_CATCH
+
+}
diff --git a/pinot_amd/executor.py b/pinot_amd/executor.py
--- a/pinot_amd/executor.py
+++ b/pinot_amd/executor.py
@@ -216,6 +216,20 @@
         c = L.ConfigC()
         L.check(self.lib.pgpu_config_default(ctypes.byref(c)))
         L.check(self.lib.pgpu_table_set_config(self.handle, ctypes.byref(c)))
+
+    def set_filter_sketch(self, min_bits=12, min_cover=0.125):
+        L.check(self.lib.pgpu_table_set_filter_sketch(self.handle, int(min_bits), float(min_cover)))
+
+    def segment_sketch_info(self, handle, column):
+        n, docs, nbytes = ctypes.c_int32(), ctypes.c_int64(), ctypes.c_int64()
+        first = np.zeros(257, dtype=np.int32)
+        L.check(self.lib.pgpu_segment_sketch_info(self.handle, handle, self.index[column], ctypes.byref(n),
+                                                  ctypes.byref(docs), ctypes.byref(nbytes),
+                                                  L.ptr(first, ctypes.c_int32), len(first)))
+        if n.value == 0:
+            return None
+        return {"ncodes": n.value, "singleton_docs": docs.value, "bytes": nbytes.value,
+                "first_id": first[:n.value + 1].copy()}
 
     def close(self):
         if self.handle:
@@ -592,6 +606,11 @@
         L.check(self.lib.pgpu_plan_leaf_kinds(self.handle, L.ptr(out, ctypes.c_int64)))
         return {n: int(v) for n, v in zip(L.LEAF_KIND_NAMES, out) if v}
 
+    def sketch_leaves(self):
+        used, declined = ctypes.c_int64(), ctypes.c_int64()
+        L.check(self.lib.pgpu_plan_sketch_leaves(self.handle, ctypes.byref(used), ctypes.byref(declined)))
+        return used.value, declined.value
+
     def regexp_stats(self):
         out = np.zeros(4, dtype=np.int64)
         L.check(self.lib.pgpu_plan_regexp_stats(self.handle, L.ptr(out, ctypes.c_int64)))
```

Measured after the change: 1795 billion rows/s (median of 6 runs). +14.3%, better.
